# YangChenApril/AMContrast3D

Measured on AMD Instinct MI355X. Metric: train-step points/sec (fwd+bwd) on 24k-pt S3DIS clouds, higher is better.
Workload: dtype f32; 1 GPU; PointNeXt-S + AMContrast3D-AA, S3DIS-shaped 24000-pt voxelised (0.04 m) clouds, batch 8/GPU, fwd + CE/contrast loss + bwd + clip + AdamW; global_batch=8, points=24000, parallelism=dp1, launch=hipGraph replay, batches_per_joint_fps_launch=4, geometry_queue_cus=176, feature_graph_segments=1, collectives=none, update=captured in the feature graph

## Files before the change

### amcontrast3d_amd/_lib.py

```python
import ctypes
import os
import subprocess

_CSRC = os.path.join(os.path.dirname(os.path.abspath(__file__)), "csrc")
_SO = os.environ.get("AMC3D_LIB") or os.path.join(_CSRC, "libamc3d_hip.so")

_vp, _i, _f, _sz, _l = ctypes.c_void_p, ctypes.c_int, ctypes.c_float, ctypes.c_size_t, ctypes.c_long
_ll = ctypes.c_longlong

SIGNATURES = {
    "amc3d_version": (ctypes.c_char_p, []),
    "amc3d_last_error": (ctypes.c_char_p, []),
    "amc3d_stream_create_dedicated": (_i, [ctypes.POINTER(ctypes.c_void_p)]),
    "amc3d_stream_create_masked": (_i, [_vp, _i, _i]),
    "amc3d_reserve_scratch": (_i, [_i, _vp, _vp]),
    "amc3d_stream_destroy": (_i, [_vp]),
    "amc3d_grid_search_workspace_bytes": (_sz, [_i, _i, _i]),
    "amc3d_ball_query": (_i, [_i, _i, _i, _f, _i, _vp, _vp, _vp, _vp, _sz, _vp]),
    "amc3d_group_points": (_i, [_i, _i, _i, _i, _i, _vp, _vp, _vp, _vp]),
    "amc3d_group_points_grad": (_i, [_i, _i, _i, _i, _i, _vp, _vp, _vp, _vp, _sz, _vp]),
    "amc3d_gather_points": (_i, [_i, _i, _i, _i, _vp, _vp, _vp, _vp]),
    "amc3d_gather_points_grad": (_i, [_i, _i, _i, _i, _vp, _vp, _vp, _vp]),
    "amc3d_fps_workspace_bytes": (_sz, [_i, _i]),
    "amc3d_furthest_point_sampling": (_i, [_i, _i, _i, _vp, _vp, _vp, _vp, _sz, _vp]),
    "amc3d_three_nn": (_i, [_i, _i, _i, _vp, _vp, _vp, _vp, _vp, _sz, _vp]),
    "amc3d_three_interpolate": (_i, [_i, _i, _i, _i, _vp, _vp, _vp, _vp, _vp]),
    "amc3d_three_interpolate_add": (_i, [_i, _i, _i, _i, _vp, _vp, _vp, _vp, _vp, _vp]),
    "amc3d_three_interpolate_grad": (_i, [_i, _i, _i, _i, _vp, _vp, _vp, _vp, _vp, _sz, _vp]),
    "amc3d_three_interpolate_grad_route": (_i, [_i, _i, _i, _i, ctypes.POINTER(_i), ctypes.POINTER(_i)]),
    "amc3d_three_interpolate_grad_write": (_i, [_i, _i, _i, _i, _vp, _vp, _vp, _vp, _vp]),
    "amc3d_three_interpolate_grad_lds": (_i, [_i, _i, _i, _i, _i, _i, _i, _vp, _vp, _vp, _vp, _vp]),
    "amc3d_knnquery_workspace_bytes": (_sz, [_i, _i, _i, _i]),
    "amc3d_knnquery_uses_grid": (_i, [_i, _i, _i, _i]),
    "amc3d_knnquery": (_i, [_i, _i, _i, _i, _vp, _vp, _vp, _vp, _vp, _vp, _vp, _sz, _i, _vp]),
    "amc3d_vote_labels": (_i, [_i, _i, _i, _vp, _vp, _vp, _vp]),
    "amc3d_posmask": (_i, [_i, _i, _i, _vp, _vp, _vp, _vp]),
    "amc3d_ambiguity_workspace_bytes": (_sz, [_i]),
    "amc3d_ambiguity": (_i, [_i, _i, _i, _i, _f, _vp, _vp, _vp, _vp, _vp, _sz, _vp]),
    "amc3d_contrast_csr_workspace_bytes": (_sz, [_i]),
    "amc3d_contrast_csr": (_i, [_i, _i, _i, _vp, _vp, _vp, _vp, _sz, _vp]),
    "amc3d_contrast_backward_csr_supported": (_i, [_i]),
    "amc3d_contrast_backward_rows_supported": (_i, [_i]),
    "amc3d_contrast_backward_csr": (_i, [_i, _i, _i, _i, _vp, _vp, _vp, _vp, _vp, _vp, _vp, _f, _f, _f, _vp, _vp, _vp, _vp,
                                         _vp, _vp]),
    "amc3d_contrast_mutual_workspace_bytes": (_sz, [_i]),
    "amc3d_contrast_mutual": (_i, [_i, _i, _i, _vp, _vp, _vp, _vp, _vp, _vp, _sz, _vp]),
    "amc3d_contrast_backward_mutual_workspace_bytes": (_sz, [_i]),
    "amc3d_contrast_backward_mutual": (_i, [_i, _i, _i, _i, _vp, _vp, _vp, _vp, _vp, _vp, _vp, _f, _f, _f, _vp, _vp, _vp, _vp, _vp, _sz,
                                            _vp, _vp]),
    "amc3d_contrast_variant_forward": (_i, [_i, _i, _i, _i, _vp, _vp, _vp, _vp, _vp, _i, _i, _i, _i, _f, _f, _f, _vp, _vp, _vp, _vp,
                                            _vp, _vp]),
    "amc3d_contrast_variant_backward": (_i, [_i, _i, _i, _i, _vp, _vp, _vp, _vp, _vp, _vp, _vp, _i, _i, _i, _i, _f, _f, _f, _vp, _vp,
                                             _vp, _vp, _vp, _vp]),
    "amc3d_adamw_chunk": (_i, []),
    "amc3d_adamw_step": (_i, [_vp, _vp, _i, ctypes.c_double, ctypes.c_double, _f, _f, _vp, _vp, _vp]),
    "amc3d_select_anchors_ints": (_sz, [_i]),
    "amc3d_select_anchors": (_i, [_i, _vp, _vp, _sz, _vp]),
    "amc3d_contrast_forward": (_i, [_i, _i, _i, _i, _vp, _vp, _vp, _vp, _vp, _f, _f, _f, _vp, _vp, _vp, _vp, _vp, _vp, _vp]),
    "amc3d_contrast_forward_cm": (_i, [_i, _i, _i, _i, _i, _vp, _vp, _vp, _vp, _vp, _f, _f, _f, _vp, _vp, _vp, _vp, _vp, _vp, _vp]),
    "amc3d_contrast_backward": (_i, [_i, _i, _i, _i, _vp, _vp, _vp, _vp, _vp, _vp, _f, _f, _f, _vp, _vp, _vp, _vp, _vp]),
    "amc3d_grouped_conv_supported": (_i, [_i, _i]),
    "amc3d_transpose_cn": (_i, [_i, _i, _i, _vp, _vp, _vp]),
    "amc3d_grouped_conv_forward": (_i, [_i, _i, _i, _i, _i, _i, _vp, _vp, _vp, _vp, _vp, _vp]),
    "amc3d_grouped_conv_workspace_bytes": (_sz, [_i, _i, _i, _i, _i]),
    "amc3d_grouped_conv_backward": (_i, [_i, _i, _i, _i, _i, _i, _vp, _vp, _vp, _vp, _vp, _vp, _vp, _vp, _sz, _vp]),
    "amc3d_confusion_update": (_i, [_i, _i, _l, _vp, _vp, _ll, _i, _vp, _vp, _vp]),
    "amc3d_cross_entropy_workspace_bytes": (_sz, [_i, _l]),
    "amc3d_cross_entropy_forward": (_i, [_i, _i, _l, _vp, _vp, _ll, _vp, _vp, _vp, _sz, _vp]),
    "amc3d_cross_entropy_backward": (_i, [_i, _i, _l, _vp, _vp, _ll, _vp, _vp, _vp, _vp, _vp]),
    "amc3d_cross_entropy_general_workspace_bytes": (_sz, [_i, _l]),
    "amc3d_cross_entropy_general_forward": (_i, [_i, _i, _l, _vp, _vp, _ll, _i, _f, _vp, _vp, _vp, _vp, _sz, _vp]),
    "amc3d_cross_entropy_general_backward": (_i, [_i, _i, _l, _vp, _vp, _ll, _i, _f, _vp, _vp, _vp, _vp, _vp, _vp]),
    "amc3d_pointwise_conv_forward": (_i, [_i, _i, _i, _l, _vp, _vp, _vp, _vp, _vp]),
    "amc3d_pointwise_conv_forward_workspace_bytes": (_sz, [_i, _i, _i, _l, _i]),
    "amc3d_pointwise_conv_forward_ws": (_i, [_i, _i, _i, _l, _vp, _vp, _vp, _vp, _vp, _sz, _vp]),
    "amc3d_pointwise_conv_workspace_bytes": (_sz, [_i, _i, _i, _l]),
    "amc3d_pointwise_conv_backward": (_i, [_i, _i, _i, _l, _vp, _vp, _vp, _vp, _vp, _vp, _sz, _vp]),
    "amc3d_pointwise_conv_forward_strided": (_i, [_i, _i, _i, _l, _vp, _vp, _l, _vp, _vp, _vp, _sz, _vp]),
    "amc3d_pointwise_conv_backward_strided": (_i, [_i, _i, _i, _l, _vp, _vp, _l, _vp, _vp, _i, _vp, _l, _vp, _sz, _vp]),
    "amc3d_bn_residual_forward": (_i, [_i, _i, _l, _f, _f] + [_vp] * 11 + [_vp, _sz, _vp]),
    "amc3d_bn_residual_backward": (_i, [_i, _i, _l] + [_vp] * 11 + [_vp, _sz, _vp]),
    "amc3d_split_columns": (_i, [_i, _i, _i, _vp, _vp, _vp, _vp]),
    "amc3d_join_columns": (_i, [_i, _i, _i, _vp, _vp, _vp, _vp]),
    "amc3d_masked_refine_workspace_ints": (_sz, [_i]),
    "amc3d_masked_refine_forward": (_i, [_i, _i, _i, _i, _i, _vp, _vp, _vp, _f, _f, _f, _vp, _vp, _vp, _vp, _vp, _vp]),
    "amc3d_masked_refine_backward": (_i, [_i, _i, _i, _f, _vp, _vp, _vp, _vp, _vp]),
    "amc3d_bn_sigmoid_forward": (_i, [_i, _i, _l, _f, _f] + [_vp] * 10 + [_vp, _sz, _vp]),
    "amc3d_bn_sigmoid_backward": (_i, [_i, _i, _l] + [_vp] * 10 + [_vp, _sz, _vp]),
    "amc3d_bias_grad": (_i, [_i, _i, _l, _vp, _vp, _vp]),
    "amc3d_sa_residual_forward": (_i, [_i, _i, _i, _i, _i] + [_vp] * 8),
    "amc3d_sa_residual_workspace_bytes": (_sz, [_i, _i, _i, _i]),
    "amc3d_sa_residual_backward": (_i, [_i, _i, _i, _i, _i] + [_vp] * 11 + [_sz, _vp]),
    "amc3d_index_duplicates_workspace_bytes": (_sz, [_i, _i]),
    "amc3d_index_duplicates": (_i, [_i, _i, _i, _vp, _vp, _vp, _sz, _vp]),
    "amc3d_augment_workspace_bytes": (_sz, [_i]),
    "amc3d_augment_clouds": (_i, [_i, _i, _i, _f, _f] + [_vp] * 10 + [_sz, _vp]),
    "amc3d_voxelize_workspace_bytes": (_sz, [_i]),
    "amc3d_voxelize": (_i, [_i, _vp, ctypes.c_double] + [_vp] * 7 + [_sz, _vp]),
    "amc3d_voxel_select": (_i, [_i, _vp, _vp, _vp, _vp, _vp, _vp]),
    "amc3d_crop_nearest_workspace_bytes": (_sz, [_i]),
    "amc3d_crop_nearest": (_i, [_i, _vp, _i, _i, _vp, _vp, _vp, _sz, _vp]),
    "amc3d_voxelize_f64": (_i, [_i, _vp, ctypes.c_double] + [_vp] * 7 + [_sz, _vp]),
    "amc3d_crop_nearest_f64_workspace_bytes": (_sz, [_i]),
    "amc3d_crop_nearest_f64": (_i, [_i, _vp, _i, _i, _vp, _vp, _vp, _sz, _vp]),
    "amc3d_scannet_stats_workspace_bytes": (_sz, [_i]),
    "amc3d_scannet_room_stats": (_i, [_i, _vp, _vp, _vp, _vp, _vp, _sz, _vp]),
    "amc3d_scannet_transform_rooms": (_i, [_i, _ll] + [_vp] * 9 + [_vp]),
    "amc3d_scannet_crop_tail": (_i, [_i, _i] + [_vp] * 10 + [_vp]),
    "amc3d_s3dis_voxelize_workspace_bytes": (_sz, [_i, _ll]),
    "amc3d_s3dis_voxelize_rooms": (_i, [_i, _ll, _i, _vp, _vp, _vp, ctypes.c_double] + [_vp] * 8 + [_vp, _sz, _vp]),
    "amc3d_s3dis_crop_workspace_bytes": (_sz, [_i]),
    "amc3d_s3dis_select_crop": (_i, [_i, _i, _i, _i] + [_vp] * 13 + [_vp, _sz, _vp]),
    "amc3d_s3dis_crop_tail": (_i, [_i, _i, _i, _i] + [_vp] * 12 + [_vp]),
    "amc3d_scannet_voxelize_workspace_bytes": (_sz, [_i, _ll]),
    "amc3d_scannet_voxelize_rooms": (_i, [_i, _ll, _vp, _vp, ctypes.c_double] + [_vp] * 8 + [_vp, _sz, _vp]),
    "amc3d_scannet_crop_workspace_bytes": (_sz, [_i]),
    "amc3d_scannet_select_crop": (_i, [_i, _i, _i, _i] + [_vp] * 13 + [_vp, _sz, _vp]),
    "amc3d_scannet_crop_tail_workspace_bytes": (_sz, [_i]),
    "amc3d_scannet_crop_tail_rooms": (_i, [_i, _i, _i, _i] + [_vp] * 12 + [_vp, _sz, _vp]),
    "amc3d_room_parts": (_i, [_i, _i, _i] + [_vp] * 6 + [_vp]),
    "amc3d_part_batch_workspace_bytes": (_sz, [_i]),
    "amc3d_part_batch": (_i, [_i] * 6 + [_vp] * 12 + [_sz, _vp]),
    "amc3d_vote_parts": (_i, [_i, _i, _i, _i] + [_vp] * 8 + [_vp]),
    "amc3d_s3dis_part_batch_workspace_bytes": (_sz, [_i]),
    "amc3d_s3dis_part_batch": (_i, [_i] * 7 + [_vp] * 14 + [_sz, _vp]),
    "amc3d_room_representatives": (_i, [_i, _i] + [_vp] * 7 + [_vp]),
    "amc3d_expand_parts": (_i, [_i, _i, _i] + [_vp] * 6 + [_vp]),
    "amc3d_local_aggregation_supported": (_i, [_i, _i]),
    "amc3d_group_moments_bytes": (_sz, [_i, _i]),
    "amc3d_group_moments": (_i, [_i, _i, _i, _i, _vp, _vp, _vp, _sz, _vp]),
    "amc3d_local_aggregation_workspace_bytes": (_sz, [_i, _i, _i, _i]),
    "amc3d_local_aggregation_forward": (_i, [_i] * 7 + [_f, _f] + [_vp] * 18 + [_i, _vp, _vp, _sz, _vp]),
    "amc3d_local_aggregation_forward_strided": (_i, [_i] * 7 + [_f, _f] + [_vp] * 4 + [_l] + [_vp] * 14 + [_i, _vp, _vp, _sz, _vp]),
    "amc3d_local_aggregation_backward": (_i, [_i] * 6 + [_vp] * 17 + [_i, _vp, _vp, _vp, _sz, _vp]),
    "amc3d_local_aggregation_backward_strided": (_i, [_i] * 6 + [_vp] * 7 + [_l] + [_vp] * 8 + [_l] + [_vp] * 2 + [_i, _vp, _vp, _vp, _sz, _vp]),
    "amc3d_local_aggregation_csr_workspace_bytes": (_sz, [_i, _i, _i, _i]),
    "amc3d_local_aggregation_workspace_q_offset": (_sz, [_i, _i, _i, _i]),
    "amc3d_local_aggregation_backward_csr": (_i, [_i] * 6 + [_vp] * 19 + [_i, _vp, _vp, _vp, _sz, _vp]),
    "amc3d_local_aggregation_backward_csr_strided": (_i, [_i] * 6 + [_vp] * 7 + [_l] + [_vp] * 10 + [_l] + [_vp] * 2 + [_i, _vp, _vp, _vp, _sz, _vp]),
    "amc3d_three_interpolate_grad_csr": (_i, [_i, _i, _i, _i, _vp, _vp, _vp, _vp, _vp, _vp, _vp]),
    "amc3d_masked_refine_backward_csr": (_i, [_i, _i, _i, _f, _vp, _vp, _vp, _vp, _vp, _vp, _vp]),
    "amc3d_pointwise_conv_forward_bf16": (_i, [_i, _i, _i, _l, _vp, _vp, _vp, _vp, _vp]),
    "amc3d_pointwise_conv_workspace_bytes_bf16": (_sz, [_i, _i, _i, _l]),
    "amc3d_pointwise_conv_backward_bf16": (_i, [_i, _i, _i, _l, _vp, _vp, _vp, _vp, _vp, _vp, _sz, _vp]),
    "amc3d_grouped_conv_bn_supported": (_i, [_i, _i]),
    "amc3d_grouped_conv_bn_forward": (_i, [_i] * 7 + [_f, _f] + [_vp] * 16 + [_i, _vp, _vp, _sz, _vp]),
    "amc3d_grouped_conv_bn_forward_strided": (_i, [_i] * 7 + [_f, _f] + [_vp] * 4 + [_l] + [_vp] * 12 + [_i, _vp, _vp, _sz, _vp]),
    "amc3d_grouped_conv_bn_backward": (_i, [_i] * 6 + [_vp] * 15 + [_i, _vp, _vp, _vp, _sz, _vp]),
    "amc3d_grouped_conv_bn_backward_strided": (_i, [_i] * 6 + [_vp] * 5 + [_l] + [_vp] * 8 + [_l] + [_vp] * 2 + [_i, _vp, _vp, _vp, _sz, _vp]),
    "amc3d_group_csr_workspace_bytes": (_sz, [_i, _i, _i]),
    "amc3d_group_csr": (_i, [_i, _i, _i, _i, _vp, _vp, _vp, _vp, _sz, _vp]),
    "amc3d_group_moments_csr": (_i, [_i, _i, _i, _i, _vp, _vp, _vp, _vp, _sz, _vp]),
    "amc3d_grouped_conv_bn_csr_workspace_bytes": (_sz, [_i, _i, _i, _i, _i]),
    "amc3d_grouped_conv_bn_backward_csr": (_i, [_i] * 6 + [_vp, _i] + [_vp] * 16 + [_i, _vp, _vp, _vp, _sz, _vp]),
    "amc3d_grouped_conv_bn_backward_csr_strided": (_i, [_i] * 6 + [_vp, _i] + [_vp] * 6 + [_l] + [_vp] * 8 + [_l] + [_vp] * 2 + [_i, _vp, _vp, _vp, _sz, _vp]),
    "amc3d_group_csr_dp": (_i, [_i, _i, _i, _vp, _vp, _vp, _vp]),
    "amc3d_sa_tail_supported": (_i, [_i, _i, _i]),
    "amc3d_sa_tail_pays": (_i, [_i, _i]),
    "amc3d_sa_tail_workspace_bytes": (_sz, [_i, _i, _i, _i]),
    "amc3d_sa_tail_forward": (_i, [_i, _i, _i, _i, _i] + [_vp] * 8 + [_f, _f, _i] + [_vp] * 10 + [_sz, _vp]),
    "amc3d_sa_tail_backward": (_i, [_i, _i, _i, _i, _i] + [_vp] * 10 + [_i, _vp, _vp, _vp, _vp, _i] + [_vp] * 5 + [_sz, _vp]),
    "amc3d_bn_workspace_bytes": (_sz, [_i]),
    "amc3d_bn_stats": (_i, [_i, _i, _l, _f, _vp, _vp, _vp, _vp, _vp, _sz, _vp]),
    "amc3d_bn_forward": (_i, [_i, _i, _l, _i, _i, _f, _f, _vp, _vp, _vp, _vp, _vp, _vp, _vp, _vp, _vp, _vp, _vp, _vp, _sz, _vp]),
    "amc3d_bn_update_running": (_i, [_i, _f, _vp, _vp, _vp, _vp, _vp, _vp]),
    "amc3d_bn_act": (_i, [_i, _i, _l, _i, _vp, _vp, _vp, _vp, _vp, _vp, _vp]),
    "amc3d_bn_max": (_i, [_i, _i, _i, _i, _i, _vp, _vp, _vp, _vp, _vp, _vp, _vp, _vp]),
    "amc3d_bn_backward": (_i, [_i, _i, _l, _i, _i, _vp, _vp, _vp, _vp, _vp, _vp, _vp, _vp, _vp, _vp, _vp, _sz, _vp]),
    "amc3d_bn_sums": (_i, [_i, _i, _l, _vp, _vp, _vp, _sz, _vp]),
    "amc3d_bn_forward_synced": (_i, [_i, _i, _l, _i, _i, _f, _f, _vp, _vp, _vp, _vp, _vp, _vp, _vp, _vp, _vp, _vp, _vp, _vp, _vp]),
    "amc3d_bn_backward_sums": (_i, [_i, _i, _l, _i, _i, _vp, _vp, _vp, _vp, _vp, _vp, _vp, _vp, _vp, _vp, _vp, _sz, _vp]),
    "amc3d_bn_backward_synced": (_i, [_i, _i, _l, _i, _i, _vp, _vp, _vp, _vp, _vp, _vp, _vp, _vp, _vp, _vp, _vp]),
}


def build(force=False):
    cmd = ["make", "-C", _CSRC, "-j8"] + (["-B"] if force else [])
    proc = subprocess.run(cmd, stdout=subprocess.PIPE, stderr=subprocess.STDOUT, text=True)
    if proc.returncode != 0:
        raise RuntimeError("building libamc3d_hip.so failed:\n" + proc.stdout)
    return _SO


_lib = None


def load():
    global _lib
    if _lib is not None:
        return _lib
    if not os.path.exists(_SO):
        raise ImportError(
            f"{_SO} not found: the HIP extension is not built (run `python -c 'import __graft_entry__ as g; "
            f"g.build()'` or `make -C {_CSRC}`); there is no CPU fallback")
    import torch
    lib = ctypes.CDLL(_SO)
    for name, (res, args) in SIGNATURES.items():
        fn = getattr(lib, name)
        fn.restype = res
        fn.argtypes = args
    _lib = lib
    return lib


def check(status, what):
    if status != 0:
        raise RuntimeError(f"{what} failed (hipError {status}): {load().amc3d_last_error().decode()}")
```

### amcontrast3d_amd/csrc/loss.hip

```cpp
#include "common.h"

#include <type_traits>

namespace amc {

__global__ __launch_bounds__(256) void vote_labels_kernel(int m, int kr, int ncls, const int *__restrict__ labels0,
                                                          const int *__restrict__ nbr, int *__restrict__ out)
{
    const int lane = threadIdx.x & 63;
    const int q = blockIdx.x * 4 + (threadIdx.x >> 6);
    if (q >= m) return;
    int c0 = -1, c1 = -1;
    if (lane < kr) c0 = labels0[nbr[(size_t)q * kr + lane]];
    if (lane + 64 < kr) c1 = labels0[nbr[(size_t)q * kr + lane + 64]];
    int best = -1, bestc = 0;
    for (int c = 0; c < ncls; ++c) {
        const int cnt = (int)__popcll(__ballot(c0 == c)) + (int)__popcll(__ballot(c1 == c));
        if (cnt > best) { best = cnt; bestc = c; }
    }
    if (lane == 0) out[q] = bestc;
}

__global__ void posmask_kernel(int m, int k, int nbr_stride, const int *__restrict__ labels,
                               const int *__restrict__ nbr, unsigned char *__restrict__ posmask)
{
    const size_t t = (size_t)blockIdx.x * blockDim.x + threadIdx.x;
    if (t >= (size_t)m * k) return;
    const int i = (int)(t / k), j = (int)(t - (size_t)i * k);
    posmask[t] = labels[nbr[(size_t)i * nbr_stride + j]] == labels[i] ? 1 : 0;
}

__global__ __launch_bounds__(256) void ambiguity_stats_kernel(int m, int k, int nbr_stride, int mode,
                                                              const float *__restrict__ p,
                                                              const unsigned char *__restrict__ posmask,
                                                              const int *__restrict__ nbr, int *__restrict__ n_pos,
                                                              float *__restrict__ d_pos, float *__restrict__ d_neg,
                                                              int *__restrict__ max_npos)
{
    const int i = blockIdx.x * blockDim.x + threadIdx.x;
    int np = 0;
    if (i < m) {
        const float px = p[(size_t)i * 3], py = p[(size_t)i * 3 + 1], pz = p[(size_t)i * 3 + 2];
        const float ss = __fadd_rn(__fadd_rn(__fmul_rn(px, px), __fmul_rn(py, py)), __fmul_rn(pz, pz));
        float dp = 0.f, dn = 0.f;
        for (int j = 0; j < k; ++j) {
            const int nb = nbr[(size_t)i * nbr_stride + j];
            const float qx = p[(size_t)nb * 3], qy = p[(size_t)nb * 3 + 1], qz = p[(size_t)nb * 3 + 2];
            const float dot = __fadd_rn(__fadd_rn(__fmul_rn(px, qx), __fmul_rn(py, qy)), __fmul_rn(pz, qz));
            const float sd = __fadd_rn(__fadd_rn(__fmul_rn(qx, qx), __fmul_rn(qy, qy)), __fmul_rn(qz, qz));
            float dd = __fadd_rn(__fadd_rn(__fmul_rn(-2.f, dot), ss), sd);
            if (mode == 3) dd = sqrtf(__fadd_rn(fabsf(dd), 1e-12f));
            const bool pos = posmask[(size_t)i * k + j] != 0;
            np += pos ? 1 : 0;
            dp = __fadd_rn(dp, pos ? dd : 0.f);
            dn = __fadd_rn(dn, pos ? 0.f : dd);
        }
        n_pos[i] = np;
        d_pos[i] = mode == 1 ? 5.f : dp;
        d_neg[i] = mode == 1 ? 5.f : dn;
    }
    int w = np;
    for (int s = 32; s >= 1; s >>= 1) w = max(w, __shfl_xor(w, s, 64));
    if ((threadIdx.x & 63) == 0 && w > 0) atomicMax(max_npos, w);
}

__global__ void ambiguity_kernel(int m, int k, float beta, const int *__restrict__ n_pos,
                                 const float *__restrict__ d_pos, const float *__restrict__ d_neg,
                                 const int *__restrict__ max_npos, float *__restrict__ a)
{
    const int i = blockIdx.x * blockDim.x + threadIdx.x;
    if (i >= m) return;
    const int top = *max_npos;
    const int np = n_pos[i];
    float v = __fdiv_rn((float)abs(np - top), (float)top);
    if (0 < np && np < top) {
        const float cc = __fsub_rn(__fdiv_rn((float)np, d_pos[i]), __fdiv_rn((float)(k - np), d_neg[i]));
        v = __fdiv_rn(1.f, __fadd_rn(1.f, powf(2.718281828459045f, __fmul_rn(beta, cc))));
    }
    a[i] = v;
}

__global__ __launch_bounds__(256) void row_norm_kernel(int m, int C, const float *__restrict__ f,
                                                       float *__restrict__ norm)
{
    const int lane = threadIdx.x & 63;
    const int i = blockIdx.x * 4 + (threadIdx.x >> 6);
    if (i >= m) return;
    float s = 0.f;
    for (int c = lane; c < C; c += 64) {
        const float v = f[(size_t)i * C + c];
        s += v * v;
    }
    for (int sft = 32; sft >= 1; sft >>= 1) s += __shfl_xor(s, sft, 64);
    if (lane == 0) norm[i] = fmaxf(sqrtf(s), 1e-8f);
}

template <int LPR>
__global__ __launch_bounds__(256) void row_unit_kernel(int m, const float *__restrict__ f, float *__restrict__ norm,
                                                       float *__restrict__ unit)
{
    const int q = threadIdx.x & (LPR - 1);
    const long i = ((long)blockIdx.x * 256 + threadIdx.x) / LPR;
    if (i >= m) return;
    float4 v = reinterpret_cast<const float4 *>(f)[i * LPR + q];
    float s = v.x * v.x;
    s += v.y * v.y;
    s += v.z * v.z;
    s += v.w * v.w;
#pragma unroll
    for (int d = LPR / 2; d >= 1; d >>= 1) s += __shfl_xor(s, d, 64);
    const float n = fmaxf(sqrtf(s), 1e-8f);
    v.x = __fdiv_rn(v.x, n); v.y = __fdiv_rn(v.y, n); v.z = __fdiv_rn(v.z, n); v.w = __fdiv_rn(v.w, n);
    reinterpret_cast<float4 *>(unit)[i * LPR + q] = v;
    if (q == 0) norm[i] = n;
}

template <int LPR, int TP>
__global__ __launch_bounds__(256) void row_unit_cm_kernel(int n, const float *__restrict__ f_cm, float *__restrict__ norm,
                                                          float *__restrict__ unit)
{
    constexpr int C = 4 * LPR, TS = TP + 1;
    extern __shared__ float s_tile[];
    const int b = blockIdx.y, n0 = blockIdx.x * TP;
    for (int e = threadIdx.x; e < C * TP; e += 256) {
        const int ch = e / TP, pt = e - ch * TP;
        s_tile[ch * TS + pt] = n0 + pt < n ? f_cm[((size_t)b * C + ch) * n + n0 + pt] : 0.f;
    }
    __syncthreads();
    const int q = threadIdx.x & (LPR - 1);
    for (int pl = threadIdx.x / LPR; pl < TP; pl += 256 / LPR) {
        float4 v = make_float4(s_tile[(4 * q) * TS + pl], s_tile[(4 * q + 1) * TS + pl], s_tile[(4 * q + 2) * TS + pl],
                               s_tile[(4 * q + 3) * TS + pl]);
        float s = v.x * v.x;
        s += v.y * v.y;
        s += v.z * v.z;
        s += v.w * v.w;
#pragma unroll
        for (int d = LPR / 2; d >= 1; d >>= 1) s += __shfl_xor(s, d, 64);
        const float nv = fmaxf(sqrtf(s), 1e-8f);
        v.x = __fdiv_rn(v.x, nv); v.y = __fdiv_rn(v.y, nv); v.z = __fdiv_rn(v.z, nv); v.w = __fdiv_rn(v.w, nv);
        if (n0 + pl < n) {
            const size_t i = (size_t)b * n + n0 + pl;
            reinterpret_cast<float4 *>(unit)[i * LPR + q] = v;
            if (q == 0) norm[i] = nv;
        }
    }
}

__device__ __forceinline__ bool contrast_selected(float a) { return 0.f < a && a <= 1.f; }

__device__ __forceinline__ bool contrast_anchor(const int *__restrict__ sel, int m, int w, const float *__restrict__ a, int &i,
                                                float &ai)
{
    if (w >= (sel ? sel[0] : m)) return false;
    i = sel ? sel[1 + w] : w;
    ai = a[i];
    return true;
}

__device__ __forceinline__ float contrast_margin(float mu, float a, float nu) { return __fadd_rn(__fmul_rn(mu, a), nu); }

__device__ __forceinline__ float contrast_exp(float s, bool pos, float margin, float temperature)
{
    return expf(__fdiv_rn(pos ? __fsub_rn(s, margin) : s, temperature));
}

__device__ __forceinline__ float contrast_coef(float scale, float psum, float tsum, float temperature)
{
    const float r = psum / tsum;
    return -scale / ((r + 1e-12f) * tsum * tsum * temperature);
}

__device__ __forceinline__ float contrast_edge_g(float coef, float e, bool pos, float nsum, float psum)
{
    return coef * e * (pos ? nsum : -psum);
}

__device__ __forceinline__ float group32_sum(float v)
{
#pragma unroll
    for (int s = 16; s >= 1; s >>= 1) v += __shfl_xor(v, s, 64);
    return v;
}

struct ContrastSums { float psum, nsum, tsum; };

__device__ __forceinline__ ContrastSums contrast_sums32(int k, int sub, const unsigned char *__restrict__ pm_i,
                                                        const float *__restrict__ sim_i, float margin, float temperature)
{
    ContrastSums r{0.f, 0.f, 0.f};
    for (int j = sub; j < k; j += 32) {
        const bool pos = pm_i[j] != 0;
        const float e = contrast_exp(sim_i[j], pos, margin, temperature);
        r.psum += pos ? e : 0.f;
        r.nsum += pos ? 0.f : e;
        r.tsum += e;
    }
    for (int s = 16; s >= 1; s >>= 1) {
        r.psum += __shfl_xor(r.psum, s, 64);
        r.nsum += __shfl_xor(r.nsum, s, 64);
        r.tsum += __shfl_xor(r.tsum, s, 64);
    }
    return r;
}

__device__ __forceinline__ float row_cosine(const float *__restrict__ fi, const float *__restrict__ fj, float ni, float nj, int C)
{
    float a0 = 0.f, a1 = 0.f, a2 = 0.f, a3 = 0.f;
    if ((C & 3) == 0) {
        for (int c = 0; c < C; c += 4) {
            const float4 u = *reinterpret_cast<const float4 *>(fi + c);
            const float4 v = *reinterpret_cast<const float4 *>(fj + c);
            a0 += __fdiv_rn(u.x, ni) * __fdiv_rn(v.x, nj);
            a1 += __fdiv_rn(u.y, ni) * __fdiv_rn(v.y, nj);
            a2 += __fdiv_rn(u.z, ni) * __fdiv_rn(v.z, nj);
            a3 += __fdiv_rn(u.w, ni) * __fdiv_rn(v.w, nj);
        }
    } else {
        int c = 0;
        for (; c + 3 < C; c += 4) {
            a0 += __fdiv_rn(fi[c], ni) * __fdiv_rn(fj[c], nj);
            a1 += __fdiv_rn(fi[c + 1], ni) * __fdiv_rn(fj[c + 1], nj);
            a2 += __fdiv_rn(fi[c + 2], ni) * __fdiv_rn(fj[c + 2], nj);
            a3 += __fdiv_rn(fi[c + 3], ni) * __fdiv_rn(fj[c + 3], nj);
        }
        for (; c < C; ++c) a0 += __fdiv_rn(fi[c], ni) * __fdiv_rn(fj[c], nj);
    }
    return (a0 + a1) + (a2 + a3);
}

__device__ __forceinline__ float unit_dot4(const float4 &a, const float4 &b)
{
    return __fmaf_rn(a.w, b.w, __fmaf_rn(a.z, b.z, __fmaf_rn(a.y, b.y, __fmul_rn(a.x, b.x))));
}

constexpr int UNIT_U = 4;

template <int LPR>
__device__ __forceinline__ void unit_row_cosines(const float4 *__restrict__ h4, const float4 &u, int q, const int (&x)[UNIT_U],
                                                 float4 (&v)[UNIT_U], float (&s)[UNIT_U])
{
#pragma unroll
    for (int t = 0; t < UNIT_U; ++t) v[t] = x[t] >= 0 ? h4[(unsigned)x[t] * (unsigned)LPR + (unsigned)q] : make_float4(0.f, 0.f, 0.f, 0.f);
#pragma unroll
    for (int t = 0; t < UNIT_U; ++t) {
        float acc = unit_dot4(u, v[t]);
#pragma unroll
        for (int d = LPR / 2; d >= 1; d >>= 1) acc += __shfl_xor(acc, d, 64);
        s[t] = acc;
    }
}

template <int LPR>
__device__ __forceinline__ void unit_gather_indices(const int *__restrict__ nbr, int i, int nbr_stride, int k, int j0, int r,
                                                    int (&nb)[UNIT_U])
{
#pragma unroll
    for (int t = 0; t < UNIT_U; ++t) {
        const int j = j0 + t * (64 / LPR) + r;
        nb[t] = j < k ? nbr[(size_t)i * nbr_stride + j] : -1;
    }
}

template <int LPR>
__device__ __forceinline__ float unit_gather_rows(const float4 *__restrict__ h4, const float4 &u, int q, const int (&nb)[UNIT_U])
{
    float4 v[UNIT_U];
    float c[UNIT_U];
    unit_row_cosines<LPR>(h4, u, q, nb, v, c);
    float s = 0.f;
#pragma unroll
    for (int t = 0; t < UNIT_U; ++t) s = q == t ? c[t] : s;
    return s;
}

__device__ __forceinline__ float contrast_projection(float norm, float s) { return norm > 1e-8f ? s : 0.f; }

template <int LPA, int VPT>
struct EdgeWalk {
    static constexpr int U = VPT >= 8 ? 2 : (VPT >= 4 ? 4 : 8);
    float fhi[VPT], gi[VPT];

    __device__ __forceinline__ void begin(int C, int sub, const float *__restrict__ f, int i, float ni)
    {
#pragma unroll
        for (int v = 0; v < VPT; ++v) {
            const int c = sub + v * LPA;
            fhi[v] = c < C ? __fdiv_rn(f[(size_t)i * C + c], ni) : 0.f;
            gi[v] = 0.f;
        }
    }

    __device__ __forceinline__ void chunk(int C, int sub, const float *__restrict__ f, float ni, int cnt, int nb_l, float sj_l,
                                          float nj_l, float g_l, float *__restrict__ grad_f)
    {
        for (int jj = 0; jj < cnt; jj += U) {
            int nb[U];
            float fj[U][VPT];
#pragma unroll
            for (int u = 0; u < U; ++u) {
                const int src = min(jj + u, LPA - 1);
                const int t = __shfl(nb_l, src, LPA);
                nb[u] = jj + u < cnt ? t : -1;
            }
#pragma unroll
            for (int u = 0; u < U; ++u)
#pragma unroll
                for (int v = 0; v < VPT; ++v) {
                    const int c = sub + v * LPA;
                    fj[u][v] = (nb[u] >= 0 && c < C) ? f[(size_t)nb[u] * C + c] : 0.f;
                }
#pragma unroll
            for (int u = 0; u < U; ++u) {
                const int src = min(jj + u, LPA - 1);
                const float g = __shfl(g_l, src, LPA), sj = __shfl(sj_l, src, LPA), nj = __shfl(nj_l, src, LPA);
                if (nb[u] < 0) continue;
                const float gin = g / ni, gjn = g / nj;
                const float si = contrast_projection(ni, sj), sx = contrast_projection(nj, sj);
#pragma unroll
                for (int v = 0; v < VPT; ++v) {
                    const int c = sub + v * LPA;
                    if (c < C) {
                        const float fhj = __fdiv_rn(fj[u][v], nj);
                        gi[v] += gin * (fhj - si * fhi[v]);
                        atomicAdd(grad_f + (size_t)nb[u] * C + c, gjn * (fhi[v] - sx * fhj));
                    }
                }
            }
        }
    }

    __device__ __forceinline__ void finish(int C, int sub, int i, float *__restrict__ grad_f)
    {
#pragma unroll
        for (int v = 0; v < VPT; ++v) {
            const int c = sub + v * LPA;
            if (c < C) atomicAdd(grad_f + (size_t)i * C + c, gi[v]);
        }
    }
};

__device__ __forceinline__ void rows_edge(int t, int total, int own, int n, int k, const int *__restrict__ nbr_n,
                                          const int *__restrict__ rev_n, const float *__restrict__ gco,
                                          const float *__restrict__ sim, int &x, float &g, float &s)
{
    x = -1; g = 0.f; s = 0.f;
    if (t < total) {
        int pos;
        if (t < own) { pos = n * k + t; x = nbr_n[t]; }
        else { pos = rev_n[t - own]; x = pos / k; }
        g = gco[pos];
        s = sim[pos];
    }
}

__device__ __forceinline__ void rows_accumulate(float4 &acc, float g, float s, float nn, const float4 &fn, const float4 &v, float nx)
{
    const float gn = g / nn;
    const float sn = contrast_projection(nn, s);
    acc.x += gn * (__fdiv_rn(v.x, nx) - sn * fn.x);
    acc.y += gn * (__fdiv_rn(v.y, nx) - sn * fn.y);
    acc.z += gn * (__fdiv_rn(v.z, nx) - sn * fn.z);
    acc.w += gn * (__fdiv_rn(v.w, nx) - sn * fn.w);
}

__global__ __launch_bounds__(256) void select_count_kernel(int m, const float *__restrict__ a, int *__restrict__ sel)
{
    __shared__ int s_cnt[4];
    const int i = blockIdx.x * 256 + threadIdx.x;
    const bool s = i < m && contrast_selected(a[i]);
    const int c = (int)__popcll(__ballot(s));
    if ((threadIdx.x & 63) == 0) s_cnt[threadIdx.x >> 6] = c;
    __syncthreads();
    if (threadIdx.x == 0) sel[(size_t)m + 1 + blockIdx.x] = s_cnt[0] + s_cnt[1] + s_cnt[2] + s_cnt[3];
}

__global__ __launch_bounds__(256) void select_write_kernel(int m, const float *__restrict__ a, int *__restrict__ sel)
{
    __shared__ int s_part[4], s_cnt[4];
    const int *bc = sel + (size_t)m + 1;
    int before = 0;
    for (int b = threadIdx.x; b < (int)blockIdx.x; b += 256) before += bc[b];
    for (int s = 32; s >= 1; s >>= 1) before += __shfl_xor(before, s, 64);
    const int i = blockIdx.x * 256 + threadIdx.x;
    const bool sl = i < m && contrast_selected(a[i]);
    const unsigned long long mask = __ballot(sl);
    const int lane = threadIdx.x & 63, wv = threadIdx.x >> 6;
    if (lane == 0) { s_part[wv] = before; s_cnt[wv] = (int)__popcll(mask); }
    __syncthreads();
    int base = s_part[0] + s_part[1] + s_part[2] + s_part[3];
    for (int w = 0; w < wv; ++w) base += s_cnt[w];
    if (sl) sel[1 + base + (int)__popcll(mask & ((1ull << lane) - 1ull))] = i;
    if (blockIdx.x == gridDim.x - 1 && threadIdx.x == 0)
        sel[0] = s_part[0] + s_part[1] + s_part[2] + s_part[3] + s_cnt[0] + s_cnt[1] + s_cnt[2] + s_cnt[3];
}

template <int LPR>
__global__ __launch_bounds__(256) void contrast_forward_unit_kernel(
    int m, int k, int nbr_stride, const float *__restrict__ unit, const int *__restrict__ nbr,
    const unsigned char *__restrict__ posmask, const float *__restrict__ a, const int *__restrict__ sel, float mu, float nu,
    float temperature, float *__restrict__ sim, float *__restrict__ stats, float *__restrict__ loss_pt)
{
    constexpr int R = 64 / LPR;
    const int lane = threadIdx.x & 63, q = lane & (LPR - 1), r = lane / LPR;
    int i;
    float ai;
    if (!contrast_anchor(sel, m, blockIdx.x * 4 + (threadIdx.x >> 6), a, i, ai)) return;
    if (!contrast_selected(ai)) {
        if (lane == 0) loss_pt[i] = 0.f;
        return;
    }
    const float margin = contrast_margin(mu, ai, nu);
    const float4 *h4 = reinterpret_cast<const float4 *>(unit);
    const float4 u = h4[(size_t)i * LPR + q];
    float psum = 0.f, tsum = 0.f, nsum = 0.f;
    for (int j0 = 0; j0 < k; j0 += UNIT_U * R) {
        int nb[UNIT_U];
        unit_gather_indices<LPR>(nbr, i, nbr_stride, k, j0, r, nb);
        const int jq = j0 + q * R + r;
        const bool mine = q < UNIT_U && jq < k;
        const bool pos = mine ? posmask[(size_t)i * k + jq] != 0 : false;
        const float s = unit_gather_rows<LPR>(h4, u, q, nb);
        if (mine) {
            if (sim) sim[(size_t)i * k + jq] = s;
            const float e = contrast_exp(s, pos, margin, temperature);
            psum += pos ? e : 0.f;
            nsum += pos ? 0.f : e;
            tsum += e;
        }
    }
#pragma unroll
    for (int d = 1; d < 64; d <<= 1) {
        psum += __shfl_xor(psum, d, 64);
        tsum += __shfl_xor(tsum, d, 64);
    }
    if (stats) {
#pragma unroll
        for (int d = 1; d < 64; d <<= 1) nsum += __shfl_xor(nsum, d, 64);
    }
    if (lane == 0) {
        loss_pt[i] = -logf(__fadd_rn(__fdiv_rn(psum, tsum), 1e-12f));
        if (stats) { stats[(size_t)i * 2] = psum; stats[(size_t)i * 2 + 1] = nsum; }
    }
}

__global__ __launch_bounds__(256) void contrast_forward_kernel(
    int m, int C, int k, int nbr_stride, const float *__restrict__ f, const float *__restrict__ norm,
    const int *__restrict__ nbr, const unsigned char *__restrict__ posmask, const float *__restrict__ a,
    const int *__restrict__ sel, float mu, float nu, float temperature, float *__restrict__ sim,
    float *__restrict__ loss_pt)
{
    const int sub = threadIdx.x & 31;
    int i;
    float ai;
    if (!contrast_anchor(sel, m, (blockIdx.x * blockDim.x + threadIdx.x) >> 5, a, i, ai)) return;
    if (!contrast_selected(ai)) {
        if (sub == 0) loss_pt[i] = 0.f;
        return;
    }
    const float ni = norm[i];
    const float margin = contrast_margin(mu, ai, nu);
    const float *fi = f + (size_t)i * C;
    float psum = 0.f, tsum = 0.f;
    for (int j0 = 0; j0 < k; j0 += 32) {
        const int j = j0 + sub;
        float e = 0.f;
        bool pos = false;
        if (j < k) {
            const int nb = nbr[(size_t)i * nbr_stride + j];
            const float nj = norm[nb];
            const float acc = row_cosine(fi, f + (size_t)nb * C, ni, nj, C);
            sim[(size_t)i * k + j] = acc;
            pos = posmask[(size_t)i * k + j] != 0;
            e = contrast_exp(acc, pos, margin, temperature);
        }
        psum += pos ? e : 0.f;
        tsum += e;
    }
    for (int s = 16; s >= 1; s >>= 1) {
        psum += __shfl_xor(psum, s, 64);
        tsum += __shfl_xor(tsum, s, 64);
    }
    if (sub == 0) loss_pt[i] = -logf(__fadd_rn(__fdiv_rn(psum, tsum), 1e-12f));
}

__global__ __launch_bounds__(1024) void masked_mean_kernel(int m, const float *__restrict__ loss_pt,
                                                           const float *__restrict__ a, float *__restrict__ out)
{
    __shared__ double s_sum[16];
    __shared__ int s_cnt[16];
    double sum = 0.0;
    int cnt = 0;
    const int m4 = ((((uintptr_t)loss_pt | (uintptr_t)a) & 15) == 0) ? (m & ~3) : 0;
    for (int i0 = threadIdx.x * 4; i0 < m4; i0 += 4096 * 4) {
        float4 lv[4], av[4];
#pragma unroll
        for (int u = 0; u < 4; ++u) {
            const int i = i0 + u * 4096;
            const bool ok = i < m4;
            lv[u] = ok ? *reinterpret_cast<const float4 *>(loss_pt + i) : make_float4(0.f, 0.f, 0.f, 0.f);
            av[u] = ok ? *reinterpret_cast<const float4 *>(a + i) : make_float4(-1.f, -1.f, -1.f, -1.f);
        }
#pragma unroll
        for (int u = 0; u < 4; ++u) {
            const float l4[4] = {lv[u].x, lv[u].y, lv[u].z, lv[u].w}, a4[4] = {av[u].x, av[u].y, av[u].z, av[u].w};
#pragma unroll
            for (int e = 0; e < 4; ++e)
                if (contrast_selected(a4[e])) { sum += (double)l4[e]; cnt += 1; }
        }
    }
    for (int i = m4 + threadIdx.x; i < m; i += 1024) {
        const float ai = a[i];
        if (contrast_selected(ai)) { sum += (double)loss_pt[i]; cnt += 1; }
    }
    for (int s = 32; s >= 1; s >>= 1) {
        sum += __shfl_xor(sum, s, 64);
        cnt += __shfl_xor(cnt, s, 64);
    }
    if ((threadIdx.x & 63) == 0) { s_sum[threadIdx.x >> 6] = sum; s_cnt[threadIdx.x >> 6] = cnt; }
    __syncthreads();
    if (threadIdx.x == 0) {
        double t = 0.0;
        int c = 0;
        for (int w = 0; w < 16; ++w) { t += s_sum[w]; c += s_cnt[w]; }
        out[0] = (float)(t / (double)c);
        out[1] = (float)c;
    }
}

template <int LPA, int VPT>
__global__ __launch_bounds__(256) void contrast_backward_kernel(
    int m, int C, int k, int nbr_stride, const float *__restrict__ f, const float *__restrict__ norm,
    const int *__restrict__ nbr, const unsigned char *__restrict__ posmask, const float *__restrict__ a,
    const int *__restrict__ sel, float mu, float nu, float temperature, const float *__restrict__ sim,
    const float *__restrict__ mean_cnt, const float *__restrict__ grad_out, float *__restrict__ grad_f)
{
    const int sub = threadIdx.x & (LPA - 1);
    int i;
    float ai;
    if (!contrast_anchor(sel, m, (blockIdx.x * blockDim.x + threadIdx.x) / LPA, a, i, ai)) return;
    if (!contrast_selected(ai)) return;
    const float scale = grad_out[0] / mean_cnt[1];
    const float ni = norm[i];
    const float margin = contrast_margin(mu, ai, nu);

    EdgeWalk<LPA, VPT> walk;
    walk.begin(C, sub, f, i, ni);
    int nb_l = -1;
    bool pos_l = false;
    float sj_l = 0.f, nj_l = 1.f, e_l = 0.f;
    auto load_chunk = [&](int j0) {
        const int j = j0 + sub;
        nb_l = -1; pos_l = false; sj_l = 0.f; nj_l = 1.f; e_l = 0.f;
        if (j < k) {
            nb_l = nbr[(size_t)i * nbr_stride + j];
            pos_l = posmask[(size_t)i * k + j] != 0;
            sj_l = sim[(size_t)i * k + j];
            nj_l = norm[nb_l];
            e_l = contrast_exp(sj_l, pos_l, margin, temperature);
        }
    };
    float psum = 0.f, tsum = 0.f, nsum = 0.f;
    for (int j0 = (k - 1) / LPA * LPA; j0 >= 0; j0 -= LPA) {
        load_chunk(j0);
        psum += pos_l ? e_l : 0.f;
        nsum += pos_l ? 0.f : e_l;
        tsum += e_l;
    }
#pragma unroll
    for (int s = LPA / 2; s >= 1; s >>= 1) {
        psum += __shfl_xor(psum, s, 64);
        nsum += __shfl_xor(nsum, s, 64);
        tsum += __shfl_xor(tsum, s, 64);
    }
    const float coef = contrast_coef(scale, psum, tsum, temperature);
    if (psum == 0.f) return;

    for (int j0 = 0; j0 < k; j0 += LPA) {
        if (j0 > 0) load_chunk(j0);
        const float g_l = contrast_edge_g(coef, e_l, pos_l, nsum, psum);
        walk.chunk(C, sub, f, ni, min(LPA, k - j0), nb_l, sj_l, nj_l, g_l, grad_f);
    }
    walk.finish(C, sub, i, grad_f);
}

__global__ __launch_bounds__(256) void contrast_coef_kernel(
    int m, int k, const unsigned char *__restrict__ posmask, const float *__restrict__ a, const int *__restrict__ sel,
    float mu, float nu, float temperature, const float *__restrict__ sim, const float *__restrict__ mean_cnt,
    const float *__restrict__ grad_out, float *__restrict__ gco)
{
    const int sub = threadIdx.x & 31;
    int i;
    float ai;
    if (!contrast_anchor(sel, m, (blockIdx.x * blockDim.x + threadIdx.x) >> 5, a, i, ai)) return;
    const float scale = grad_out[0] / mean_cnt[1];
    const float margin = contrast_margin(mu, ai, nu);
    const unsigned char *pm_i = posmask + (size_t)i * k;
    const float *sim_i = sim + (size_t)i * k;
    const ContrastSums t = contrast_sums32(k, sub, pm_i, sim_i, margin, temperature);
    const float coef = t.psum == 0.f ? 0.f : contrast_coef(scale, t.psum, t.tsum, temperature);
    for (int j = sub; j < k; j += 32) {
        const bool pos = pm_i[j] != 0;
        const float e = contrast_exp(sim_i[j], pos, margin, temperature);
        gco[(size_t)i * k + j] = t.psum == 0.f ? 0.f : contrast_edge_g(coef, e, pos, t.nsum, t.psum);
    }
}

template <int LPR>
__global__ __launch_bounds__(256) void contrast_backward_rows_kernel(
    int m, int k, int nbr_stride, const float *__restrict__ f, const float *__restrict__ norm,
    const int *__restrict__ nbr, const float *__restrict__ a, const int *__restrict__ rev,
    const float *__restrict__ sim, const float *__restrict__ gco, float *__restrict__ grad_f)
{
    constexpr int R = 64 / LPR;
    constexpr int U = 4;
    const int lane = threadIdx.x & 63, q = lane & (LPR - 1), r = lane / LPR;
    const int n = blockIdx.x * 4 + (threadIdx.x >> 6);
    if (n >= m) return;
    const float an = a[n];
    const int own = contrast_selected(an) ? k : 0;
    const int e0 = rev[n], deg = rev[n + 1] - e0;
    const int *rev_edge = rev + m + 1;
    const int total = own + deg;
    const float4 *f4 = reinterpret_cast<const float4 *>(f);
    float4 acc = make_float4(0.f, 0.f, 0.f, 0.f);
    if (total > 0) {
        const float nn = norm[n];
        float4 fn = f4[(size_t)n * LPR + q];
        fn.x = __fdiv_rn(fn.x, nn); fn.y = __fdiv_rn(fn.y, nn); fn.z = __fdiv_rn(fn.z, nn); fn.w = __fdiv_rn(fn.w, nn);
        for (int t0 = 0; t0 < total; t0 += U * R) {
            int x[U];
            float g[U], sv[U], nx[U];
            float4 v[U];
#pragma unroll
            for (int u = 0; u < U; ++u)
                rows_edge(t0 + u * R + r, total, own, n, k, nbr + (size_t)n * nbr_stride, rev_edge + e0, gco, sim, x[u], g[u], sv[u]);
#pragma unroll
            for (int u = 0; u < U; ++u) {
                nx[u] = x[u] >= 0 ? norm[x[u]] : 1.f;
                v[u] = x[u] >= 0 ? f4[(size_t)x[u] * LPR + q] : make_float4(0.f, 0.f, 0.f, 0.f);
            }
#pragma unroll
            for (int u = 0; u < U; ++u) {
                if (x[u] < 0) continue;
                rows_accumulate(acc, g[u], sv[u], nn, fn, v[u], nx[u]);
            }
        }
#pragma unroll
        for (int s = LPR; s < 64; s <<= 1) {
            acc.x += __shfl_xor(acc.x, s, 64);
            acc.y += __shfl_xor(acc.y, s, 64);
            acc.z += __shfl_xor(acc.z, s, 64);
            acc.w += __shfl_xor(acc.w, s, 64);
        }
    }
    if (r == 0) reinterpret_cast<float4 *>(grad_f)[(size_t)n * LPR + q] = acc;
}

template <int P>
__global__ __launch_bounds__(256) void contrast_backward_rows_wide_kernel(
    int m, int C4, int k, int nbr_stride, const float *__restrict__ f, const float *__restrict__ norm,
    const int *__restrict__ nbr, const float *__restrict__ a, const int *__restrict__ rev,
    const float *__restrict__ sim, const float *__restrict__ gco, float *__restrict__ grad_f)
{
    constexpr int U = 4;
    const int q = threadIdx.x & 63;
    const int n = blockIdx.x * 4 + (threadIdx.x >> 6);
    if (n >= m) return;
    const float an = a[n];
    const int own = contrast_selected(an) ? k : 0;
    const int e0 = rev[n], deg = rev[n + 1] - e0;
    const int *rev_edge = rev + m + 1;
    const int total = own + deg;
    const float4 *f4 = reinterpret_cast<const float4 *>(f);
    const float4 zero = make_float4(0.f, 0.f, 0.f, 0.f);
    float4 acc[P];
#pragma unroll
    for (int p = 0; p < P; ++p) acc[p] = zero;
    if (total > 0) {
        const float nn = norm[n];
        float4 fn[P];
#pragma unroll
        for (int p = 0; p < P; ++p) {
            const int piece = q + 64 * p;
            fn[p] = piece < C4 ? f4[(size_t)n * C4 + piece] : zero;
            fn[p].x = __fdiv_rn(fn[p].x, nn); fn[p].y = __fdiv_rn(fn[p].y, nn);
            fn[p].z = __fdiv_rn(fn[p].z, nn); fn[p].w = __fdiv_rn(fn[p].w, nn);
        }
        for (int t0 = 0; t0 < total; t0 += U) {
            int x[U];
            float g[U], sv[U], nx[U];
            float4 v[U][P];
#pragma unroll
            for (int u = 0; u < U; ++u)
                rows_edge(t0 + u, total, own, n, k, nbr + (size_t)n * nbr_stride, rev_edge + e0, gco, sim, x[u], g[u], sv[u]);
#pragma unroll
            for (int u = 0; u < U; ++u) {
                nx[u] = x[u] >= 0 ? norm[x[u]] : 1.f;
#pragma unroll
                for (int p = 0; p < P; ++p) {
                    const int piece = q + 64 * p;
                    v[u][p] = (x[u] >= 0 && piece < C4) ? f4[(size_t)x[u] * C4 + piece] : zero;
                }
            }
#pragma unroll
            for (int u = 0; u < U; ++u) {
                if (x[u] < 0) continue;
#pragma unroll
                for (int p = 0; p < P; ++p) rows_accumulate(acc[p], g[u], sv[u], nn, fn[p], v[u][p], nx[u]);
            }
        }
    }
#pragma unroll
    for (int p = 0; p < P; ++p) {
        const int piece = q + 64 * p;
        if (piece < C4) reinterpret_cast<float4 *>(grad_f)[(size_t)n * C4 + piece] = acc[p];
    }
}

struct __attribute__((aligned(16))) ContrastRecord { float norm, coef, tsum, psum, margin, nsum, pad1, pad2; };

__global__ __launch_bounds__(256) void contrast_record_kernel(
    int m, int k, const float *__restrict__ norm, const unsigned char *__restrict__ posmask, const float *__restrict__ a,
    float mu, float nu, float temperature, const float *__restrict__ sim, const float *__restrict__ mean_cnt,
    const float *__restrict__ grad_out, ContrastRecord *__restrict__ rec)
{
    const int sub = threadIdx.x & 31;
    const int i = (blockIdx.x * blockDim.x + threadIdx.x) >> 5;
    if (i >= m) return;
    const float ai = a[i];
    const bool selected = contrast_selected(ai);
    const float margin = contrast_margin(mu, ai, nu);
    const ContrastSums t = contrast_sums32(selected ? k : 0, sub, posmask + (size_t)i * k, sim + (size_t)i * k, margin, temperature);
    if (sub == 0) {
        const float scale = grad_out[0] / mean_cnt[1];
        ContrastRecord o;
        o.norm = norm[i];
        o.coef = (selected && t.psum != 0.f) ? contrast_coef(scale, t.psum, t.tsum, temperature) : 0.f;
        o.tsum = t.tsum; o.psum = t.psum; o.margin = margin; o.nsum = t.nsum; o.pad1 = o.pad2 = 0.f;
        rec[i] = o;
    }
}

__global__ __launch_bounds__(256) void contrast_record_stats_kernel(int m, const float *__restrict__ norm, const float *__restrict__ a,
                                                                    float mu, float nu, float temperature,
                                                                    const float *__restrict__ stats, const float *__restrict__ mean_cnt,
                                                                    const float *__restrict__ grad_out, ContrastRecord *__restrict__ rec)
{
    const int i = blockIdx.x * 256 + threadIdx.x;
    if (i >= m) return;
    const float ai = a[i];
    const bool selected = contrast_selected(ai);
    const float psum = selected ? stats[(size_t)i * 2] : 0.f, nsum = selected ? stats[(size_t)i * 2 + 1] : 1.f;
    const float tsum = __fadd_rn(psum, nsum);
    const float scale = grad_out[0] / mean_cnt[1];
    ContrastRecord o;
    o.norm = norm[i];
    o.coef = (selected && psum != 0.f) ? contrast_coef(scale, psum, tsum, temperature) : 0.f;
    o.tsum = tsum; o.psum = psum; o.margin = contrast_margin(mu, ai, nu); o.nsum = nsum; o.pad1 = o.pad2 = 0.f;
    rec[i] = o;
}

template <int LPR>
__global__ __launch_bounds__(256) void contrast_backward_mutual_kernel(
    int m, int k, int nbr_stride, const float *__restrict__ unit, const int *__restrict__ nbr,
    const unsigned char *__restrict__ posmask, const unsigned char *__restrict__ mutual, const int *__restrict__ rev,
    const ContrastRecord *__restrict__ rec, float temperature, float *__restrict__ grad_f)
{
    constexpr int R = 64 / LPR;
    constexpr int U = UNIT_U;
    const int lane = threadIdx.x & 63, q = lane & (LPR - 1), r = lane / LPR, row0 = lane & ~(LPR - 1);
    const int n = blockIdx.x * 4 + (threadIdx.x >> 6);
    if (n >= m) return;
    const float4 *h4 = reinterpret_cast<const float4 *>(unit);
    const float4 *rec4 = reinterpret_cast<const float4 *>(rec);
    const float4 rn0 = rec4[(size_t)n * 2];
    const float4 rn1 = rec4[(size_t)n * 2 + 1];
    const float margin_n = rn1.x, nsum_n = rn1.y;
    const float nn = rn0.x, coef_n = rn0.y, psum_n = rn0.w;
    const float4 fn = h4[(size_t)n * LPR + q];
    const int e0 = rev[n], deg = rev[n + 1] - e0;
    const int *rev_edge = rev + m + 1;
    const int total = k + deg;
    float4 acc = make_float4(0.f, 0.f, 0.f, 0.f);
    for (int t0 = 0; t0 < total; t0 += U * R) {
        const int tq = t0 + q * R + r;
        int myx = -1;
        bool pos = false, own = false;
        float inc = 0.f;
        if (q < U) {
            if (tq < k) {
                myx = nbr[(size_t)n * nbr_stride + tq];
                pos = posmask[(size_t)n * k + tq] != 0;
                inc = (float)(mutual[(size_t)n * k + tq] & 0x7f);
                own = coef_n != 0.f;
                if (!own && inc == 0.f) myx = -1;
            } else if (tq < total) {
                const int p = rev_edge[e0 + tq - k];
                myx = p / k;
                pos = posmask[p] != 0;
                inc = 1.f;
            }
        }
        int x[U];
        float4 v[U];
#pragma unroll
        for (int u = 0; u < U; ++u) x[u] = __shfl(myx, row0 | u, 64);
        const float4 rx = myx >= 0 ? rec4[(size_t)myx * 2] : make_float4(1.f, 0.f, 1.f, 0.f);
        const float4 rx1 = myx >= 0 ? rec4[(size_t)myx * 2 + 1] : make_float4(0.f, 0.f, 0.f, 0.f);
        const float mx = rx1.x;
        float s[U], smine = 0.f;
        unit_row_cosines<LPR>(h4, fn, q, x, v, s);
#pragma unroll
        for (int u = 0; u < U; ++u) smine = q == u ? s[u] : smine;
        float gn = 0.f;
        if (myx >= 0) {
            float g = 0.f;
            if (own) {
                g += contrast_edge_g(coef_n, contrast_exp(smine, pos, margin_n, temperature), pos, nsum_n, psum_n);
            }
            if (inc != 0.f && rx.y != 0.f) {
                g += inc * contrast_edge_g(rx.y, contrast_exp(smine, pos, mx, temperature), pos, rx1.y, rx.w);
            }
            gn = g / nn;
        }
#pragma unroll
        for (int u = 0; u < U; ++u) {
            const float gu = __shfl(gn, row0 | u, 64);
            const float sn = contrast_projection(nn, s[u]);
            acc.x = __fmaf_rn(gu, __fmaf_rn(-sn, fn.x, v[u].x), acc.x);
            acc.y = __fmaf_rn(gu, __fmaf_rn(-sn, fn.y, v[u].y), acc.y);
            acc.z = __fmaf_rn(gu, __fmaf_rn(-sn, fn.z, v[u].z), acc.z);
            acc.w = __fmaf_rn(gu, __fmaf_rn(-sn, fn.w, v[u].w), acc.w);
        }
    }
#pragma unroll
    for (int d = LPR; d < 64; d <<= 1) {
        acc.x += __shfl_xor(acc.x, d, 64);
        acc.y += __shfl_xor(acc.y, d, 64);
        acc.z += __shfl_xor(acc.z, d, 64);
        acc.w += __shfl_xor(acc.w, d, 64);
    }
    if (r == 0) reinterpret_cast<float4 *>(grad_f)[(size_t)n * LPR + q] = acc;
}

template <int LPR>
__global__ __launch_bounds__(256) void contrast_sim_unit_kernel(
    int m, int k, int nbr_stride, const float *__restrict__ unit, const int *__restrict__ nbr, const float *__restrict__ a,
    const int *__restrict__ sel, float *__restrict__ sim)
{
    constexpr int R = 64 / LPR;
    const int lane = threadIdx.x & 63, q = lane & (LPR - 1), r = lane / LPR;
    int i;
    float ai;
    if (!contrast_anchor(sel, m, blockIdx.x * 4 + (threadIdx.x >> 6), a, i, ai)) return;
    if (!contrast_selected(ai)) return;
    const float4 *h4 = reinterpret_cast<const float4 *>(unit);
    const float4 u = h4[(size_t)i * LPR + q];
    for (int j0 = 0; j0 < k; j0 += UNIT_U * R) {
        int nb[UNIT_U];
        unit_gather_indices<LPR>(nbr, i, nbr_stride, k, j0, r, nb);
        const int jq = j0 + q * R + r;
        const float s = unit_gather_rows<LPR>(h4, u, q, nb);
        if (q < UNIT_U && jq < k) sim[(size_t)i * k + jq] = s;
    }
}

__global__ __launch_bounds__(256) void contrast_sim_kernel(
    int m, int C, int k, int nbr_stride, const float *__restrict__ f, const float *__restrict__ norm,
    const int *__restrict__ nbr, const float *__restrict__ a, const int *__restrict__ sel, float *__restrict__ sim)
{
    const int sub = threadIdx.x & 31;
    int i;
    float ai;
    if (!contrast_anchor(sel, m, (blockIdx.x * blockDim.x + threadIdx.x) >> 5, a, i, ai)) return;
    if (!contrast_selected(ai)) return;
    const float ni = norm[i];
    const float *fi = f + (size_t)i * C;
    for (int j = sub; j < k; j += 32) {
        const int nb = nbr[(size_t)i * nbr_stride + j];
        const float nj = norm[nb];
        sim[(size_t)i * k + j] = row_cosine(fi, f + (size_t)nb * C, ni, nj, C);
    }
}

struct ContrastForm { int margin_mode, db, method, has_temperature; float mu, nu, temperature; };

__device__ __forceinline__ float variant_arg(const ContrastForm &F, float s, bool pos, float margin)
{
    float z = s;
    if (F.db == 1) z = pos ? __fsub_rn(s, margin) : s;
    else if (F.db == 2) z = pos ? s : __fadd_rn(s, margin);
    return F.has_temperature ? __fdiv_rn(z, F.temperature) : z;
}

struct ContrastAnchorSums { float margin, psum, nsum, npos, ysum, wsum; };

__device__ __forceinline__ ContrastAnchorSums variant_anchor_sums(const ContrastForm &F, int k, int sub, float ai,
                                                                 const float *__restrict__ sim_i,
                                                                 const unsigned char *__restrict__ pm_i)
{
    ContrastAnchorSums r;
    r.margin = F.nu;
    if (F.margin_mode == 1) r.margin = contrast_margin(F.mu, ai, F.nu);
    if (F.margin_mode == 2) {
        float su = 0.f, sv = 0.f;
        for (int j = sub; j < k; j += 32) {
            const bool pos = pm_i[j] != 0;
            const float s = sim_i[j];
            su += pos ? 0.f : s;
            sv += pos ? s : 0.f;
        }
        const float u = __fdiv_rn(group32_sum(su), (float)k), v = __fdiv_rn(group32_sum(sv), (float)k);
        r.margin = __fadd_rn(__fmul_rn(__fsub_rn(u, 1.f), ai), v);
    }
    float psum = 0.f, nsum = 0.f, npos = 0.f;
    for (int j = sub; j < k; j += 32) {
        const bool pos = pm_i[j] != 0;
        const float e = expf(variant_arg(F, sim_i[j], pos, r.margin));
        psum += pos ? e : 0.f;
        nsum += pos ? 0.f : e;
        npos += pos ? 1.f : 0.f;
    }
    r.psum = group32_sum(psum);
    r.nsum = group32_sum(nsum);
    r.npos = group32_sum(npos);
    r.ysum = r.wsum = 0.f;
    if (F.method == 2) {
        float y = 0.f, wv = 0.f;
        for (int j = sub; j < k; j += 32) {
            const bool pos = pm_i[j] != 0;
            const float ep = pos ? expf(variant_arg(F, sim_i[j], pos, r.margin)) : 0.f;
            const float den = ep + r.nsum;
            y += __fadd_rn(__fdiv_rn(ep, den), 1e-12f);
            wv += pos ? __fdiv_rn(__fdiv_rn(ep, den), den) : 0.f;
        }
        r.ysum = group32_sum(y);
        r.wsum = group32_sum(wv);
    }
    return r;
}

__global__ __launch_bounds__(256) void contrast_variant_loss_kernel(
    int m, int k, const unsigned char *__restrict__ posmask, const float *__restrict__ a, const int *__restrict__ sel,
    ContrastForm F, const float *__restrict__ sim, float *__restrict__ loss_pt)
{
    const int sub = threadIdx.x & 31;
    int i;
    float ai;
    if (!contrast_anchor(sel, m, (blockIdx.x * blockDim.x + threadIdx.x) >> 5, a, i, ai)) return;
    if (!contrast_selected(ai)) {
        if (sub == 0) loss_pt[i] = 0.f;
        return;
    }
    const ContrastAnchorSums r = variant_anchor_sums(F, k, sub, ai, sim + (size_t)i * k, posmask + (size_t)i * k);
    if (sub == 0) {
        const float ratio = F.method == 2 ? __fdiv_rn(r.ysum, __fadd_rn(r.npos, 1e-12f))
                                          : __fadd_rn(__fdiv_rn(r.psum, __fadd_rn(r.psum, r.nsum)), 1e-12f);
        loss_pt[i] = -logf(ratio);
    }
}

__global__ __launch_bounds__(256) void contrast_variant_coef_kernel(
    int m, int k, const unsigned char *__restrict__ posmask, const float *__restrict__ a, const int *__restrict__ sel,
    ContrastForm F, const float *__restrict__ sim, const float *__restrict__ mean_cnt,
    const float *__restrict__ grad_out, float *__restrict__ gco)
{
    const int sub = threadIdx.x & 31;
    int i;
    float ai;
    if (!contrast_anchor(sel, m, (blockIdx.x * blockDim.x + threadIdx.x) >> 5, a, i, ai)) return;
    if (!contrast_selected(ai)) return;
    const float *sim_i = sim + (size_t)i * k;
    const unsigned char *pm_i = posmask + (size_t)i * k;
    const ContrastAnchorSums r = variant_anchor_sums(F, k, sub, ai, sim_i, pm_i);
    const float scale = grad_out[0] / mean_cnt[1];
    const float inv_t = F.has_temperature ? 1.f / F.temperature : 1.f;
    float cp, cn, qpos;
    bool dead = false;
    if (F.method == 2) {
        cp = -1.f / r.ysum;
        cn = r.wsum / r.ysum;
        qpos = -r.nsum * cn;
    } else {
        const float S = r.psum + r.nsum, rp = r.psum / S, rn = r.nsum / S;
        const float den = (rp + 1e-12f) * S;
        cp = -rn / den;
        cn = rp / den;
        qpos = -rn * rp / (rp + 1e-12f);
        dead = r.psum == 0.f;
    }
    const float dm = F.db != 0 ? -inv_t * qpos : 0.f;
    const float dm_pos = F.margin_mode == 2 ? dm / (float)k : 0.f, dm_neg = dm_pos * ai;
    for (int j = sub; j < k; j += 32) {
        const bool pos = pm_i[j] != 0;
        const float e = expf(variant_arg(F, sim_i[j], pos, r.margin));
// ... 111 lines not shown
    const long long t = target[(size_t)b * N + n];
    const bool counted = t != ignore && t >= 0 && t < C;
    const float scale = counted ? grad_out[0] / mean_cnt[1] : 0.f;
    const float l = lse[(size_t)b * N + n];
    for (int c = 0; c < C; ++c) {
        const float p = __expf(x[(size_t)c * N] - l);
        d[(size_t)c * N] = scale * (p - (c == (int)t ? 1.f : 0.f));
    }
}

__global__ __launch_bounds__(CE_THREADS) void ce_general_forward_kernel(int C, long N, const float *__restrict__ logits,
                                                                        const long long *__restrict__ target, long long ignore,
                                                                        int has_ignore, float eps, const float *__restrict__ weight,
                                                                        float *__restrict__ lse, double *__restrict__ partial)
{
    __shared__ double s_num[CE_THREADS / 64], s_den[CE_THREADS / 64];
    const int b = blockIdx.y;
    const long n = (long)blockIdx.x * CE_THREADS + threadIdx.x;
    double num = 0.0, den = 0.0;
    if (n < N) {
        const float *x = logits + (size_t)b * C * N + n;
        float mx = -__builtin_inff();
        for (int c = 0; c < C; ++c) mx = fmaxf(mx, x[(size_t)c * N]);
        float se = 0.f;
        for (int c = 0; c < C; ++c) se += expf(x[(size_t)c * N] - mx);
        const float l = mx + logf(se);
        lse[(size_t)b * N + n] = l;
        const long long t = target[(size_t)b * N + n];
        if (!(has_ignore && t == ignore) && t >= 0 && t < C) {
            const float wy = weight ? weight[t] : 1.f;
            den = (double)wy;
            num = (1.0 - (double)eps) * (double)wy * (double)(l - x[(size_t)t * N]);
            if (eps > 0.f) {
                float sm = 0.f;
                for (int c = 0; c < C; ++c) {
                    const float nlp = l - x[(size_t)c * N];
                    sm += weight ? weight[c] * nlp : nlp;
                }
                num += (double)eps / (double)C * (double)sm;
            }
        }
    }
    for (int s = 32; s >= 1; s >>= 1) {
        num += __shfl_xor(num, s, 64);
        den += __shfl_xor(den, s, 64);
    }
    if ((threadIdx.x & 63) == 0) { s_num[threadIdx.x >> 6] = num; s_den[threadIdx.x >> 6] = den; }
    __syncthreads();
    if (threadIdx.x == 0) {
        double t = 0.0, d = 0.0;
        for (int w = 0; w < CE_THREADS / 64; ++w) { t += s_num[w]; d += s_den[w]; }
        const size_t slot = (size_t)blockIdx.y * gridDim.x + blockIdx.x;
        partial[slot * 2] = t;
        partial[slot * 2 + 1] = d;
    }
}

__global__ __launch_bounds__(CE_THREADS) void ce_general_backward_kernel(int C, long N, const float *__restrict__ logits,
                                                                         const long long *__restrict__ target, long long ignore,
                                                                         int has_ignore, float eps, const float *__restrict__ weight,
                                                                         const float *__restrict__ lse,
                                                                         const float *__restrict__ loss_den,
                                                                         const float *__restrict__ grad_out,
                                                                         float *__restrict__ dlogits)
{
    const int b = blockIdx.y;
    const long n = (long)blockIdx.x * CE_THREADS + threadIdx.x;
    if (n >= N) return;
    const float *x = logits + (size_t)b * C * N + n;
    float *d = dlogits + (size_t)b * C * N + n;
    const long long t = target[(size_t)b * N + n];
    if ((has_ignore && t == ignore) || t < 0 || t >= C) {
        for (int c = 0; c < C; ++c) d[(size_t)c * N] = 0.f;
        return;
    }
    float wsum = (float)C;
    if (weight) {
        wsum = 0.f;
        for (int c = 0; c < C; ++c) wsum += weight[c];
    }
    const float scale = grad_out[0] / loss_den[1];
    const float hard = (1.f - eps) * (weight ? weight[t] : 1.f);
    const float soft = eps / (float)C;
    const float l = lse[(size_t)b * N + n];
    for (int c = 0; c < C; ++c) {
        const float p = expf(x[(size_t)c * N] - l);
        const float wc = weight ? weight[c] : 1.f;
        d[(size_t)c * N] = scale * (hard * (p - (c == (int)t ? 1.f : 0.f)) + soft * (p * wsum - wc));
    }
}

}

using namespace amc;

AMC_API int amc3d_vote_labels(int m, int kr, int num_classes, const int *labels0, const int *nbr_idx, int *labels,
                              void *stream)
{
    if (m <= 0) return 0;
    if (kr <= 0 || kr > 128 || num_classes <= 0 || !labels0 || !nbr_idx || !labels)
        return bad_arg("amc3d_vote_labels: bad argument (kr must be in 1..128)");
    hipLaunchKernelGGL(vote_labels_kernel, dim3(div_up(m, 4)), dim3(256), 0, (hipStream_t)stream, m, kr, num_classes,
                       labels0, nbr_idx, labels);
    return launch_status("amc3d_vote_labels");
}

AMC_API int amc3d_posmask(int m, int k, int nbr_stride, const int *labels, const int *nbr, unsigned char *posmask,
                          void *stream)
{
    if (m <= 0) return 0;
    if (k <= 0 || nbr_stride < k || !labels || !nbr || !posmask) return bad_arg("amc3d_posmask: bad argument");
    hipLaunchKernelGGL(posmask_kernel, dim3(div_up((long)m * k, 256)), dim3(256), 0, (hipStream_t)stream, m, k,
                       nbr_stride, labels, nbr, posmask);
    return launch_status("amc3d_posmask");
}

AMC_API size_t amc3d_ambiguity_workspace_bytes(int m) { return (size_t)m * 12 + 64; }

AMC_API int amc3d_ambiguity(int m, int k, int nbr_stride, int mode, float beta, const float *p,
                            const unsigned char *posmask, const int *nbr, float *a, void *workspace,
                            size_t workspace_bytes, void *stream_)
{
    if (m <= 0) return 0;
    if (k <= 0 || nbr_stride < k || mode < 1 || mode > 3 || !p || !posmask || !nbr || !a || !workspace ||
        workspace_bytes < amc3d_ambiguity_workspace_bytes(m))
        return bad_arg("amc3d_ambiguity: bad argument");
    hipStream_t stream = (hipStream_t)stream_;
    int *max_npos = (int *)workspace;
    int *n_pos = (int *)((char *)workspace + 64);
    float *d_pos = (float *)(n_pos + m);
    float *d_neg = d_pos + m;
    if (int st = fill_i32(max_npos, 0, 1, stream)) return st;
    hipLaunchKernelGGL(ambiguity_stats_kernel, dim3(div_up(m, 256)), dim3(256), 0, stream, m, k, nbr_stride, mode, p,
                       posmask, nbr, n_pos, d_pos, d_neg, max_npos);
    hipLaunchKernelGGL(ambiguity_kernel, dim3(div_up(m, 256)), dim3(256), 0, stream, m, k, beta, n_pos, d_pos, d_neg,
                       max_npos, a);
    return launch_status("amc3d_ambiguity");
}

AMC_API size_t amc3d_select_anchors_ints(int m) { return (size_t)(m > 0 ? m : 0) + 1 + (size_t)div_up(m > 0 ? m : 1, 256); }

AMC_API int amc3d_select_anchors(int m, const float *a, int *sel, size_t sel_ints, void *stream_)
{
    if (m < 0 || !sel || sel_ints < amc3d_select_anchors_ints(m) || (m > 0 && !a))
        return bad_arg("amc3d_select_anchors: bad argument");
    hipStream_t stream = (hipStream_t)stream_;
    if (m == 0) return fill_i32(sel, 0, 1, stream);
    const int nb = div_up(m, 256);
    hipLaunchKernelGGL(select_count_kernel, dim3(nb), dim3(256), 0, stream, m, a, sel);
    hipLaunchKernelGGL(select_write_kernel, dim3(nb), dim3(256), 0, stream, m, a, sel);
    return launch_status("amc3d_select_anchors");
}

template <int N> using int_c = std::integral_constant<int, N>;

template <class F>
static bool with_lpr(int C, F &&fn)
{
    switch (C) {
    case 16: fn(int_c<4>{}); return true;
    case 32: fn(int_c<8>{}); return true;
    case 64: fn(int_c<16>{}); return true;
    case 128: fn(int_c<32>{}); return true;
    case 256: fn(int_c<64>{}); return true;
    default: return false;
    }
}

template <class F>
static void with_wide_p(int C, F &&fn)
{
    if (C < 256) fn(int_c<1>{});
    else fn(int_c<2>{});
}

template <class F>
static void with_lpa_vpt(int C, F &&fn)
{
    if (C <= 32) fn(int_c<32>{}, int_c<1>{});
    else if (C <= 64) fn(int_c<64>{}, int_c<1>{});
    else if (C <= 128) fn(int_c<64>{}, int_c<2>{});
    else if (C <= 256) fn(int_c<64>{}, int_c<4>{});
    else fn(int_c<64>{}, int_c<8>{});
}

static bool contrast_rows_ok(const float *f, const float *unit, int m, int C)
{
    return unit && ((((uintptr_t)f) | ((uintptr_t)unit)) & 15) == 0 && amc3d_contrast_backward_csr_supported(C) &&
           (long)m * C < (1L << 34);
}

static int contrast_forward_launch(int cm_b, int m, int C, int k, int nbr_stride, const float *f, const int *nbr,
                                   const unsigned char *posmask, const float *a, const int *sel, float mu, float nu,
                                   float temperature, float *norm, float *unit, float *sim, float *stats, float *loss_pt,
                                   float *mean_cnt, hipStream_t stream)
{
    const bool rows = contrast_rows_ok(f, unit, m, C);
    if (cm_b > 0 && !rows) return bad_arg("amc3d_contrast_forward_cm: C must be 16, 32, 64, 128 or 256; unit required, 16-byte aligned");
    if (!sim && !(rows && stats)) return bad_arg("amc3d_contrast_forward: sim may be NULL only with the unit-row kernels and stats");
    if (rows) {
        const bool launched = with_lpr(C, [&](auto lpr) {
            constexpr int LPR = decltype(lpr)::value;
            if (cm_b > 0) {
                constexpr int TP = LPR >= 32 ? 16 : 64;
                const size_t lds = (size_t)4 * LPR * (TP + 1) * sizeof(float);
                hipLaunchKernelGGL((row_unit_cm_kernel<LPR, TP>), dim3(div_up(m / cm_b, TP), cm_b), dim3(256), lds, stream,
                                   m / cm_b, f, norm, unit);
            } else
                hipLaunchKernelGGL((row_unit_kernel<LPR>), dim3(div_up((long)m * LPR, 256)), dim3(256), 0, stream, m, f, norm, unit);
            hipLaunchKernelGGL((contrast_forward_unit_kernel<LPR>), dim3(div_up(m, 4)), dim3(256), 0, stream, m, k, nbr_stride,
                               (const float *)unit, nbr, posmask, a, sel, mu, nu, temperature, sim, stats, loss_pt);
        });
        if (!launched) return bad_arg("amc3d_contrast_forward: no unit-row kernel for this width");
    } else {
        hipLaunchKernelGGL(row_norm_kernel, dim3(div_up(m, 4)), dim3(256), 0, stream, m, C, f, norm);
        hipLaunchKernelGGL(contrast_forward_kernel, dim3(div_up((long)m * 32, 256)), dim3(256), 0, stream, m, C, k,
                           nbr_stride, f, norm, nbr, posmask, a, sel, mu, nu, temperature, sim, loss_pt);
    }
    hipLaunchKernelGGL(masked_mean_kernel, dim3(1), dim3(1024), 0, stream, m, loss_pt, a, mean_cnt);
    return launch_status("amc3d_contrast_forward");
}

AMC_API int amc3d_contrast_forward(int m, int C, int k, int nbr_stride, const float *f, const int *nbr,
                                   const unsigned char *posmask, const float *a, const int *sel, float mu, float nu,
                                   float temperature, float *norm, float *unit, float *sim, float *stats, float *loss_pt,
                                   float *mean_cnt, void *stream_)
{
    if (m <= 0) return 0;
    if (C <= 0 || k <= 0 || nbr_stride < k || !f || !nbr || !posmask || !a || !norm || !loss_pt || !mean_cnt)
        return bad_arg("amc3d_contrast_forward: bad argument");
    return contrast_forward_launch(0, m, C, k, nbr_stride, f, nbr, posmask, a, sel, mu, nu, temperature, norm, unit, sim, stats,
                                   loss_pt, mean_cnt, (hipStream_t)stream_);
}

AMC_API int amc3d_contrast_forward_cm(int b, int C, int n, int k, int nbr_stride, const float *f_cm, const int *nbr,
                                      const unsigned char *posmask, const float *a, const int *sel, float mu, float nu,
                                      float temperature, float *norm, float *unit, float *sim, float *stats, float *loss_pt,
                                      float *mean_cnt, void *stream_)
{
    if (b <= 0 || n <= 0) return 0;
    if ((long)b * n > 0x7fffffffL || C <= 0 || k <= 0 || nbr_stride < k || !f_cm || !nbr || !posmask || !a || !norm || !unit ||
        !loss_pt || !mean_cnt)
        return bad_arg("amc3d_contrast_forward_cm: bad argument");
    return contrast_forward_launch(b, b * n, C, k, nbr_stride, f_cm, nbr, posmask, a, sel, mu, nu, temperature, norm, unit, sim,
                                   stats, loss_pt, mean_cnt, (hipStream_t)stream_);
}

AMC_API int amc3d_contrast_backward(int m, int C, int k, int nbr_stride, const float *f, const float *norm,
                                    const int *nbr, const unsigned char *posmask, const float *a, const int *sel,
                                    float mu, float nu, float temperature, const float *sim, const float *mean_cnt,
                                    const float *grad_out, float *grad_f, void *stream_)
{
    if (m <= 0) return 0;
    if (C <= 0 || C > 512 || k <= 0 || !f || !norm || !nbr || !posmask || !a || !sim || !mean_cnt || !grad_out || !grad_f)
        return bad_arg("amc3d_contrast_backward: bad argument (C must be in 1..512)");
    hipStream_t stream = (hipStream_t)stream_;
    with_lpa_vpt(C, [&](auto lpa, auto vpt) {
        constexpr int LPA = decltype(lpa)::value, VPT = decltype(vpt)::value;
        hipLaunchKernelGGL((contrast_backward_kernel<LPA, VPT>), dim3(div_up((long)m * LPA, 256)), dim3(256), 0, stream, m, C, k,
                           nbr_stride, f, norm, nbr, posmask, a, sel, mu, nu, temperature, sim, mean_cnt, grad_out, grad_f);
    });
    return launch_status("amc3d_contrast_backward");
}

AMC_API int amc3d_contrast_backward_csr_supported(int C)
{
    return C == 16 || C == 32 || C == 64 || C == 128 || C == 256;
}

AMC_API int amc3d_contrast_backward_rows_supported(int C) { return C % 4 == 0 && C >= 4 && C <= 512; }

static void contrast_rows_launch(int m, int C, int k, int nbr_stride, const float *f, const float *norm, const int *nbr,
                                 const float *a, const int *rev, const float *sim, const float *gco, float *grad_f,
                                 hipStream_t stream)
{
    const bool narrow = with_lpr(C, [&](auto lpr) {
        hipLaunchKernelGGL((contrast_backward_rows_kernel<decltype(lpr)::value>), dim3(div_up(m, 4)), dim3(256), 0, stream, m, k,
                           nbr_stride, f, norm, nbr, a, rev, sim, gco, grad_f);
    });
    if (!narrow)
        with_wide_p(C, [&](auto p) {
            hipLaunchKernelGGL((contrast_backward_rows_wide_kernel<decltype(p)::value>), dim3(div_up(m, 4)), dim3(256), 0, stream,
                               m, C / 4, k, nbr_stride, f, norm, nbr, a, rev, sim, gco, grad_f);
        });
}

AMC_API int amc3d_contrast_backward_csr(int m, int C, int k, int nbr_stride, const float *f, const float *norm,
                                        const int *nbr, const unsigned char *posmask, const float *a, const int *sel,
                                        const int *rev, float mu, float nu, float temperature, const float *sim,
                                        const float *mean_cnt, const float *grad_out, float *gco, float *grad_f,
                                        void *stream_)
{
    if (m <= 0) return 0;
    if (!amc3d_contrast_backward_rows_supported(C) || k <= 0 || nbr_stride < k || !f || !norm || !nbr || !posmask || !a ||
        !sel || !rev || !sim || !mean_cnt || !grad_out || !gco || !grad_f || (((uintptr_t)f | (uintptr_t)grad_f) & 15))
        return bad_arg("amc3d_contrast_backward_csr: bad argument (C must be a multiple of 4 in 4..512; 16-byte aligned rows)");
    hipStream_t stream = (hipStream_t)stream_;
    hipLaunchKernelGGL(contrast_coef_kernel, dim3(div_up((long)m * 32, 256)), dim3(256), 0, stream, m, k, posmask, a, sel, mu,
                       nu, temperature, sim, mean_cnt, grad_out, gco);
    contrast_rows_launch(m, C, k, nbr_stride, f, norm, nbr, a, rev, sim, gco, grad_f, stream);
    return launch_status("amc3d_contrast_backward_csr");
}

static bool contrast_form_ok(int margin_mode, int db, int method, int has_temperature, float temperature)
{
    return margin_mode >= 0 && margin_mode <= 2 && db >= 0 && db <= 2 && (method == 1 || method == 2) &&
           (has_temperature == 0 || (has_temperature == 1 && temperature != 0.f));
}

AMC_API int amc3d_contrast_variant_forward(int m, int C, int k, int nbr_stride, const float *f, const int *nbr,
                                           const unsigned char *posmask, const float *a, const int *sel, int margin_mode,
                                           int db, int method, int has_temperature, float mu, float nu, float temperature,
                                           float *norm, float *unit, float *sim, float *loss_pt, float *mean_cnt,
                                           void *stream_)
{
    if (m <= 0) return 0;
    if (C <= 0 || k <= 0 || nbr_stride < k || !f || !nbr || !posmask || !a || !norm || !sim || !loss_pt || !mean_cnt ||
        !contrast_form_ok(margin_mode, db, method, has_temperature, temperature))
        return bad_arg("amc3d_contrast_variant_forward: bad argument (margin_mode 0..2, db 0..2, method 1..2, has_temperature 0..1)");
    hipStream_t stream = (hipStream_t)stream_;
    const ContrastForm F{margin_mode, db, method, has_temperature, mu, nu, temperature};
    if (contrast_rows_ok(f, unit, m, C)) {
        const bool launched = with_lpr(C, [&](auto lpr) {
            constexpr int LPR = decltype(lpr)::value;
            hipLaunchKernelGGL((row_unit_kernel<LPR>), dim3(div_up((long)m * LPR, 256)), dim3(256), 0, stream, m, f, norm, unit);
            hipLaunchKernelGGL((contrast_sim_unit_kernel<LPR>), dim3(div_up(m, 4)), dim3(256), 0, stream, m, k, nbr_stride,
                               (const float *)unit, nbr, a, sel, sim);
        });
        if (!launched) return bad_arg("amc3d_contrast_variant_forward: no unit-row kernel for this width");
    } else {
        hipLaunchKernelGGL(row_norm_kernel, dim3(div_up(m, 4)), dim3(256), 0, stream, m, C, f, norm);
        hipLaunchKernelGGL(contrast_sim_kernel, dim3(div_up((long)m * 32, 256)), dim3(256), 0, stream, m, C, k, nbr_stride, f,
                           (const float *)norm, nbr, a, sel, sim);
    }
    hipLaunchKernelGGL(contrast_variant_loss_kernel, dim3(div_up((long)m * 32, 256)), dim3(256), 0, stream, m, k, posmask, a, sel,
                       F, (const float *)sim, loss_pt);
    hipLaunchKernelGGL(masked_mean_kernel, dim3(1), dim3(1024), 0, stream, m, loss_pt, a, mean_cnt);
    return launch_status("amc3d_contrast_variant_forward");
}

AMC_API int amc3d_contrast_variant_backward(int m, int C, int k, int nbr_stride, const float *f, const float *norm,
                                            const int *nbr, const unsigned char *posmask, const float *a, const int *sel,
                                            const int *rev, int margin_mode, int db, int method, int has_temperature,
                                            float mu, float nu, float temperature, const float *sim, const float *mean_cnt,
                                            const float *grad_out, float *gco, float *grad_f, void *stream_)
{
    if (m <= 0) return 0;
    if (C <= 0 || C > 512 || k <= 0 || nbr_stride < k || !f || !norm || !nbr || !posmask || !a || !sim || !mean_cnt ||
        !grad_out || !gco || !grad_f || !contrast_form_ok(margin_mode, db, method, has_temperature, temperature))
        return bad_arg("amc3d_contrast_variant_backward: bad argument (C in 1..512, margin_mode 0..2, db 0..2, method 1..2)");
    if (rev && (!sel || !amc3d_contrast_backward_rows_supported(C) || (((uintptr_t)f | (uintptr_t)grad_f) & 15) ||
                (long)m * k > 0x7fffffffL))
        return bad_arg("amc3d_contrast_variant_backward: rev needs sel, C a multiple of 4 in 4..512 and 16-byte aligned rows");
    hipStream_t stream = (hipStream_t)stream_;
    const ContrastForm F{margin_mode, db, method, has_temperature, mu, nu, temperature};
    hipLaunchKernelGGL(contrast_variant_coef_kernel, dim3(div_up((long)m * 32, 256)), dim3(256), 0, stream, m, k, posmask, a, sel,
                       F, sim, mean_cnt, grad_out, gco);
    if (rev) {
        contrast_rows_launch(m, C, k, nbr_stride, f, norm, nbr, a, rev, sim, gco, grad_f, stream);
    } else {
        with_lpa_vpt(C, [&](auto lpa, auto vpt) {
            constexpr int LPA = decltype(lpa)::value, VPT = decltype(vpt)::value;
            hipLaunchKernelGGL((contrast_backward_edges_kernel<LPA, VPT>), dim3(div_up((long)m * LPA, 256)), dim3(256), 0, stream,
                               m, C, k, nbr_stride, f, norm, nbr, a, sel, sim, (const float *)gco, grad_f);
        });
    }
    return launch_status("amc3d_contrast_variant_backward");
}

AMC_API size_t amc3d_contrast_backward_mutual_workspace_bytes(int m) { return (size_t)(m > 0 ? m : 0) * sizeof(ContrastRecord) + 64; }

AMC_API int amc3d_contrast_backward_mutual(int m, int C, int k, int nbr_stride, const float *unit, const float *norm,
                                           const int *nbr, const unsigned char *posmask, const float *a,
                                           const unsigned char *mutual, const int *rev, float mu, float nu, float temperature,
                                           const float *sim, const float *stats, const float *mean_cnt, const float *grad_out,
                                           void *workspace, size_t workspace_bytes, float *grad_f, void *stream_)
{
    if (m <= 0) return 0;
    if (!amc3d_contrast_backward_csr_supported(C) || k <= 0 || nbr_stride < k || !unit || !norm || !nbr || !posmask || !a || !mutual ||
        !rev || (!sim && !stats) || !mean_cnt || !grad_out || !grad_f || !workspace ||
        workspace_bytes < amc3d_contrast_backward_mutual_workspace_bytes(m) || (long)m * C >= (1L << 34) ||
        (((uintptr_t)unit | (uintptr_t)grad_f | (uintptr_t)workspace) & 15))
        return bad_arg("amc3d_contrast_backward_mutual: bad argument (C must be 16, 32, 64, 128 or 256; 16-byte aligned rows)");
    hipStream_t stream = (hipStream_t)stream_;
    ContrastRecord *rec = (ContrastRecord *)workspace;
    if (stats)
        hipLaunchKernelGGL(contrast_record_stats_kernel, dim3(div_up(m, 256)), dim3(256), 0, stream, m, norm, a, mu, nu, temperature, stats,
                           mean_cnt, grad_out, rec);
    else
        hipLaunchKernelGGL(contrast_record_kernel, dim3(div_up((long)m * 32, 256)), dim3(256), 0, stream, m, k, norm, posmask, a, mu, nu,
                           temperature, sim, mean_cnt, grad_out, rec);
    const bool launched = with_lpr(C, [&](auto lpr) {
        hipLaunchKernelGGL((contrast_backward_mutual_kernel<decltype(lpr)::value>), dim3(div_up(m, 4)), dim3(256), 0, stream, m, k,
                           nbr_stride, unit, nbr, posmask, mutual, rev, (const ContrastRecord *)rec, temperature, grad_f);
    });
    if (!launched) return bad_arg("amc3d_contrast_backward_mutual: no row kernel for this width");
    return launch_status("amc3d_contrast_backward_mutual");
}

__global__ __launch_bounds__(256) void confusion_kernel(int C, long N, int v, long long ignore, int has_ignore,
                                                        const float *__restrict__ logits, const long long *__restrict__ target,
                                                        long long *__restrict__ cm, long long *__restrict__ invalid)
{
    extern __shared__ int s_bins[];
    for (int i = threadIdx.x; i <= v * v; i += 256) s_bins[i] = 0;
    __syncthreads();
    const int b = blockIdx.y;
    for (long n = (long)blockIdx.x * 256 + threadIdx.x; n < N; n += (long)gridDim.x * 256) {
        const float *lp = logits + (size_t)b * C * N + n;
        float best = lp[0];
        int arg = 0;
        for (int c = 1; c < C; ++c) {
            const float x = lp[(size_t)c * N];
            if (x > best || (x != x && best == best)) { best = x; arg = c; }
        }
        long long t = target[(size_t)b * N + n];
        int p = arg;
        if (has_ignore && t == ignore) { t = v - 1; p = v - 1; }
        if (t >= 0 && t < v) atomicAdd(&s_bins[(int)t * v + p], 1);
        else atomicAdd(&s_bins[v * v], 1);
    }
    __syncthreads();
    for (int i = threadIdx.x; i < v * v; i += 256)
        if (s_bins[i]) atomicAdd((unsigned long long *)(cm + i), (unsigned long long)s_bins[i]);
    if (threadIdx.x == 0 && s_bins[v * v]) atomicAdd((unsigned long long *)invalid, (unsigned long long)s_bins[v * v]);
}

AMC_API int amc3d_confusion_update(int B, int C, long N, const float *logits, const long long *target, long long ignore,
                                   int has_ignore, long long *cm, long long *invalid, void *stream_)
{
    if (B <= 0 || N <= 0) return 0;
    const int v = C + (has_ignore ? 1 : 0);
    if (C <= 0 || v > 64 || !logits || !target || !cm || !invalid) return bad_arg("amc3d_confusion_update: bad argument (at most 64 classes)");
    const int bx = (int)(div_up(N, 256) < 64 ? div_up(N, 256) : 64);
    hipLaunchKernelGGL(confusion_kernel, dim3(bx, B), dim3(256), (size_t)(v * v + 1) * sizeof(int), (hipStream_t)stream_, C, N, v, ignore,
                       has_ignore, logits, target, cm, invalid);
    return launch_status("amc3d_confusion_update");
}

AMC_API size_t amc3d_cross_entropy_workspace_bytes(int B, long N)
{
    return (size_t)(B > 0 ? B : 0) * (size_t)div_up(N > 0 ? N : 1, CE_THREADS) * 2 * sizeof(double);
}

AMC_API int amc3d_cross_entropy_forward(int B, int C, long N, const float *logits, const long long *target,
                                        long long ignore_index, float *lse, float *mean_cnt, void *workspace,
                                        size_t workspace_bytes, void *stream_)
{
    if (B <= 0 || N <= 0) return 0;
    if (C <= 0 || !logits || !target || !lse || !mean_cnt || !workspace ||
        workspace_bytes < amc3d_cross_entropy_workspace_bytes(B, N))
        return bad_arg("amc3d_cross_entropy_forward: bad argument");
    hipStream_t stream = (hipStream_t)stream_;
    const int gx = div_up(N, CE_THREADS);
    hipLaunchKernelGGL(ce_forward_kernel, dim3(gx, B), dim3(CE_THREADS), 0, stream, C, N, logits, target, ignore_index, lse,
                       (double *)workspace);
    hipLaunchKernelGGL(ce_finalize_kernel, dim3(1), dim3(1024), 0, stream, gx * B, (const double *)workspace, mean_cnt);
    return launch_status("amc3d_cross_entropy_forward");
}

AMC_API int amc3d_cross_entropy_backward(int B, int C, long N, const float *logits, const long long *target,
                                         long long ignore_index, const float *lse, const float *mean_cnt,
                                         const float *grad_out, float *dlogits, void *stream)
{
    if (B <= 0 || N <= 0) return 0;
    if (C <= 0 || !logits || !target || !lse || !mean_cnt || !grad_out || !dlogits)
        return bad_arg("amc3d_cross_entropy_backward: bad argument");
    hipLaunchKernelGGL(ce_backward_kernel, dim3(div_up(N, CE_THREADS), B), dim3(CE_THREADS), 0, (hipStream_t)stream, C, N,
                       logits, target, ignore_index, lse, mean_cnt, grad_out, dlogits);
    return launch_status("amc3d_cross_entropy_backward");
}

AMC_API size_t amc3d_cross_entropy_general_workspace_bytes(int B, long N) { return amc3d_cross_entropy_workspace_bytes(B, N); }

AMC_API int amc3d_cross_entropy_general_forward(int B, int C, long N, const float *logits, const long long *target,
                                                long long ignore_index, int has_ignore, float label_smoothing,
                                                const float *weight, float *lse, float *loss_den, void *workspace,
                                                size_t workspace_bytes, void *stream_)
{
    if (B <= 0 || N <= 0) return 0;
    if (C <= 0 || !logits || !target || !lse || !loss_den || !workspace || !(label_smoothing >= 0.f && label_smoothing < 1.f) ||
        workspace_bytes < amc3d_cross_entropy_general_workspace_bytes(B, N))
        return bad_arg("amc3d_cross_entropy_general_forward: bad argument (label_smoothing must be in [0, 1))");
    hipStream_t stream = (hipStream_t)stream_;
    const int gx = div_up(N, CE_THREADS);
    hipLaunchKernelGGL(ce_general_forward_kernel, dim3(gx, B), dim3(CE_THREADS), 0, stream, C, N, logits, target, ignore_index,
                       has_ignore, label_smoothing, weight, lse, (double *)workspace);
    hipLaunchKernelGGL(ce_finalize_kernel, dim3(1), dim3(1024), 0, stream, gx * B, (const double *)workspace, loss_den);
    return launch_status("amc3d_cross_entropy_general_forward");
}

AMC_API int amc3d_cross_entropy_general_backward(int B, int C, long N, const float *logits, const long long *target,
                                                 long long ignore_index, int has_ignore, float label_smoothing,
                                                 const float *weight, const float *lse, const float *loss_den,
                                                 const float *grad_out, float *dlogits, void *stream)
{
    if (B <= 0 || N <= 0) return 0;
    if (C <= 0 || !logits || !target || !lse || !loss_den || !grad_out || !dlogits ||
        !(label_smoothing >= 0.f && label_smoothing < 1.f))
        return bad_arg("amc3d_cross_entropy_general_backward: bad argument (label_smoothing must be in [0, 1))");
    hipLaunchKernelGGL(ce_general_backward_kernel, dim3(div_up(N, CE_THREADS), B), dim3(CE_THREADS), 0, (hipStream_t)stream, C, N,
                       logits, target, ignore_index, has_ignore, label_smoothing, weight, lse, loss_den, grad_out, dlogits);
    return launch_status("amc3d_cross_entropy_general_backward");
}
```

### amcontrast3d_amd/openpoints/AMContrast3D/MarginContrast.py

```python
import os

import torch
import torch.nn as nn
import torch.nn.functional as F

from openpoints.cpp.pointops.functions import pointops
from .AEF.ambiguity import ambiguity_function
from .AEF.function import _eps
from .AEF.utils import fetch_pxo, get_ftype, get_subscene_class, get_subscene_label_CBL


def _posmask_cnt(labels, neighbor_label):
    return torch.argmax(torch.unsqueeze(labels, -2), -1) == torch.argmax(neighbor_label, -1)


def plan_stage(n, i, stageACE_list, target, nstride, num_classes, ignore_index, ambiguity_args, ftype='f_out'):
    from amcontrast3d_amd import ops
    p, o = stageACE_list[n][i]['p_out'], stageACE_list[n][i]['offset']
    labels, _ = get_subscene_class(n, i, stageACE_list, target, nstride, num_classes, ignore_index)
    knn = ops.knnquery_squared if p.is_cuda else pointops.knnquery
    neighbor_idx, neighbor_d2 = knn(ambiguity_args.nsample, p, p, o, o)
    neighbor_idx = neighbor_idx[..., 1:]
    posmask = ops.posmask_from_labels(labels, neighbor_idx)
    a, shares = ambiguity_function(p, posmask, neighbor_idx.shape[1], neighbor_idx, ambiguity_args.cctype,
                                   ambiguity_args.ccbeta, ambiguity_args.vis, ambiguity_args.nu)
    anchors = ops.select_anchors(a) if a.is_cuda and a.dtype == torch.float32 else None
    rev = mutual = None
    default_form = ops.contrast_form_is_default(getattr(ambiguity_args, 'margin', 'adaptive'), getattr(ambiguity_args, 'db', '-m'),
                                                getattr(ambiguity_args, 'supervisedCL', 'Method1'),
                                                getattr(ambiguity_args, 'temperature', 1.0))
    if anchors is not None and neighbor_idx.shape[1] <= 64 and not default_form:
        rev = ops.contrast_csr(neighbor_idx, anchors)
    elif anchors is not None and neighbor_idx.shape[1] <= 64:
        d2 = neighbor_d2[..., 1:] if (torch.is_tensor(neighbor_d2) and neighbor_d2.dtype == torch.float32 and o.numel() == 1
                                      and neighbor_d2.shape[0] == neighbor_idx.shape[0] > neighbor_idx.shape[1] + 2) else None
        mutual, rev = ops.contrast_mutual(neighbor_idx, a, d2)
    return {'neighbor_idx': neighbor_idx, 'posmask': posmask, 'ambiguity': a, 'shares': shares, 'anchors': anchors,
            'rev': rev, 'mutual': mutual}


def _stage_plan(n, i, stageACE_list, target, nstride, num_classes, ignore_index, ambiguity_args, ftype):
    geometry = stageACE_list.get('geometry') if hasattr(stageACE_list, 'get') else None
    if geometry is not None and 'loss' in geometry:
        return geometry['loss'][i]
    return plan_stage(n, i, stageACE_list, target, nstride, num_classes, ignore_index, ambiguity_args, ftype)


class AmbiguityHead(nn.Module):
    def __init__(self):
        super().__init__()
        self.nstride = torch.tensor([4, 4, 4, 4])
        self.ftype = get_ftype('latent')[0]
        self.posmask_func = _posmask_cnt
        self.main = self.point_ambiguity

    def posmask_cnt(self, labels, neighbor_label):
        return _posmask_cnt(labels, neighbor_label)

    def point_ambiguity(self, n, i, stageACE_list, target, num_classes, ignore_index, ambiguity_args):
        return _stage_plan(n, i, stageACE_list, target, self.nstride, num_classes, ignore_index, ambiguity_args,
                           self.ftype)['ambiguity']

    def forward(self, target, stageACE_list, num_classes, ignore_index, ambiguity_args):
        return [self.main(ambiguity_args.stages, i, stageACE_list, target, num_classes, ignore_index, ambiguity_args)
                for i in range(ambiguity_args.stages_num)]


class ContrastHead(nn.Module):
    def __init__(self):
        super().__init__()
        self.nstride = torch.tensor([4, 4, 4, 4])
        self.stages = [('up', 0), ('up', 1), ('up', 2), ('up', 3)]
        self.ftype = get_ftype('latent')[0]
        self.project = None
        self.dist_func = self.dist_cos
        self.contrast_func = self.contrast_softnn_margin
        self.posmask_func = self.posmask_cnt
        self.main_contrast = self.point_contrast_margin

    def dist_cos(self, features, neighbor_feature):
        return F.cosine_similarity(torch.unsqueeze(features, -2), neighbor_feature, dim=2)

    def posmask_cnt(self, labels, neighbor_label):
        return _posmask_cnt(labels, neighbor_label)

    def contrast_softnn_margin(self, dist, posmask, ambiguity, ambiguity_args, invalid_mask=None):
        if ambiguity_args.margin == 'constant':
            margin = ambiguity_args.nu
        elif ambiguity_args.margin == 'adaptive':
            margin = ambiguity_args.mu * torch.unsqueeze(ambiguity, -1) + ambiguity_args.nu
        elif ambiguity_args.margin == 'learned':
            u = torch.mean(dist * ~posmask, 1)
            v = torch.mean(dist * posmask, 1)
            margin = (torch.unsqueeze(u, -1) - 1) * torch.unsqueeze(ambiguity, -1) + torch.unsqueeze(v, -1)

        if ambiguity_args.db == '-m':
            dist = (dist - margin) * posmask + dist * ~posmask
        elif ambiguity_args.db == '+m':
            dist = dist * posmask + (dist + margin) * ~posmask
        else:
            dist = dist * posmask + dist * ~posmask

        if ambiguity_args.temperature is not None:
            dist = dist / ambiguity_args.temperature
        exp = torch.exp(dist)
        if invalid_mask is not None:
            exp = exp * (1 - invalid_mask)

        pos = torch.sum(exp * posmask, axis=-1)
        neg = torch.sum(exp * (1 - posmask.int()), axis=-1)
        pos_neg = torch.sum(exp, axis=-1)
        if ambiguity_args.supervisedCL == 'Method1':
            loss = pos / pos_neg + _eps
        elif ambiguity_args.supervisedCL == 'Method2':
            loss = (exp * posmask) / (exp * posmask + neg.unsqueeze(-1)) + _eps
            loss = torch.sum(loss, axis=-1) / (torch.sum(posmask.int(), axis=-1) + _eps)
        return -torch.log(loss)

    def plan(self, target, stageACE_list, num_classes, ignore_index, ambiguity_args):
        from amcontrast3d_amd import ops
        with torch.no_grad(), ops.knn_grid_reuse():
            return [plan_stage(ambiguity_args.stages, i, stageACE_list, target.flatten(), self.nstride, num_classes,
                               ignore_index, ambiguity_args, self.ftype) for i in range(ambiguity_args.stages_num)]

    def point_contrast_margin(self, n, i, stageACE_list, target, num_classes, ignore_index, ambiguity_args):
        from amcontrast3d_amd import ops
        g = _stage_plan(n, i, stageACE_list, target, self.nstride, num_classes, ignore_index, ambiguity_args,
                        self.ftype)
        neighbor_idx, posmask, ambiguity_soft = g['neighbor_idx'], g['posmask'], g['ambiguity']
        target_ai = ambiguity_soft
        output_ai = stageACE_list['ambiguity'][i].flatten() if 'ambiguity' in stageACE_list.keys() else None
        fused = (ambiguity_args.margin == 'adaptive' and ambiguity_args.db == '-m'
                 and ambiguity_args.supervisedCL == 'Method1' and ambiguity_args.temperature is not None)
        stage = stageACE_list[n][i]
        f_cm = stage.channel_major() if fused and hasattr(stage, 'channel_major') else None
        if (f_cm is not None
                and ops.contrast_stage_supported_cm(f_cm, g.get('anchors'), g.get('rev'), g.get('mutual'))):
            loss = ops.contrast_stage_cm(f_cm, neighbor_idx, posmask, ambiguity_soft, ambiguity_args.mu, ambiguity_args.nu,
                                         ambiguity_args.temperature, g['anchors'], g['rev'], g['mutual'])
            return loss, output_ai, target_ai
        features = fetch_pxo(n, i, stageACE_list, self.ftype)[1]
        if features.dtype != torch.float32:
            features = features.float()
        k = neighbor_idx.shape[1]
        if fused:
            loss = ops.contrast_stage(features, neighbor_idx, posmask, ambiguity_soft, ambiguity_args.mu,
                                      ambiguity_args.nu, ambiguity_args.temperature, g.get('anchors'), g.get('rev'),
                                      g.get('mutual'))
            return loss, output_ai, target_ai
        if features.is_cuda:
            rev = g.get('rev') if g.get('mutual') is None else None
            loss = ops.contrast_stage_variant(features, neighbor_idx, posmask, ambiguity_soft, ambiguity_args.margin,
                                              ambiguity_args.db, ambiguity_args.supervisedCL, ambiguity_args.mu,
                                              ambiguity_args.nu, ambiguity_args.temperature, g.get('anchors'), rev)
            return loss, output_ai, target_ai
        keep = torch.logical_and(0 < ambiguity_soft, ambiguity_soft <= 1)
        m = neighbor_idx.shape[0]
        neighbor_feature = features[neighbor_idx.reshape(-1).long(), :].view(m, k, features.shape[1])
        dist = self.dist_func(features[keep], neighbor_feature[keep])
        loss = self.contrast_func(dist, posmask[keep], ambiguity_soft[keep], ambiguity_args)
        return torch.mean(loss), output_ai, target_ai

    def forward(self, output, target, stageACE_list, num_classes, ignore_index, ambiguity_args):
        loss_sum = 0
        target_ai_list = []
        for i in range(ambiguity_args.stages_num):
            loss, _, target_ai = self.main_contrast(ambiguity_args.stages, i, stageACE_list, target, num_classes,
                                                    ignore_index, ambiguity_args)
            loss_sum += loss
            target_ai_list.append(target_ai)
        return loss_sum, torch.cat(target_ai_list), target_ai_list
```

### amcontrast3d_amd/openpoints/loss/build.py

```python
import torch
from torch.nn import BCEWithLogitsLoss, CrossEntropyLoss

from openpoints.AMContrast3D.MarginContrast import ContrastHead
from openpoints.utils import registry

LOSS = registry.Registry('loss')


class CrossEntropy(CrossEntropyLoss):

    def forward(self, input, target):
        if ((self.label_smoothing > 0.0 or self.weight is not None) and self.reduction == 'mean' and input.is_cuda
                and input.dtype == torch.float32 and input.dim() == 3 and input.is_contiguous()
                and target.dtype == torch.int64 and target.shape == (input.shape[0], input.shape[2])
                and (self.weight is None or (self.weight.is_cuda and self.weight.dtype == torch.float32))):
            from amcontrast3d_amd.ops import cross_entropy_general
            return cross_entropy_general(input, target, self.ignore_index, self.label_smoothing, self.weight)
        return super().forward(input, target)


LOSS.register_module(name='CrossEntropy', module=CrossEntropy)
LOSS.register_module(name='CrossEntropyLoss', module=CrossEntropy)
LOSS.register_module(name='BCEWithLogitsLoss', module=BCEWithLogitsLoss)


def _cross_entropy(crit, logit, target):
    if (type(crit) is CrossEntropyLoss and crit.weight is None and crit.label_smoothing == 0.0
            and crit.reduction == 'mean' and logit.is_cuda and logit.dtype == torch.float32 and logit.dim() == 3):
        from amcontrast3d_amd.ops import cross_entropy_mean
        return cross_entropy_mean(logit, target, crit.ignore_index), target.flatten()
    target = target.flatten()
    return crit(logit.transpose(1, 2).reshape(-1, logit.shape[1]), target), target


def _l1_mean(crit, pred, target, rows=1024):
    if not (type(crit) is torch.nn.L1Loss and crit.reduction == 'mean' and pred.is_cuda and pred.dim() == 1
            and pred.shape == target.shape and pred.numel() > rows):
        return crit(pred, target)
    d = (pred - target).abs()
    n = d.numel()
    pad = (-n) % rows
    if pad:
        d = torch.nn.functional.pad(d, (0, pad))
    return d.view(-1, rows).sum(1).sum() / n


@LOSS.register_module()
class CrossEntropyAce(torch.nn.Module):

    def __init__(self, **kwargs):
        super().__init__()
        self.creterion = CrossEntropyLoss()
        self.contrast_head = ContrastHead()

    def forward(self, logit, target, stageACE_list, num_classes, ignore_index, ambiguity_args):
        ce, target = _cross_entropy(self.creterion, logit, target)
        contrast, _, _ = self.contrast_head(logit, target, stageACE_list, num_classes, ignore_index, ambiguity_args)
        return ambiguity_args.w1 * ce + ambiguity_args.w2 * contrast


@LOSS.register_module()
class CrossEntropyAcePre(torch.nn.Module):

    def __init__(self, **kwargs):
        super().__init__()
        self.creterion = CrossEntropyLoss()
        self.contrast_head = ContrastHead()
        self.MAE = torch.nn.L1Loss()
        self.MSE = torch.nn.MSELoss()
        self.HUBER = torch.nn.HuberLoss(reduction='mean', delta=0.1)

    def forward(self, logit, target, stageACE_list, num_classes, ignore_index, ambiguity_args):
        ce, target = _cross_entropy(self.creterion, logit, target)
        contrast, target_ai, _ = self.contrast_head(logit, target, stageACE_list, num_classes, ignore_index,
                                                    ambiguity_args)
        logits_ai = torch.cat(stageACE_list['ambiguity']).flatten()
        regression = _l1_mean(self.MAE, logits_ai, target_ai)
        ce = ambiguity_args.w1 * ce
        contrast = ambiguity_args.w2 * contrast
        regression = ambiguity_args.w3 * regression
        return ce + contrast, ce, contrast, regression


def build_criterion_from_cfg(cfg, **kwargs):
    return LOSS.build(cfg, **kwargs)
```

### amcontrast3d_amd/ops.py

```python
import ctypes

import torch
from torch.autograd import Function

from . import _lib, timing


def _ptr(t):
    return ctypes.c_void_p(t.data_ptr())


_dedicated = []


def _destroy_dedicated():
    if not _dedicated:
        return
    try:
        torch.cuda.synchronize()
        for handle, _ in _dedicated:
            _lib.load().amc3d_stream_destroy(handle)
    finally:
        _dedicated.clear()

# ... 625 lines not shown
        g = _contrast_grad_out(grad_out)
        nptr = _ptr(nbr)
        lib = _lib.load()
        route, anchors, rev = _contrast_route_and_lists("contrast_backward", ctx, f, nbr, a, anchors, rev, mutual, unit)
        if route == "mutual":
            grad_f = torch.empty_like(f)
            wb = int(lib.amc3d_contrast_backward_mutual_workspace_bytes(m))
            work = torch.empty(wb, dtype=torch.uint8, device=f.device)
            with torch.cuda.device(f.device), timing.span("contrast_backward", m * C * 8 + m * k * 10 + m * 8,
                                                          moved=m * C * 4 * (2 + k) + m * k * 42 + m * 40):
                _lib.check(lib.amc3d_contrast_backward_mutual(m, C, k, stride, _ptr(unit), _ptr(norm), nptr, _ptr(posmask), _ptr(a),
                                                              _ptr(mutual), _ptr(rev), mu, nu, temperature, _ptr(sim), None,
                                                              _ptr(mean_cnt), _ptr(g), _ptr(work), wb, _ptr(grad_f), _stream(f)),
                           "contrast_backward_mutual")
        elif route == "rows":
            grad_f = torch.empty_like(f)
            gco = torch.empty(m * k, dtype=torch.float32, device=f.device)
            with torch.cuda.device(f.device), timing.span("contrast_backward_csr", m * C * 8 + m * k * 17, moved=m * C * 4 * (2 + 2 * k) + m * k * 17):
                _lib.check(lib.amc3d_contrast_backward_csr(m, C, k, stride, _ptr(f), _ptr(norm), nptr, _ptr(posmask),
                                                           _ptr(a), _ptr(anchors), _ptr(rev), mu, nu, temperature,
                                                           _ptr(sim), _ptr(mean_cnt), _ptr(g), _ptr(gco), _ptr(grad_f),
                                                           _stream(f)), "contrast_backward_csr")
        else:
            grad_f = torch.zeros_like(f)
            with torch.cuda.device(f.device), timing.span("contrast_backward", m * C * 8 + m * k * 9 + m * 8, moved=m * C * 4 * (1 + 2 * k) + m * k * 9):
                _lib.check(lib.amc3d_contrast_backward(m, C, k, stride, _ptr(f), _ptr(norm), nptr, _ptr(posmask), _ptr(a),
                                                       _opt(anchors), mu, nu, temperature, _ptr(sim), _ptr(mean_cnt),
                                                       _ptr(g), _ptr(grad_f), _stream(f)), "contrast_backward")
        return (grad_f,) + (None,) * 9


contrast_stage = ContrastStage.apply


_MARGIN_MODE = {"constant": 0, "adaptive": 1, "learned": 2}
_SUPERVISED_CL = {"Method1": 1, "Method2": 2}


def contrast_form(margin, db, supervisedCL, temperature):
    if margin not in _MARGIN_MODE:
        raise ValueError(f"ambiguity_args.margin must be one of {sorted(_MARGIN_MODE)} (got {margin!r})")
    if supervisedCL not in _SUPERVISED_CL:
        raise ValueError(f"ambiguity_args.supervisedCL must be one of {sorted(_SUPERVISED_CL)} (got {supervisedCL!r})")
    return (_MARGIN_MODE[margin], {"-m": 1, "+m": 2}.get(db, 0), _SUPERVISED_CL[supervisedCL],
            0 if temperature is None else 1, 1.0 if temperature is None else float(temperature))


def contrast_form_is_default(margin, db, supervisedCL, temperature):
    return margin == "adaptive" and db == "-m" and supervisedCL == "Method1" and temperature is not None


def contrast_variant_forward(features, neighbor_idx, posmask, a, form, mu, nu, anchors=None):
    f = features.contiguous()
    m, C = f.shape
    nptr, k, stride, keep = _contrast_inputs(f, m, neighbor_idx, posmask, a, anchors)
    lib = _lib.load()
    norm, unit, sim, loss_pt, mean_cnt = _contrast_buffers(m, C, k, f.device, lib.amc3d_contrast_backward_csr_supported(C), True)
    mode, dbv, method, has_t, T = form
    with torch.cuda.device(f.device), timing.span("contrast_variant_forward", m * C * 4 + m * k * 13 + m * 12,
                                             moved=m * C * 4 * (3 + k) + m * k * 13 + m * 12):
        _lib.check(lib.amc3d_contrast_variant_forward(m, C, k, stride, _ptr(f), nptr, _ptr(posmask), _ptr(a), _opt(anchors),
                                                      mode, dbv, method, has_t, float(mu), float(nu), T, _ptr(norm),
                                                      _opt(unit), _ptr(sim), _ptr(loss_pt), _ptr(mean_cnt), _stream(f)),
                   "contrast_variant_forward")
    return {"f": f, "norm": norm, "unit": unit, "sim": sim, "loss_pt": loss_pt, "mean_cnt": mean_cnt, "nbr": keep, "k": k,
            "stride": stride}


class ContrastStageVariant(Function):

    @staticmethod
    def forward(ctx, features, neighbor_idx, posmask, a, margin, db, supervisedCL, mu, nu, temperature, anchors=None, rev=None):
        form = contrast_form(margin, db, supervisedCL, temperature)
        f = features.contiguous()
        _contrast_inputs(f, f.shape[0], neighbor_idx, posmask, a, anchors, rev)
        b = contrast_variant_forward(f, neighbor_idx, posmask, a, form, mu, nu, anchors)
        ctx.save_for_backward(b["f"], b["norm"], b["nbr"], posmask, a, b["sim"], b["mean_cnt"], anchors, rev)
        ctx.args = (form, float(mu), float(nu), b["k"], b["stride"])
        ctx.det = deterministic()
        return b["mean_cnt"][0].clone()

    @staticmethod
    def backward(ctx, grad_out):
        f, norm, nbr, posmask, a, sim, mean_cnt, anchors, rev = ctx.saved_tensors
        (mode, dbv, method, has_t, T), mu, nu, k, stride = ctx.args
        m, C = f.shape
        g = _contrast_grad_out(grad_out)
        lib = _lib.load()
        route, anchors, rev = _contrast_route_and_lists("contrast_variant_backward", ctx, f, nbr, a, anchors, rev)
        gather = route == "rows"
        grad_f = torch.empty_like(f) if gather else torch.zeros_like(f)
        gco = torch.empty(m * k, dtype=torch.float32, device=f.device)
        name = "contrast_variant_backward_csr" if gather else "contrast_variant_backward"
        with torch.cuda.device(f.device), timing.span(name, m * C * 8 + m * k * 17, moved=m * C * 4 * (2 + 2 * k) + m * k * 17):
            _lib.check(lib.amc3d_contrast_variant_backward(m, C, k, stride, _ptr(f), _ptr(norm), _ptr(nbr), _ptr(posmask), _ptr(a),
                                                           _opt(anchors), _ptr(rev) if gather else None, mode, dbv, method, has_t,
                                                           mu, nu, T, _ptr(sim), _ptr(mean_cnt), _ptr(g), _ptr(gco), _ptr(grad_f),
                                                           _stream(f)), name)
        return (grad_f,) + (None,) * 11


def contrast_stage_variant(features, neighbor_idx, posmask, a, margin, db, supervisedCL, mu, nu, temperature, anchors=None,
                           rev=None):
    return ContrastStageVariant.apply(features, neighbor_idx, posmask, a, margin, db, supervisedCL, mu, nu, temperature,
                                      anchors, rev)


class ContrastStageChannelMajor(Function):

    @staticmethod
    def forward(ctx, f_cm, neighbor_idx, posmask, a, mu, nu, temperature, anchors, rev, mutual):
        assert anchors is not None and rev is not None and mutual is not None
        f_cm = f_cm.contiguous()
        B, C, n = f_cm.shape
        m = B * n
        nptr, k, stride, keep = _contrast_inputs(f_cm, m, neighbor_idx, posmask, a, anchors, rev, mutual, "f_cm")
        norm, unit, stats, loss_pt, mean_cnt = _contrast_buffers(m, C, k, f_cm.device, True, False)
        with torch.cuda.device(f_cm.device), timing.span("contrast_forward", m * C * 4 + m * k * 5 + m * 20, moved=m * C * 4 * (2 + k) + m * k * 5 + m * 20):
            _lib.check(_lib.load().amc3d_contrast_forward_cm(B, C, n, k, stride, _ptr(f_cm), nptr, _ptr(posmask), _ptr(a), _ptr(anchors),
                                                             float(mu), float(nu), float(temperature), _ptr(norm), _ptr(unit),
                                                             None, _ptr(stats), _ptr(loss_pt), _ptr(mean_cnt), _stream(f_cm)),
                       "contrast_forward_cm")
        ctx.save_for_backward(norm, keep, posmask, a, stats, mean_cnt, rev, mutual, unit)
        ctx.args = (float(mu), float(nu), float(temperature), k, stride, B, C, n)
        return mean_cnt[0].clone()

    @staticmethod
    def backward(ctx, grad_out):
        norm, nbr, posmask, a, stats, mean_cnt, rev, mutual, unit = ctx.saved_tensors
        mu, nu, temperature, k, stride, B, C, n = ctx.args
        m = B * n
        g = _contrast_grad_out(grad_out)
        lib = _lib.load()
        grad_rows = torch.empty_like(unit)
        grad_cm = torch.empty(B, C, n, dtype=torch.float32, device=unit.device)
        wb = int(lib.amc3d_contrast_backward_mutual_workspace_bytes(m))
        work = torch.empty(wb, dtype=torch.uint8, device=unit.device)
        with torch.cuda.device(unit.device), timing.span("contrast_backward", m * C * 8 + m * k * 10 + m * 8,
                                                         moved=m * C * 4 * (4 + k) + m * k * 42 + m * 40):
            _lib.check(lib.amc3d_contrast_backward_mutual(m, C, k, stride, _ptr(unit), _ptr(norm), _ptr(nbr), _ptr(posmask), _ptr(a),
                                                          _ptr(mutual), _ptr(rev), mu, nu, temperature, None, _ptr(stats),
                                                          _ptr(mean_cnt), _ptr(g), _ptr(work), wb, _ptr(grad_rows), _stream(unit)),
                       "contrast_backward_mutual")
            _lib.check(lib.amc3d_transpose_cn(B, n, C, _ptr(grad_rows), _ptr(grad_cm), _stream(unit)), "transpose_cn")
        return (grad_cm,) + (None,) * 9


def contrast_stage_supported_cm(f_cm, anchors, rev, mutual):
    return (torch.is_tensor(f_cm) and f_cm.is_cuda and f_cm.dtype == torch.float32 and f_cm.dim() == 3 and anchors is not None
            and rev is not None and mutual is not None and bool(_lib.load().amc3d_contrast_backward_csr_supported(int(f_cm.shape[1]))))


contrast_stage_cm = ContrastStageChannelMajor.apply


def _bn_ws(C, dev, extra=0):
    n = int(_lib.load().amc3d_bn_workspace_bytes(C)) + extra
    return torch.empty(n, dtype=torch.uint8, device=dev), n


def _bn_running_args(bn):
    if bn is None or not bn.track_running_stats or bn.running_mean is None:
        return 0.0, None, None, None
    assert bn.running_mean.dtype == torch.float32 and bn.num_batches_tracked.dtype == torch.int64
    mom = -1.0 if bn.momentum is None else float(bn.momentum)
    return mom, _ptr(bn.running_mean), _ptr(bn.running_var), _ptr(bn.num_batches_tracked)


def _bn_stat_bufs(C, dev):
    mean = torch.empty(C, dtype=torch.float32, device=dev)
    return mean, torch.empty_like(mean), torch.empty_like(mean)


def _bn_begin(x, bn):
    x = x.contiguous()
    B, C = x.shape[0], x.shape[1]
    return x, (B, C, x.numel() // (B * C)), _bn_stat_bufs(C, x.device), _bn_ws(C, x.device), _bn_running_args(bn)


def _bn_finish(ctx, y, mean, var_u, *saved):
    ctx.save_for_backward(*saved)
    ctx.mark_non_differentiable(mean, var_u)
    ctx.set_materialize_grads(False)
    return y, mean, var_u


def _bn_backward_begin(x, dy, gamma, beta):
    B, C = x.shape[0], x.shape[1]
    return ((B, C, x.numel() // (B * C)), dy.contiguous(), torch.empty_like(x), torch.empty_like(gamma), torch.empty_like(beta),
            _bn_ws(C, x.device, extra=C * 8))


class BatchNormAct(Function):

    @staticmethod
    def forward(ctx, x, gamma, beta, eps, relu, bn=None):
        _need_gpu(x, gamma, beta)
        x, (B, C, L), (mean, invstd, var_u), (work, wb), (mom, rm, rv, nbt) = _bn_begin(x, bn)
        y = torch.empty_like(x)
        with torch.cuda.device(x.device), timing.span("bn_act_forward", x.numel() * 8, moved=x.numel() * 12):
            _lib.check(_lib.load().amc3d_bn_forward(B, C, L, 0, int(bool(relu)), float(eps), mom, _ptr(x), _ptr(gamma),
                                                    _ptr(beta), _ptr(y), None, _ptr(mean), _ptr(invstd), _ptr(var_u), rm, rv,
                                                    nbt, _ptr(work), wb, _stream(x)), "bn_forward")
        ctx.relu = bool(relu)
        return _bn_finish(ctx, y, mean, var_u, x, gamma, beta, mean, invstd)

    @staticmethod
    def backward(ctx, dy, _dm, _dv):
        x, gamma, beta, mean, invstd = ctx.saved_tensors
        (B, C, L), dy, dx, dgamma, dbeta, (work, wb) = _bn_backward_begin(x, dy, gamma, beta)
        with torch.cuda.device(x.device), timing.span("bn_act_backward", x.numel() * 12, moved=x.numel() * 20):
            _lib.check(_lib.load().amc3d_bn_backward(B, C, L, 1, int(ctx.relu), _ptr(x), _ptr(dy), None, _ptr(mean),
                                                     _ptr(invstd), _ptr(gamma), _ptr(beta), _ptr(dx), _ptr(dgamma),
                                                     _ptr(dbeta), _ptr(work), wb, _stream(x)), "bn_backward")
        return dx, dgamma, dbeta, None, None, None


class BatchNormResidualAct(Function):

    @staticmethod
    def forward(ctx, x, res, gamma, beta, eps, bn=None):
        _need_gpu(x, res, gamma, beta)
        _need_dtype(torch.float32, x=x, res=res, gamma=gamma, beta=beta)
        x, (B, C, L), (mean, invstd, var_u), (work, wb), (mom, rm, rv, nbt) = _bn_begin(x, bn)
        res = res.contiguous()
        assert x.shape == res.shape
        y = torch.empty_like(x)
        with torch.cuda.device(x.device), timing.span("bn_residual_forward", x.numel() * 12, moved=x.numel() * 16):
            _lib.check(_lib.load().amc3d_bn_residual_forward(B, C, L, float(eps), mom, _ptr(x), _ptr(res), _ptr(gamma), _ptr(beta),
                                                             _ptr(y), _ptr(mean), _ptr(invstd), _ptr(var_u), rm, rv, nbt,
                                                             _ptr(work), wb, _stream(x)), "bn_residual_forward")
        return _bn_finish(ctx, y, mean, var_u, x, y, gamma, beta, mean, invstd)

    @staticmethod
    def backward(ctx, dy, _dm, _dv):
        x, y, gamma, beta, mean, invstd = ctx.saved_tensors
        (B, C, L), dy, dx, dgamma, dbeta, (work, wb) = _bn_backward_begin(x, dy, gamma, beta)
        dres = torch.empty_like(x)
        with torch.cuda.device(x.device), timing.span("bn_residual_backward", x.numel() * 20, moved=x.numel() * 28):
            _lib.check(_lib.load().amc3d_bn_residual_backward(B, C, L, _ptr(x), _ptr(y), _ptr(dy), _ptr(mean), _ptr(invstd),
                                                              _ptr(gamma), _ptr(beta), _ptr(dx), _ptr(dres), _ptr(dgamma),
                                                              _ptr(dbeta), _ptr(work), wb, _stream(x)), "bn_residual_backward")
        return dx, dres, dgamma, dbeta, None, None


class BatchNormSigmoid(Function):

    @staticmethod
    def forward(ctx, x, gamma, beta, eps, bn=None):
        _need_gpu(x, gamma, beta)
        _need_dtype(torch.float32, x=x, gamma=gamma, beta=beta)
        x, (B, C, L), (mean, invstd, var_u), (work, wb), (mom, rm, rv, nbt) = _bn_begin(x, bn)
        y = torch.empty_like(x)
        with torch.cuda.device(x.device), timing.span("bn_sigmoid_forward", x.numel() * 8, moved=x.numel() * 12):
            _lib.check(_lib.load().amc3d_bn_sigmoid_forward(B, C, L, float(eps), mom, _ptr(x), _ptr(gamma), _ptr(beta), _ptr(y),
                                                            _ptr(mean), _ptr(invstd), _ptr(var_u), rm, rv, nbt, _ptr(work), wb,
                                                            _stream(x)), "bn_sigmoid_forward")
        return _bn_finish(ctx, y, mean, var_u, x, y, gamma, beta, mean, invstd)

    @staticmethod
    def backward(ctx, dy, _dm, _dv):
        x, y, gamma, beta, mean, invstd = ctx.saved_tensors
        (B, C, L), dy, dx, dgamma, dbeta, (work, wb) = _bn_backward_begin(x, dy, gamma, beta)
        with torch.cuda.device(x.device), timing.span("bn_sigmoid_backward", x.numel() * 16, moved=x.numel() * 24):
            _lib.check(_lib.load().amc3d_bn_sigmoid_backward(B, C, L, _ptr(x), _ptr(y), _ptr(dy), _ptr(mean), _ptr(invstd),
                                                             _ptr(gamma), _ptr(beta), _ptr(dx), _ptr(dgamma), _ptr(dbeta),
                                                             _ptr(work), wb, _stream(x)), "bn_sigmoid_backward")
        return dx, dgamma, dbeta, None, None


@torch.no_grad()
def bn_update_running(bn, mean, var_unbiased):
    _need_gpu(mean, var_unbiased, bn.running_mean, bn.running_var, bn.num_batches_tracked)
    mom = -1.0 if bn.momentum is None else float(bn.momentum)
    _lib.check(_lib.load().amc3d_bn_update_running(mean.numel(), mom, _ptr(mean), _ptr(var_unbiased),
                                                   _ptr(bn.running_mean), _ptr(bn.running_var),
                                                   _ptr(bn.num_batches_tracked), _stream(mean)), "bn_update_running")


class BatchNormMax(Function):

    @staticmethod
    def forward(ctx, x, gamma, beta, eps, relu, bn=None):
        _need_gpu(x, gamma, beta)
        x, (B, C, L), (mean, invstd, var_u), (work, wb), (mom, rm, rv, nbt) = _bn_begin(x, bn)
        _, _, M, K = x.shape
        y = torch.empty(B, C, M, dtype=torch.float32, device=x.device)
        arg = torch.empty(B, C, M, dtype=torch.uint8, device=x.device)
        with torch.cuda.device(x.device), timing.span("bn_max_forward", x.numel() * 4 + y.numel() * 5, moved=x.numel() * 8 + y.numel() * 5):
            _lib.check(_lib.load().amc3d_bn_forward(B, C, L, K, int(bool(relu)), float(eps), mom, _ptr(x), _ptr(gamma),
                                                    _ptr(beta), _ptr(y), _ptr(arg), _ptr(mean), _ptr(invstd), _ptr(var_u), rm, rv,
                                                    nbt, _ptr(work), wb, _stream(x)), "bn_forward")
        ctx.relu = bool(relu)
        if _pool_log is not None:
            _pool_log[_next_pool_seq()] = arg
        return _bn_finish(ctx, y, mean, var_u, x, gamma, beta, mean, invstd, arg)

    @staticmethod
    def backward(ctx, dy, _dm, _dv):
        x, gamma, beta, mean, invstd, arg = ctx.saved_tensors
        (B, C, L), dy, dx, dgamma, dbeta, (work, wb) = _bn_backward_begin(x, dy, gamma, beta)
        with torch.cuda.device(x.device), timing.span("bn_max_backward", x.numel() * 4 + dy.numel() * 9, moved=x.numel() * 8 + dy.numel() * 5):
            _lib.check(_lib.load().amc3d_bn_backward(B, C, L, x.shape[-1], int(ctx.relu), _ptr(x), _ptr(dy), _ptr(arg),
                                                     _ptr(mean), _ptr(invstd), _ptr(gamma), _ptr(beta), _ptr(dx),
                                                     _ptr(dgamma), _ptr(dbeta), _ptr(work), wb, _stream(x)),
                       "bn_backward")
# ... 1156 lines not shown
```

### amcontrast3d_amd/roofline.py

```python
import csv
import json
import os

HBM_PEAK_GBS = 8000.0
F32_MFMA_PEAK_TFLOPS = 157.3
ALGORITHMIC_PER_POINT = {"S": (1.197e9 / 192000, 137.7e9 / 192000), "L": (1.992e9 / 192000, 578.8e9 / 192000),
                         "XL": (4.26e9 / 192000, 3241e9 / 192000)}
GEOMETRY_OPS = ("furthest_point_sampling", "ball_query", "three_nn", "knnquery", "posmask", "ambiguity", "vote_labels",
                "select_anchors", "group_csr", "group_moments", "group_points", "contrast_csr")
OPERATOR_KERNELS = {
    "contrast_backward": ("contrast_backward_kernel", "contrast_backward_mutual_kernel", "contrast_record_kernel",
                          "contrast_record_stats_kernel"),
    "contrast_backward_csr": ("contrast_backward_rows_kernel", "contrast_backward_rows_wide_kernel", "contrast_coef_kernel"),
    "contrast_forward": ("contrast_forward_unit_kernel", "contrast_forward_kernel", "row_norm_kernel", "row_unit_kernel",
                         "row_unit_cm_kernel", "masked_mean_kernel"),
    "pointwise_conv_forward": ("pw_gemm_kernel", "gm_gemm_kernel", "gb_gemm_kernel", "gm_split_reduce"),
    "pointwise_conv_backward": ("pw_gemm_kernel", "pw_wgrad_kernel", "gw_wgrad_kernel", "gm_gemm_kernel", "gcc_reduce", "gb_gemm_kernel"),
    "sa_tail_forward": ("sat_kernel", "sat_finalize"),
    "sa_tail_backward": ("sat_kernel", "sat_bwd", "sat_pool_grad", "sat_alg_reduce", "sat_alg_dw"),
    "grouped_conv_bn_forward": ("lagg_stats", "lagg_expand", "lagg_finalize"),
    "grouped_conv_bn_backward": ("csr_collapse", "lagg_collapse", "lagg_bwd"),
    "local_aggregation_forward": ("lagg_stats", "lagg_pool", "lagg_finalize"),
    "local_aggregation_backward": ("lagg_bwd_scatter", "lagg_bwd_apply"),
    "bn_act_forward": ("bn_stats", "bn_act_kernel", "bn_fwd_channel"), "bn_act_backward": ("bn_bwd",),
    "bn_max_forward": ("bn_stats", "bn_max"), "bn_max_backward": ("bn_max_bwd", "bn_bwd"),
    "three_interpolate": ("three_interpolate",), "three_interpolate_grad": ("three_interpolate_grad", "scatter_pm"),
    "local_aggregation_backward_csr": ("lagg_bwd_scatter", "lagg_bwd_gather", "lagg_bwd_apply"),
    "three_interpolate_grad_csr": ("three_interpolate_grad_csr",), "masked_refine_backward_csr": ("refine_backward_csr",),
    "sa_residual_forward": ("sa_res_fwd",), "sa_residual_backward": ("sa_res_mask", "sa_res_bwd"),
    "cross_entropy_forward": ("ce_forward",), "cross_entropy_backward": ("ce_backward",),
    "furthest_point_sampling": ("fps_kernel",), "knnquery": ("kg_", "knn_"),
}


def _profiles_dir():
    return os.path.join(os.path.dirname(os.path.dirname(os.path.abspath(__file__))), "profiles")


def load_profiles(variant="S"):
    d = _profiles_dir()
    traffic, rows, name = {}, [], None
    try:
        with open(os.path.join(d, "hbm_traffic.json")) as fh:
            traffic = json.load(fh)
    except OSError:
        pass
    name = "round3_kernel_stats.csv" if variant == "S" else f"round3_{variant}_kernel_stats.csv"
    try:
        with open(os.path.join(d, name)) as fh:
            rows = list(csv.DictReader(fh))
    except OSError:
        name = None
    return traffic, rows, name


def family_traffic(op, kernels, steps):
    pats = OPERATOR_KERNELS.get(op)
    try:
        with open(os.path.join(_profiles_dir(), "round3_hbm_pmc.csv")) as fh:
            pmc = list(csv.DictReader(fh))
    except OSError:
        return None
    if not pats or not pmc:
        return None
    family = sorted(o for o, ps in OPERATOR_KERNELS.items() if set(ps) & set(pats) and o in kernels)
    allp = sorted({p for o in family for p in OPERATOR_KERNELS[o]})
    mb = sum(float(r["HBM_MB_per_step_corrected"]) for r in pmc if any(p in r["kernel"] for p in allp))
    alg = sum(kernels[o]["bytes"] for o in family) / steps
    if not mb or not alg:
        return None
    return {"operators": family, "traffic_GB_per_step": round(mb / 1e3, 3), "algorithmic_GB_per_step": round(alg / 1e9, 3),
            "ratio": round(mb * 1e6 / alg, 2), "file": "profiles/round3_hbm_pmc.csv"}


def rocprof_of(op, rows, csv_name):
    pats = OPERATOR_KERNELS.get(op)
    if not pats or not rows:
        return None
    hit = [r for r in rows if any(p in r["Name"] for p in pats)]
    if not hit:
        return None
    return {"file": f"profiles/{csv_name}", "us_per_step": round(sum(float(r["UsPerStep"]) for r in hit), 1),
            "kernels": [{"name": r["Name"].split("(")[0][-60:], "calls_per_step": float(r["CallsPerStep"]),
                         "avg_us": float(r["AverageUs"])} for r in hit[:6]]}


def operator_roofline(name, v, steps, traffic, rows, csv_name):
    nbytes, fl, tms, n = v["bytes"], v["flops"], v["total_ms"], max(v["launches"], 1)
    tr = traffic.get(name, {}).get("bytes_per_launch")
    if tr is None and traffic.get(name, {}).get("bytes_per_step"):
        tr = traffic[name]["bytes_per_step"] / max(n / steps, 1e-9)
    out = {"kernel": name, "avg_launch_ms": round(tms / n, 4), "launches_per_step": round(n / steps, 2),
           "ms_per_step": round(tms / steps, 4), "algorithmic_bytes_per_launch": int(nbytes / n),
           "moved_bytes_per_launch": int(v.get("moved", nbytes) / n),
           "moved_note": "what the implementation requests incl. gathered neighbour rows / atomic rows / re-read passes; mostly L2 + Infinity Cache",
           "traffic": tr, "traffic_over_algorithmic": round(tr / (nbytes / n), 2) if tr and nbytes else None,
           "rocprof": rocprof_of(name, rows, csv_name)}
    if fl > 0 and fl / max(nbytes, 1) > F32_MFMA_PEAK_TFLOPS * 1e12 / (HBM_PEAK_GBS * 1e9):
        ach = fl / (tms * 1e-3) / 1e12
        out.update(bound="mfma", achieved=round(ach, 2), peak=F32_MFMA_PEAK_TFLOPS, unit="TFLOP/s",
                   frac=round(ach / F32_MFMA_PEAK_TFLOPS, 4), algorithmic_flops_per_launch=fl / n)
    else:
        ach = nbytes / (tms * 1e-3) / 1e9
        out.update(bound="hbm", achieved=round(ach, 1), peak=HBM_PEAK_GBS, unit="GB/s", frac=round(ach / HBM_PEAK_GBS, 4))
    return out


def report(kernels, steps, ms_per_step, points_per_step, variant, mm, overlapped, fps=None):
    traffic, rows, csv_name = load_profiles(variant)
    crit = {k: v for k, v in kernels.items() if not (overlapped and k in GEOMETRY_OPS)}
    out = {"roofline": None, "roofline_hbm": None, "roofline_mfma": None, "roofline_step": None, "latency_chain": None}
    if crit:
        name, v = max(crit.items(), key=lambda kv: kv[1]["total_ms"])
        out["roofline"] = operator_roofline(name, v, steps, traffic, rows, csv_name)
        if out["roofline"]["traffic"] is None:
            out["roofline"]["traffic_family"] = family_traffic(name, kernels, steps)
        out["roofline"]["note"] = ("largest live HIP-event time among the operators of the feature half (the stream that bounds the "
                                   "overlapped step); achieved = SURVEY 8(d) algorithmic bytes or FLOPs / that time")
    hbm = {k: v for k, v in crit.items() if v["flops"] == 0 or v["flops"] / max(v["bytes"], 1) < 19.7}
    if hbm:
        name, v = max(hbm.items(), key=lambda kv: kv[1]["total_ms"])
        out["roofline_hbm"] = operator_roofline(name, v, steps, traffic, rows, csv_name)
    mf = [k for k in kernels if k.startswith(("grouped_conv", "pointwise_conv", "sa_tail", "local_aggregation"))]
    if mf:
        fl, tm = sum(kernels[k]["flops"] for k in mf), sum(kernels[k]["total_ms"] for k in mf)
        ach = fl / (tm * 1e-3) / 1e12
        out["roofline_mfma"] = {"bound": "mfma", "kernel": "+".join(sorted(mf)), "achieved": round(ach, 2), "peak": F32_MFMA_PEAK_TFLOPS,
                                "unit": "TFLOP/s", "frac": round(ach / F32_MFMA_PEAK_TFLOPS, 4), "traffic": None,
                                "ms_per_step": round(tm / steps, 3),
                                "note": "launched FLOPs (recomputation included) of every MFMA operator / their summed time"}
    if variant in ALGORITHMIC_PER_POINT and not mm:
        bpp, fpp = ALGORITHMIC_PER_POINT[variant]
        ab, af = bpp * points_per_step, fpp * points_per_step
        st = traffic.get("_step", {})
        meas = st.get("bytes_per_step") if st.get("workload") == f"{variant}:{points_per_step}" else None
        out["roofline_step"] = {
            "algorithmic_GB": round(ab / 1e9, 3), "algorithmic_GFLOP": round(af / 1e9, 1), "ms": round(ms_per_step, 3),
            "hbm_GBps": round(ab / (ms_per_step * 1e-3) / 1e9, 1), "hbm_frac": round(ab / (ms_per_step * 1e-3) / 1e9 / HBM_PEAK_GBS, 4),
            "mfma_TFLOPs": round(af / (ms_per_step * 1e-3) / 1e12, 2),
            "mfma_frac": round(af / (ms_per_step * 1e-3) / 1e12 / F32_MFMA_PEAK_TFLOPS, 4),
            "measured_hbm_GB": round(meas / 1e9, 2) if meas else None,
            "traffic_over_algorithmic": round(meas / ab, 2) if meas else None,
            "algorithmic_over_measured": round(ab / meas, 3) if meas else None,
            "operators_algorithmic_GB": round(sum(v["bytes"] for v in kernels.values()) / steps / 1e9, 3),
            "note": "algorithmic = SURVEY 8(d) (ideal fusion, forward x 3); measured = sum over every kernel of one step of FETCH_SIZE x 2 "
                    "+ WRITE_SIZE (profiles/hbm_traffic.json, rocprofv3 --pmc passes); operators_algorithmic = sum of the per-operator "
                    "figures (each operator's own inputs + outputs: what fusion of neighbouring operators could still remove)"}
    if fps and "furthest_point_sampling" in kernels:
        its = sum(fps["points"] // 4 ** k for k in range(1, fps["levels"]))
        out["latency_chain"] = {
            "kernel": "furthest_point_sampling", "iterations_per_cloud_all_levels": its, "joint_launch_ms": fps["joint_ms"],
            "us_per_iteration": round(fps["joint_ms"] * 1e3 / its, 3) if fps["joint_ms"] else None,
            "clouds_per_launch": fps["clouds"], "launch_every_steps": fps["lanes"],
            "hbm_bytes_per_launch": traffic.get("furthest_point_sampling", {}).get("bytes_per_launch"),
            "note": (f"serial arg-max chain, off the critical path: all sampling levels of {fps['lanes']} future batches run as one "
                     f"launch every {fps['lanes']} steps on the sampling queue, one workgroup per cloud")}
    return out
```

### amcontrast3d_amd/timing.py

```python
import collections

import torch

_enabled = False
_records = []
calls = None


class count_calls:

    def __enter__(self):
        global calls
        self.prev = calls
        calls = collections.Counter()
        return calls

    def __exit__(self, *exc):
        global calls
        calls = self.prev
        return False


def enable(flag=True):
    global _enabled
    _enabled = bool(flag)
    if not flag:
        _records.clear()


def enabled():
    return _enabled


def note(name):
    if calls is not None:
        calls[name] += 1


class span:
    __slots__ = ("name", "nbytes", "flops", "moved", "start")

    def __init__(self, name, nbytes=0, flops=0.0, moved=None):
        self.name, self.nbytes, self.flops, self.start = name, nbytes, flops, None
        self.moved = nbytes if moved is None else moved
        if calls is not None:
            calls[name] += 1

    def __enter__(self):
        if _enabled:
            self.start = torch.cuda.Event(enable_timing=True)
            self.start.record()
        return self

    def __exit__(self, *exc):
        if self.start is not None:
            end = torch.cuda.Event(enable_timing=True)
            end.record()
            _records.append((self.name, self.start, end, self.nbytes, self.flops, self.moved))
        return False


def collect():
    out = collections.OrderedDict()
    for name, s, e, nbytes, flops, moved in _records:
        d = out.setdefault(name, {"launches": 0, "total_ms": 0.0, "bytes": 0, "flops": 0.0, "moved": 0})
        d["launches"] += 1
        d["total_ms"] += s.elapsed_time(e)
        d["bytes"] += nbytes
        d["flops"] += flops
        d["moved"] += moved
    for d in out.values():
        d["avg_ms"] = d["total_ms"] / d["launches"]
        d["bytes_per_launch"] = d["bytes"] / d["launches"]
    _records.clear()
    return out
```

### include/amc3d.h

```cpp
#ifndef AMC3D_H
#define AMC3D_H

#include <stddef.h>
#include <stdint.h>

#ifdef __cplusplus
extern "C" {
#endif

const char *amc3d_version(void);
const char *amc3d_last_error(void);

int amc3d_stream_create_dedicated(void **stream);
int amc3d_stream_create_masked(void **stream, int first_cu, int n_cus);
int amc3d_reserve_scratch(int bytes_per_lane, int *scratch_out, void *stream);
int amc3d_stream_destroy(void *stream);


size_t amc3d_grid_search_workspace_bytes(int b, int n_support, int m_queries);
int amc3d_ball_query(int b, int n, int m, float radius, int nsample,
                     const float *new_xyz, const float *xyz, int *idx,
                     void *workspace, size_t workspace_bytes, void *stream);

int amc3d_group_points(int b, int c, int n, int npoints, int nsample,
                       const float *points, const int *idx, float *out, void *stream);

int amc3d_group_points_grad(int b, int c, int n, int npoints, int nsample,
                            const float *grad_out, const int *idx, float *grad_points,
                            void *workspace, size_t workspace_bytes, void *stream);

int amc3d_gather_points(int b, int c, int n, int npoints,
                        const float *points, const int *idx, float *out, void *stream);
int amc3d_gather_points_grad(int b, int c, int n, int npoints,
                             const float *grad_out, const int *idx, float *grad_points, void *stream);

size_t amc3d_fps_workspace_bytes(int b, int n);
int amc3d_furthest_point_sampling(int b, int n, int m, const float *dataset,
                                  float *temp, int *idxs, void *workspace, size_t workspace_bytes,
                                  void *stream);

int amc3d_three_nn(int b, int n, int m, const float *unknown, const float *known,
                   float *dist2, int *idx, void *workspace, size_t workspace_bytes, void *stream);

int amc3d_three_interpolate(int b, int c, int m, int n, const float *points,
                            const int *idx, const float *weight, float *out, void *stream);

int amc3d_three_interpolate_add(int b, int c, int m, int n, const float *points, const int *idx, const float *weight,
                                const float *base, float *out, void *stream);
int amc3d_three_interpolate_grad(int b, int c, int n, int m, const float *grad_out,
                                 const int *idx, const float *weight, float *grad_points,
                                 void *workspace, size_t workspace_bytes, void *stream);
int amc3d_three_interpolate_grad_route(int b, int c, int n, int m, int *cg, int *threads);
int amc3d_three_interpolate_grad_write(int b, int c, int n, int m, const float *grad_out, const int *idx,
                                       const float *weight, float *grad_points, void *stream);
int amc3d_three_interpolate_grad_lds(int b, int c, int n, int m, int cg, int threads, int accumulate, const float *grad_out,
                                     const int *idx, const float *weight, float *grad_points, void *stream);
int amc3d_three_interpolate_grad_csr(int b, int c, int n, int m, const float *grad_out, const int *idx, const float *weight,
                                     const int *rev_start, const int *rev_edge, float *grad_points, void *stream);


size_t amc3d_knnquery_workspace_bytes(int n, int m, int nsample, int nbatch);
int amc3d_knnquery_uses_grid(int m, int nsample, int n, int nbatch);
int amc3d_knnquery(int m, int nsample, int n, int nbatch, const float *xyz, const float *new_xyz,
                   const int *offset, const int *new_offset, int *idx, float *dist2,
                   void *workspace, size_t workspace_bytes, int reuse_grid, void *stream);


int amc3d_vote_labels(int m, int kr, int num_classes, const int *labels0, const int *nbr_idx, int *labels,
                      void *stream);

int amc3d_posmask(int m, int k, int nbr_stride, const int *labels, const int *nbr, unsigned char *posmask,
                  void *stream);

size_t amc3d_ambiguity_workspace_bytes(int m);
int amc3d_ambiguity(int m, int k, int nbr_stride, int mode, float beta, const float *p,
                    const unsigned char *posmask, const int *nbr, float *a, void *workspace,
                    size_t workspace_bytes, void *stream);

size_t amc3d_select_anchors_ints(int m);
int amc3d_select_anchors(int m, const float *a, int *sel, size_t sel_ints, void *stream);

int amc3d_contrast_forward(int m, int C, int k, int nbr_stride, const float *f, const int *nbr,
                           const unsigned char *posmask, const float *a, const int *sel, float mu, float nu,
                           float temperature, float *norm, float *unit, float *sim, float *stats, float *loss_pt,
                           float *mean_cnt, void *stream);

int amc3d_contrast_forward_cm(int b, int C, int n, int k, int nbr_stride, const float *f_cm, const int *nbr,
                              const unsigned char *posmask, const float *a, const int *sel, float mu, float nu,
                              float temperature, float *norm, float *unit, float *sim, float *stats, float *loss_pt,
                              float *mean_cnt, void *stream);

int amc3d_contrast_backward(int m, int C, int k, int nbr_stride, const float *f, const float *norm,
                            const int *nbr, const unsigned char *posmask, const float *a, const int *sel, float mu,
                            float nu, float temperature, const float *sim, const float *mean_cnt,
                            const float *grad_out, float *grad_f, void *stream);

size_t amc3d_contrast_csr_workspace_bytes(int m);
int amc3d_contrast_csr(int m, int k, int nbr_stride, const int *nbr, const int *sel, int *rev, void *workspace,
                       size_t workspace_bytes, void *stream);
int amc3d_contrast_backward_csr_supported(int C);
int amc3d_contrast_backward_rows_supported(int C);
int amc3d_contrast_backward_csr(int m, int C, int k, int nbr_stride, const float *f, const float *norm, const int *nbr,
                                const unsigned char *posmask, const float *a, const int *sel, const int *rev, float mu,
                                float nu, float temperature, const float *sim, const float *mean_cnt,
                                const float *grad_out, float *gco, float *grad_f, void *stream);

size_t amc3d_contrast_mutual_workspace_bytes(int m);
int amc3d_contrast_mutual(int m, int k, int nbr_stride, const int *nbr, const float *dist2, const float *a,
                          unsigned char *mutual, int *rev, void *workspace, size_t workspace_bytes, void *stream);
size_t amc3d_contrast_backward_mutual_workspace_bytes(int m);
int amc3d_contrast_backward_mutual(int m, int C, int k, int nbr_stride, const float *unit, const float *norm, const int *nbr,
                                   const unsigned char *posmask, const float *a, const unsigned char *mutual, const int *rev,
                                   float mu, float nu, float temperature, const float *sim, const float *stats ,
                                   const float *mean_cnt, const float *grad_out, void *workspace, size_t workspace_bytes,
                                   float *grad_f, void *stream);

int amc3d_contrast_variant_forward(int m, int C, int k, int nbr_stride, const float *f, const int *nbr,
                                   const unsigned char *posmask, const float *a, const int *sel, int margin_mode, int db,
                                   int method, int has_temperature, float mu, float nu, float temperature, float *norm,
                                   float *unit , float *sim, float *loss_pt, float *mean_cnt, void *stream);
int amc3d_contrast_variant_backward(int m, int C, int k, int nbr_stride, const float *f, const float *norm, const int *nbr,
                                    const unsigned char *posmask, const float *a, const int *sel, const int *rev ,
                                    int margin_mode, int db, int method, int has_temperature, float mu, float nu,
                                    float temperature, const float *sim, const float *mean_cnt, const float *grad_out,
                                    float *gco, float *grad_f, void *stream);

int amc3d_grouped_conv_supported(int cin, int cout);
int amc3d_transpose_cn(int b, int c, int n, const float *src, float *dst, void *stream);
int amc3d_grouped_conv_forward(int b, int cin, int cout, int n, int npoints, int nsample, const float *f_pm,
                               const float *dp, const int *idx, const float *weight, float *y, void *stream);
size_t amc3d_grouped_conv_workspace_bytes(int b, int cin, int cout, int npoints, int nsample);
int amc3d_grouped_conv_backward(int b, int cin, int cout, int n, int npoints, int nsample, const float *f_pm,
                                const float *dp, const int *idx, const float *weight, const float *dy,
                                float *df_pm, float *dweight, void *workspace, size_t workspace_bytes, void *stream);

int amc3d_confusion_update(int B, int C, long N, const float *logits, const long long *target, long long ignore,
                           int has_ignore, long long *cm, long long *invalid, void *stream);

size_t amc3d_cross_entropy_workspace_bytes(int B, long N);
int amc3d_cross_entropy_forward(int B, int C, long N, const float *logits, const long long *target,
                                long long ignore_index, float *lse, float *mean_cnt, void *workspace,
                                size_t workspace_bytes, void *stream);
int amc3d_cross_entropy_backward(int B, int C, long N, const float *logits, const long long *target,
                                 long long ignore_index, const float *lse, const float *mean_cnt,
                                 const float *grad_out, float *dlogits, void *stream);
size_t amc3d_cross_entropy_general_workspace_bytes(int B, long N);
int amc3d_cross_entropy_general_forward(int B, int C, long N, const float *logits, const long long *target,
                                        long long ignore_index, int has_ignore, float label_smoothing,
                                        const float *weight, float *lse, float *loss_den, void *workspace,
                                        size_t workspace_bytes, void *stream);
int amc3d_cross_entropy_general_backward(int B, int C, long N, const float *logits, const long long *target,
                                         long long ignore_index, int has_ignore, float label_smoothing,
                                         const float *weight, const float *lse, const float *loss_den,
                                         const float *grad_out, float *dlogits, void *stream);

int amc3d_pointwise_conv_forward(int b, int cin, int cout, long P, const float *x, const float *weight,
                                 const float *bias, float *y, void *stream);
size_t amc3d_pointwise_conv_forward_workspace_bytes(int b, int cin, int cout, long P, int has_bias);
int amc3d_pointwise_conv_forward_ws(int b, int cin, int cout, long P, const float *x, const float *weight,
                                    const float *bias, float *y, void *workspace, size_t workspace_bytes, void *stream);
size_t amc3d_pointwise_conv_workspace_bytes(int b, int cin, int cout, long P);
int amc3d_pointwise_conv_backward(int b, int cin, int cout, long P, const float *x, const float *weight,
                                  const float *dy, float *dx, float *dweight, void *workspace,
                                  size_t workspace_bytes, void *stream);
int amc3d_pointwise_conv_forward_strided(int b, int cin, int cout, long P, const float *x, const float *weight, long ldw,
                                         const float *bias, float *y, void *workspace, size_t workspace_bytes, void *stream);
int amc3d_pointwise_conv_backward_strided(int b, int cin, int cout, long P, const float *x, const float *weight, long ldw,
                                          const float *dy, float *dx, int dx_position_major, float *dweight, long lddw,
                                          void *workspace, size_t workspace_bytes, void *stream);

int amc3d_split_columns(int rows, int c1, int c2, const float *w, float *a, float *b, void *stream);
int amc3d_join_columns(int rows, int c1, int c2, const float *a, const float *b, float *w, void *stream);
int amc3d_bias_grad(int b, int c, long P, const float *dy, float *dbias, void *stream);

int amc3d_sa_residual_forward(int b, int cin, int cout, int n, int m, const float *f, const int *fps_idx,
                              const float *weight, const float *bias, const float *y, float *out, float *fi, void *stream);
size_t amc3d_sa_residual_workspace_bytes(int b, int cin, int cout, int m);
int amc3d_sa_residual_backward(int b, int cin, int cout, int n, int m, const float *dout, const float *out,
                               const float *fi, const int *fps_idx, const int *dup_flag, const float *weight, float *g, float *df,
                               float *dweight, float *dbias, void *workspace, size_t workspace_bytes, void *stream);
size_t amc3d_index_duplicates_workspace_bytes(int b, int n);
int amc3d_index_duplicates(int b, int n, int m, const int *idx, int *flag, void *workspace, size_t workspace_bytes, void *stream);

size_t amc3d_voxelize_workspace_bytes(int n);
int amc3d_voxelize(int n, const float *coord, double voxel_size, unsigned long long *key, int *idx_sort, int *voxel_idx,
                   int *start, int *count, int *nvox, void *workspace, size_t workspace_bytes, void *stream);
int amc3d_voxel_select(int nvox, const int *start, const int *count, const int *idx_sort, const int *rnd, int *idx_unique,
                       void *stream);
size_t amc3d_crop_nearest_workspace_bytes(int n);
int amc3d_crop_nearest(int n, const float *coord, int init_idx, int keep, float *d2, int *crop_idx, void *workspace,
                       size_t workspace_bytes, void *stream);
int amc3d_voxelize_f64(int n, const double *coord, double voxel_size, unsigned long long *key, int *idx_sort, int *voxel_idx,
                       int *start, int *count, int *nvox, void *workspace, size_t workspace_bytes, void *stream);
size_t amc3d_crop_nearest_f64_workspace_bytes(int n);
int amc3d_crop_nearest_f64(int n, const double *coord, int init_idx, int keep, double *d2, int *crop_idx, void *workspace,
                           size_t workspace_bytes, void *stream);

int amc3d_local_aggregation_supported(int cout, int nsample);
size_t amc3d_group_moments_bytes(int b, int n);
int amc3d_group_moments(int b, int n, int npoints, int nsample, const int *idx, const float *dp, void *moments,
                        size_t moments_bytes, void *stream);
size_t amc3d_local_aggregation_workspace_bytes(int b, int cout, int n, int npoints);
int amc3d_local_aggregation_forward(int b, int cout, int n, int npoints, int nsample, int training, int relu, float eps,
                                    float momentum, const float *g_cm, const int *idx, const float *dp, const float *w_dp,
                                    const void *moments, const float *gamma, const float *beta, float *g_pm, float *pooled,
                                    unsigned char *arg, float *ystar, float *mean, float *invstd, float *var_unbiased,
                                    double *gd, float *running_mean, float *running_var, long long *num_batches_tracked,
                                    int phase, double *sums, void *workspace, size_t workspace_bytes, void *stream);
int amc3d_local_aggregation_backward(int b, int cout, int n, int npoints, int nsample, int relu, const float *dpooled,
                                     const float *ystar, const unsigned char *arg, const float *g_pm, const int *idx,
                                     const float *dp, const float *w_dp, const void *moments, const double *gd,
                                     const float *mean, const float *invstd, const float *gamma, const float *beta,
                                     float *dg_cm, float *dw_dp, float *dgamma, float *dbeta, int phase, double *dsums,
                                     const double *count, void *workspace, size_t workspace_bytes, void *stream);

int amc3d_pointwise_conv_forward_bf16(int b, int cin, int cout, long P, const float *x, const float *weight,
                                      const float *bias, float *y, void *stream);
size_t amc3d_pointwise_conv_workspace_bytes_bf16(int b, int cin, int cout, long P);
int amc3d_pointwise_conv_backward_bf16(int b, int cin, int cout, long P, const float *x, const float *weight,
                                       const float *dy, float *dx, float *dweight, void *workspace,
                                       size_t workspace_bytes, void *stream);

int amc3d_grouped_conv_bn_supported(int cout, int nsample);
int amc3d_grouped_conv_bn_forward(int b, int cout, int n, int npoints, int nsample, int training, int relu, float eps,
                                  float momentum, const float *g_cm, const int *idx, const float *dp, const float *w_dp,
                                  const void *moments, const float *gamma, const float *beta, float *g_pm, float *x1,
                                  float *mean, float *invstd, float *var_unbiased, double *gd, float *running_mean,
                                  float *running_var, long long *num_batches_tracked, int phase, double *sums,
                                  void *workspace, size_t workspace_bytes, void *stream);
int amc3d_grouped_conv_bn_backward(int b, int cout, int n, int npoints, int nsample, int relu, const float *dx1,
                                   const float *g_pm, const int *idx, const float *dp, const float *w_dp,
                                   const void *moments, const double *gd, const float *mean, const float *invstd,
                                   const float *gamma, const float *beta, float *dg_cm, float *dw_dp, float *dgamma,
                                   float *dbeta, int phase, double *dsums, const double *count, void *workspace,
                                   size_t workspace_bytes, void *stream);

size_t amc3d_group_csr_workspace_bytes(int b, int npoints, int nsample);
int amc3d_group_csr(int b, int n, int npoints, int nsample, const int *idx, int *rev_start, int *rev_edge, void *workspace,
                    size_t workspace_bytes, void *stream);
int amc3d_group_csr_dp(int b, int npoints, int nsample, const int *rev_edge, const float *dp, float *rev_dp, void *stream);
int amc3d_group_moments_csr(int b, int n, int npoints, int nsample, const int *rev_start, const int *rev_edge,
                            const float *dp, void *moments, size_t moments_bytes, void *stream);
size_t amc3d_grouped_conv_bn_csr_workspace_bytes(int b, int cout, int n, int npoints, int nsample);
int amc3d_grouped_conv_bn_backward_csr(int b, int cout, int n, int npoints, int nsample, int relu, const float *dx1,
                                       int dx1_position_major, const float *g_pm, const int *rev_start, const int *rev_edge,
                                       const float *rev_dp , const float *dp, const float *w_dp, const void *moments, const double *gd, const float *mean,
                                       const float *invstd, const float *gamma, const float *beta, float *dg_cm, float *dw_dp,
                                       float *dgamma, float *dbeta, int phase, double *dsums, const double *count,
                                       void *workspace, size_t workspace_bytes, void *stream);
int amc3d_local_aggregation_forward_strided(int b, int cout, int n, int npoints, int nsample, int training,
                                            int relu, float eps, float momentum, const float *g_cm,
                                            const int *idx, const float *dp, const float *w_dp, long ldw,
                                            const void *moments, const float *gamma, const float *beta,
                                            float *g_pm, float *pooled, unsigned char *arg, float *ystar,
                                            float *mean, float *invstd, float *var_unbiased, double *gd,
                                            float *running_mean, float *running_var,
                                            long long *num_batches_tracked, int phase, double *sums,
                                            void *workspace, size_t workspace_bytes, void *stream);
int amc3d_local_aggregation_backward_strided(int b, int cout, int n, int npoints, int nsample, int relu,
                                             const float *dpooled, const float *ystar, const unsigned char *arg,
                                             const float *g_pm, const int *idx, const float *dp,
                                             const float *w_dp, long ldw, const void *moments, const double *gd,
                                             const float *mean, const float *invstd, const float *gamma,
                                             const float *beta, float *dg_cm, float *dw_dp, long lddw,
                                             float *dgamma, float *dbeta, int phase, double *dsums,
                                             const double *count_dev, void *workspace, size_t workspace_bytes,
                                             void *stream);
int amc3d_grouped_conv_bn_forward_strided(int b, int cout, int n, int npoints, int nsample, int training,
// ... 206 lines not shown
```

Before: 33.44 million points/s.

## Batch per-stage contrastive loss into multi-stage kernels for forward and backward

```diff
diff --git a/amcontrast3d_amd/_lib.py b/amcontrast3d_amd/_lib.py
--- a/amcontrast3d_amd/_lib.py
+++ b/amcontrast3d_amd/_lib.py
@@ -48,6 +48,9 @@
     "amc3d_contrast_backward_mutual_workspace_bytes": (_sz, [_i]),
     "amc3d_contrast_backward_mutual": (_i, [_i, _i, _i, _i, _vp, _vp, _vp, _vp, _vp, _vp, _vp, _f, _f, _f, _vp, _vp, _vp, _vp, _vp, _sz,
                                             _vp, _vp]),
+    "amc3d_contrast_stages_forward_cm": (_i, [_i, _vp, _f, _f, _f, _f, _vp, _vp]),
+    "amc3d_contrast_stages_backward_cm_workspace_bytes": (_sz, [_i, _vp]),
+    "amc3d_contrast_stages_backward_cm": (_i, [_i, _vp, _f, _f, _f, _f, _vp, _vp, _sz, _vp]),
     "amc3d_contrast_variant_forward": (_i, [_i, _i, _i, _i, _vp, _vp, _vp, _vp, _vp, _i, _i, _i, _i, _f, _f, _f, _vp, _vp, _vp, _vp,
                                             _vp, _vp]),
     "amc3d_contrast_variant_backward": (_i, [_i, _i, _i, _i, _vp, _vp, _vp, _vp, _vp, _vp, _vp, _i, _i, _i, _i, _f, _f, _f, _vp, _vp,
@@ -174,6 +177,15 @@
 }
 
 
+CONTRAST_MAX_STAGES = 8
+
+
+class ContrastStageDesc(ctypes.Structure):
+    _fields_ = ([(n, _i) for n in ("b", "C", "n", "k", "nbr_stride")]
+                + [(n, _vp) for n in ("f_cm", "nbr", "posmask", "a", "sel", "mutual", "rev", "norm", "unit", "stats", "loss_pt",
+                                      "mean_cnt", "rec", "grad_cm")])
+
+
 def build(force=False):
     cmd = ["make", "-C", _CSRC, "-j8"] + (["-B"] if force else [])
     proc = subprocess.run(cmd, stdout=subprocess.PIPE, stderr=subprocess.STDOUT, text=True)
diff --git a/amcontrast3d_amd/csrc/loss.hip b/amcontrast3d_amd/csrc/loss.hip
--- a/amcontrast3d_amd/csrc/loss.hip
+++ b/amcontrast3d_amd/csrc/loss.hip
@@ -1,6 +1,7 @@
 #include "common.h"
 
 #include <type_traits>
+#include <utility>
 
 namespace amc {
 
@@ -115,13 +116,13 @@
     if (q == 0) norm[i] = n;
 }
 
+template <int LPR> constexpr int unit_tile_points() { return LPR >= 32 ? 16 : 64; }
+
 template <int LPR, int TP>
-__global__ __launch_bounds__(256) void row_unit_cm_kernel(int n, const float *__restrict__ f_cm, float *__restrict__ norm,
-                                                          float *__restrict__ unit)
+__device__ __forceinline__ void row_unit_cm_tile(float *s_tile, int n, int b, int n0, const float *__restrict__ f_cm,
+                                                 float *__restrict__ norm, float *__restrict__ unit)
 {
     constexpr int C = 4 * LPR, TS = TP + 1;
-    extern __shared__ float s_tile[];
-    const int b = blockIdx.y, n0 = blockIdx.x * TP;
     for (int e = threadIdx.x; e < C * TP; e += 256) {
         const int ch = e / TP, pt = e - ch * TP;
         s_tile[ch * TS + pt] = n0 + pt < n ? f_cm[((size_t)b * C + ch) * n + n0 + pt] : 0.f;
@@ -145,6 +146,14 @@
             if (q == 0) norm[i] = nv;
         }
     }
+}
+
+template <int LPR, int TP>
+__global__ __launch_bounds__(256) void row_unit_cm_kernel(int n, const float *__restrict__ f_cm, float *__restrict__ norm,
+                                                          float *__restrict__ unit)
+{
+    extern __shared__ float s_tile[];
+    row_unit_cm_tile<LPR, TP>(s_tile, n, blockIdx.y, blockIdx.x * TP, f_cm, norm, unit);
 }
 
 __device__ __forceinline__ bool contrast_selected(float a) { return 0.f < a && a <= 1.f; }
@@ -396,8 +405,8 @@
 }
 
 template <int LPR>
-__global__ __launch_bounds__(256) void contrast_forward_unit_kernel(
-    int m, int k, int nbr_stride, const float *__restrict__ unit, const int *__restrict__ nbr,
+__device__ __forceinline__ void contrast_forward_unit_wave(
+    int w, int m, int k, int nbr_stride, const float *__restrict__ unit, const int *__restrict__ nbr,
     const unsigned char *__restrict__ posmask, const float *__restrict__ a, const int *__restrict__ sel, float mu, float nu,
     float temperature, float *__restrict__ sim, float *__restrict__ stats, float *__restrict__ loss_pt)
 {
@@ -405,7 +414,7 @@
     const int lane = threadIdx.x & 63, q = lane & (LPR - 1), r = lane / LPR;
     int i;
     float ai;
-    if (!contrast_anchor(sel, m, blockIdx.x * 4 + (threadIdx.x >> 6), a, i, ai)) return;
+    if (!contrast_anchor(sel, m, w, a, i, ai)) return;
     if (!contrast_selected(ai)) {
         if (lane == 0) loss_pt[i] = 0.f;
         return;
@@ -444,6 +453,16 @@
     }
 }
 
+template <int LPR>
+__global__ __launch_bounds__(256) void contrast_forward_unit_kernel(
+    int m, int k, int nbr_stride, const float *__restrict__ unit, const int *__restrict__ nbr,
+    const unsigned char *__restrict__ posmask, const float *__restrict__ a, const int *__restrict__ sel, float mu, float nu,
+    float temperature, float *__restrict__ sim, float *__restrict__ stats, float *__restrict__ loss_pt)
+{
+    contrast_forward_unit_wave<LPR>(blockIdx.x * 4 + (threadIdx.x >> 6), m, k, nbr_stride, unit, nbr, posmask, a, sel, mu, nu,
+                                    temperature, sim, stats, loss_pt);
+}
+
 __global__ __launch_bounds__(256) void contrast_forward_kernel(
     int m, int C, int k, int nbr_stride, const float *__restrict__ f, const float *__restrict__ norm,
     const int *__restrict__ nbr, const unsigned char *__restrict__ posmask, const float *__restrict__ a,
@@ -484,11 +503,9 @@
     if (sub == 0) loss_pt[i] = -logf(__fadd_rn(__fdiv_rn(psum, tsum), 1e-12f));
 }
 
-__global__ __launch_bounds__(1024) void masked_mean_kernel(int m, const float *__restrict__ loss_pt,
-                                                           const float *__restrict__ a, float *__restrict__ out)
-{
-    __shared__ double s_sum[16];
-    __shared__ int s_cnt[16];
+__device__ __forceinline__ float masked_mean_block(double (&s_sum)[16], int (&s_cnt)[16], int m, const float *__restrict__ loss_pt,
+                                                   const float *__restrict__ a, float *__restrict__ out)
+{
     double sum = 0.0;
     int cnt = 0;
     const int m4 = ((((uintptr_t)loss_pt | (uintptr_t)a) & 15) == 0) ? (m & ~3) : 0;
@@ -519,13 +536,24 @@
     }
     if ((threadIdx.x & 63) == 0) { s_sum[threadIdx.x >> 6] = sum; s_cnt[threadIdx.x >> 6] = cnt; }
     __syncthreads();
+    float mean = 0.f;
     if (threadIdx.x == 0) {
         double t = 0.0;
         int c = 0;
         for (int w = 0; w < 16; ++w) { t += s_sum[w]; c += s_cnt[w]; }
-        out[0] = (float)(t / (double)c);
+        mean = (float)(t / (double)c);
+        out[0] = mean;
         out[1] = (float)c;
     }
+    return mean;
+}
+
+__global__ __launch_bounds__(1024) void masked_mean_kernel(int m, const float *__restrict__ loss_pt,
+                                                           const float *__restrict__ a, float *__restrict__ out)
+{
+    __shared__ double s_sum[16];
+    __shared__ int s_cnt[16];
+    masked_mean_block(s_sum, s_cnt, m, loss_pt, a, out);
 }
 
 template <int LPA, int VPT>
@@ -742,18 +770,17 @@
     }
 }
 
-__global__ __launch_bounds__(256) void contrast_record_stats_kernel(int m, const float *__restrict__ norm, const float *__restrict__ a,
-                                                                    float mu, float nu, float temperature,
-                                                                    const float *__restrict__ stats, const float *__restrict__ mean_cnt,
-                                                                    const float *__restrict__ grad_out, ContrastRecord *__restrict__ rec)
-{
-    const int i = blockIdx.x * 256 + threadIdx.x;
+__device__ __forceinline__ void contrast_record_stats_anchor(int i, int m, const float *__restrict__ norm, const float *__restrict__ a,
+                                                             float mu, float nu, float temperature, const float *__restrict__ stats,
+                                                             const float *__restrict__ mean_cnt, float g,
+                                                             ContrastRecord *__restrict__ rec)
+{
     if (i >= m) return;
     const float ai = a[i];
     const bool selected = contrast_selected(ai);
     const float psum = selected ? stats[(size_t)i * 2] : 0.f, nsum = selected ? stats[(size_t)i * 2 + 1] : 1.f;
     const float tsum = __fadd_rn(psum, nsum);
-    const float scale = grad_out[0] / mean_cnt[1];
+    const float scale = g / mean_cnt[1];
     ContrastRecord o;
     o.norm = norm[i];
     o.coef = (selected && psum != 0.f) ? contrast_coef(scale, psum, tsum, temperature) : 0.f;
@@ -761,17 +788,23 @@
     rec[i] = o;
 }
 
+__global__ __launch_bounds__(256) void contrast_record_stats_kernel(int m, const float *__restrict__ norm, const float *__restrict__ a,
+                                                                    float mu, float nu, float temperature,
+                                                                    const float *__restrict__ stats, const float *__restrict__ mean_cnt,
+                                                                    const float *__restrict__ grad_out, ContrastRecord *__restrict__ rec)
+{
+    contrast_record_stats_anchor(blockIdx.x * 256 + threadIdx.x, m, norm, a, mu, nu, temperature, stats, mean_cnt, grad_out[0], rec);
+}
+
 template <int LPR>
-__global__ __launch_bounds__(256) void contrast_backward_mutual_kernel(
-    int m, int k, int nbr_stride, const float *__restrict__ unit, const int *__restrict__ nbr,
+__device__ __forceinline__ float4 contrast_mutual_row(
+    int lane, int n, int m, int k, int nbr_stride, const float *__restrict__ unit, const int *__restrict__ nbr,
     const unsigned char *__restrict__ posmask, const unsigned char *__restrict__ mutual, const int *__restrict__ rev,
-    const ContrastRecord *__restrict__ rec, float temperature, float *__restrict__ grad_f)
+    const ContrastRecord *__restrict__ rec, float temperature)
 {
     constexpr int R = 64 / LPR;
     constexpr int U = UNIT_U;
-    const int lane = threadIdx.x & 63, q = lane & (LPR - 1), r = lane / LPR, row0 = lane & ~(LPR - 1);
-    const int n = blockIdx.x * 4 + (threadIdx.x >> 6);
-    if (n >= m) return;
+    const int q = lane & (LPR - 1), r = lane / LPR, row0 = lane & ~(LPR - 1);
     const float4 *h4 = reinterpret_cast<const float4 *>(unit);
     const float4 *rec4 = reinterpret_cast<const float4 *>(rec);
     const float4 rn0 = rec4[(size_t)n * 2];
@@ -841,7 +874,138 @@
         acc.z += __shfl_xor(acc.z, d, 64);
         acc.w += __shfl_xor(acc.w, d, 64);
     }
-    if (r == 0) reinterpret_cast<float4 *>(grad_f)[(size_t)n * LPR + q] = acc;
+    return acc;
+}
+
+template <int LPR>
+__global__ __launch_bounds__(256) void contrast_backward_mutual_kernel(
+    int m, int k, int nbr_stride, const float *__restrict__ unit, const int *__restrict__ nbr,
+    const unsigned char *__restrict__ posmask, const unsigned char *__restrict__ mutual, const int *__restrict__ rev,
+    const ContrastRecord *__restrict__ rec, float temperature, float *__restrict__ grad_f)
+{
+    const int lane = threadIdx.x & 63;
+    const int n = blockIdx.x * 4 + (threadIdx.x >> 6);
+    if (n >= m) return;
+    const float4 acc = contrast_mutual_row<LPR>(lane, n, m, k, nbr_stride, unit, nbr, posmask, mutual, rev, rec, temperature);
+    if (lane < LPR) reinterpret_cast<float4 *>(grad_f)[(size_t)n * LPR + lane] = acc;
+}
+
+struct ContrastStages {
+    int nstages;
+    int first[AMC_CONTRAST_MAX_STAGES + 1];
+    AmcContrastStage st[AMC_CONTRAST_MAX_STAGES];
+};
+
+__device__ __forceinline__ int contrast_stage_of_block(const ContrastStages &S, int &blk)
+{
+    int s = 0;
+    while (s + 1 < S.nstages && blk >= S.first[s + 1]) ++s;
+    blk -= S.first[s];
+    return s;
+}
+
+template <int N> using int_c = std::integral_constant<int, N>;
+
+template <class F>
+__device__ __forceinline__ void device_with_lpr(int C, F &&fn)
+{
+    switch (C) {
+    case 16: fn(int_c<4>{}); break;
+    case 32: fn(int_c<8>{}); break;
+    case 64: fn(int_c<16>{}); break;
+    case 128: fn(int_c<32>{}); break;
+    case 256: fn(int_c<64>{}); break;
+    default: break;
+    }
+}
+
+template <int LPR> constexpr int grad_tile_points() { return LPR >= 64 ? 4 : LPR >= 32 ? 8 : 16; }
+
+__global__ __launch_bounds__(256) void contrast_stages_unit_kernel(const ContrastStages S)
+{
+    extern __shared__ float s_tile[];
+    int blk = blockIdx.x;
+    const AmcContrastStage &st = S.st[contrast_stage_of_block(S, blk)];
+    device_with_lpr(st.C, [&](auto lpr) {
+        constexpr int LPR = decltype(lpr)::value, TP = unit_tile_points<LPR>();
+        const int tiles = (st.n + TP - 1) / TP;
+        row_unit_cm_tile<LPR, TP>(s_tile, st.n, blk / tiles, (blk % tiles) * TP, st.f_cm, st.norm, st.unit);
+    });
+}
+
+__global__ __launch_bounds__(256) void contrast_stages_forward_kernel(const ContrastStages S, float mu, float nu, float temperature)
+{
+    int blk = blockIdx.x;
+    const AmcContrastStage &st = S.st[contrast_stage_of_block(S, blk)];
+    device_with_lpr(st.C, [&](auto lpr) {
+        contrast_forward_unit_wave<decltype(lpr)::value>(blk * 4 + (threadIdx.x >> 6), st.b * st.n, st.k, st.nbr_stride, st.unit, st.nbr,
+                                                         st.posmask, st.a, st.sel, mu, nu, temperature, nullptr, st.stats, st.loss_pt);
+    });
+}
+
+__global__ __launch_bounds__(1024) void contrast_stages_mean_kernel(const ContrastStages S, float scale, float *__restrict__ total)
+{
+    __shared__ double s_sum[16];
+    __shared__ int s_cnt[16];
+    __shared__ float s_mean[AMC_CONTRAST_MAX_STAGES];
+#pragma unroll 1
+    for (int s = 0; s < S.nstages; ++s) {
+        const AmcContrastStage &st = S.st[s];
+        const float l = masked_mean_block(s_sum, s_cnt, st.b * st.n, st.loss_pt, st.a, st.mean_cnt);
+        if (threadIdx.x == 0) s_mean[s] = l;
+        __syncthreads();
+    }
+    if (threadIdx.x == 0) {
+        float t = s_mean[0];
+        for (int s = 1; s < S.nstages; ++s) t = __fadd_rn(t, s_mean[s]);
+        total[0] = __fmul_rn(scale, t);
+    }
+}
+
+__global__ __launch_bounds__(256) void contrast_stages_record_kernel(const ContrastStages S, float mu, float nu, float temperature,
+                                                                     float scale, const float *__restrict__ grad_out)
+{
+    int blk = blockIdx.x;
+    const AmcContrastStage &st = S.st[contrast_stage_of_block(S, blk)];
+    contrast_record_stats_anchor(blk * 256 + threadIdx.x, st.b * st.n, st.norm, st.a, mu, nu, temperature, st.stats, st.mean_cnt,
+                                 __fmul_rn(grad_out[0], scale), (ContrastRecord *)st.rec);
+}
+
+template <int LPR, int TP>
+__device__ __forceinline__ void contrast_mutual_tile_cm(float *s_tile, const AmcContrastStage &st, int blk, float temperature)
+{
+    constexpr int C = 4 * LPR, TS = TP + 1;
+    const int tiles = (st.n + TP - 1) / TP;
+    const int b = blk / tiles, n0 = (blk % tiles) * TP;
+    const int np = min(TP, st.n - n0);
+    int lane = threadIdx.x & 63;
+    for (int pl = __builtin_amdgcn_readfirstlane(threadIdx.x >> 6); pl < np; pl += 4) {
+        asm volatile("" : "+v"(lane));
+        const float4 acc = contrast_mutual_row<LPR>(lane, b * st.n + n0 + pl, st.b * st.n, st.k, st.nbr_stride, st.unit, st.nbr, st.posmask,
+                                                    st.mutual, st.rev, (const ContrastRecord *)st.rec, temperature);
+        if (lane < LPR) {
+            s_tile[(4 * lane) * TS + pl] = acc.x;
+            s_tile[(4 * lane + 1) * TS + pl] = acc.y;
+            s_tile[(4 * lane + 2) * TS + pl] = acc.z;
+            s_tile[(4 * lane + 3) * TS + pl] = acc.w;
+        }
+    }
+    __syncthreads();
+    for (int e = threadIdx.x; e < C * TP; e += 256) {
+        const int ch = e / TP, pt = e - ch * TP;
+        if (pt < np) st.grad_cm[((size_t)b * C + ch) * st.n + n0 + pt] = s_tile[ch * TS + pt];
+    }
+}
+
+__global__ __launch_bounds__(256) void contrast_stages_backward_kernel(const ContrastStages S, float temperature)
+{
+    extern __shared__ float s_tile[];
+    int blk = blockIdx.x;
+    const AmcContrastStage &st = S.st[contrast_stage_of_block(S, blk)];
+    device_with_lpr(st.C, [&](auto lpr) {
+        constexpr int LPR = decltype(lpr)::value;
+        contrast_mutual_tile_cm<LPR, grad_tile_points<LPR>()>(s_tile, st, blk, temperature);
+    });
 }
 
 template <int LPR>
@@ -1259,7 +1423,6 @@
     return launch_status("amc3d_select_anchors");
 }
 
-template <int N> using int_c = std::integral_constant<int, N>;
 
 template <class F>
 static bool with_lpr(int C, F &&fn)
@@ -1505,6 +1668,129 @@
     return launch_status("amc3d_contrast_backward_mutual");
 }
 
+static bool contrast_stages_ok(int nstages, const AmcContrastStage *stages, bool backward)
+{
+    if (nstages < 0 || nstages > AMC_CONTRAST_MAX_STAGES || !stages) return false;
+    for (int s = 0; s < nstages; ++s) {
+        const AmcContrastStage &t = stages[s];
+        if (t.b <= 0 || t.n <= 0 || (long)t.b * t.n > 0x7fffffffL || !amc3d_contrast_backward_csr_supported(t.C) || t.k <= 0 ||
+            t.nbr_stride < t.k || (long)t.b * t.n * t.C >= (1L << 34) || !t.nbr || !t.posmask || !t.a || !t.norm || !t.unit ||
+            !t.stats || !t.mean_cnt || (((uintptr_t)t.unit) & 15))
+            return false;
+        if (backward ? (!t.mutual || !t.rev || !t.grad_cm) : (!t.f_cm || !t.sel || !t.loss_pt || (((uintptr_t)t.f_cm) & 15)))
+            return false;
+    }
+    return true;
+}
+
+template <class F>
+static bool contrast_stages_grid(ContrastStages &S, F &&blocks, bool fewest_first = false)
+{
+    long count[AMC_CONTRAST_MAX_STAGES];
+    for (int s = 0; s < S.nstages; ++s) count[s] = blocks(S.st[s]);
+    if (fewest_first)
+        for (int s = 1; s < S.nstages; ++s)
+            for (int t = s; t > 0 && count[t] < count[t - 1]; --t) {
+                std::swap(count[t], count[t - 1]);
+                std::swap(S.st[t], S.st[t - 1]);
+            }
+    long total = 0;
+    for (int s = 0; s < S.nstages; ++s) {
+        S.first[s] = (int)total;
+        total += count[s];
+        if (total > 0x7fffffffL) return false;
+    }
+    for (int s = S.nstages; s <= AMC_CONTRAST_MAX_STAGES; ++s) S.first[s] = (int)total;
+    return true;
+}
+
+template <class TileOf>
+static void contrast_stage_tiles(const AmcContrastStage &t, TileOf &&tile_of, long &blocks, size_t &lds)
+{
+    with_lpr(t.C, [&](auto lpr) {
+        const int TP = tile_of(lpr);
+        blocks = (long)t.b * div_up(t.n, TP);
+        lds = (size_t)t.C * (TP + 1) * sizeof(float);
+    });
+}
+
+static ContrastStages contrast_stages_arg(int nstages, const AmcContrastStage *stages)
+{
+    ContrastStages S{};
+    S.nstages = nstages;
+    for (int s = 0; s < nstages; ++s) S.st[s] = stages[s];
+    return S;
+}
+
+AMC_API int amc3d_contrast_stages_forward_cm(int nstages, const AmcContrastStage *stages, float mu, float nu, float temperature,
+                                             float scale, float *total, void *stream_)
+{
+    if (nstages == 0) return 0;
+    if (!contrast_stages_ok(nstages, stages, false) || !total)
+        return bad_arg("amc3d_contrast_stages_forward_cm: bad argument (1..8 stages; C must be 16, 32, 64, 128 or 256; f_cm and unit 16-byte aligned)");
+    hipStream_t stream = (hipStream_t)stream_;
+    ContrastStages tiles = contrast_stages_arg(nstages, stages), waves = tiles;
+    size_t lds = 0;
+    auto unit_blocks = [&](const AmcContrastStage &t) {
+        long blocks = 0;
+        size_t bytes = 0;
+        contrast_stage_tiles(t, [](auto lpr) { return unit_tile_points<decltype(lpr)::value>(); }, blocks, bytes);
+        lds = bytes > lds ? bytes : lds;
+        return blocks;
+    };
+    if (!contrast_stages_grid(tiles, unit_blocks) ||
+        !contrast_stages_grid(waves, [](const AmcContrastStage &t) { return (long)div_up((long)t.b * t.n, 4); }))
+        return bad_arg("amc3d_contrast_stages_forward_cm: the stages' blocks do not fit one grid");
+    hipLaunchKernelGGL(contrast_stages_unit_kernel, dim3(tiles.first[nstages]), dim3(256), lds, stream, tiles);
+    hipLaunchKernelGGL(contrast_stages_forward_kernel, dim3(waves.first[nstages]), dim3(256), 0, stream, waves, mu, nu, temperature);
+    hipLaunchKernelGGL(contrast_stages_mean_kernel, dim3(1), dim3(1024), 0, stream, waves, scale, total);
+    return launch_status("amc3d_contrast_stages_forward_cm");
+}
+
+static size_t contrast_stages_rec_bytes(const AmcContrastStage &t) { return ((size_t)t.b * t.n * sizeof(ContrastRecord) + 63) / 64 * 64; }
+
+AMC_API size_t amc3d_contrast_stages_backward_cm_workspace_bytes(int nstages, const AmcContrastStage *stages)
+{
+    size_t bytes = 64;
+    if (nstages < 0 || nstages > AMC_CONTRAST_MAX_STAGES || !stages) return bytes;
+    for (int s = 0; s < nstages; ++s)
+        if (stages[s].b > 0 && stages[s].n > 0) bytes += contrast_stages_rec_bytes(stages[s]);
+    return bytes;
+}
+
+AMC_API int amc3d_contrast_stages_backward_cm(int nstages, const AmcContrastStage *stages, float mu, float nu, float temperature,
+                                              float scale, const float *grad_out, void *workspace, size_t workspace_bytes,
+                                              void *stream_)
+{
+    if (nstages == 0) return 0;
+    if (!contrast_stages_ok(nstages, stages, true) || !grad_out || !workspace || (((uintptr_t)workspace) & 15) ||
+        workspace_bytes < amc3d_contrast_stages_backward_cm_workspace_bytes(nstages, stages))
+        return bad_arg("amc3d_contrast_stages_backward_cm: bad argument (1..8 stages; C must be 16, 32, 64, 128 or 256; unit and workspace 16-byte aligned)");
+    hipStream_t stream = (hipStream_t)stream_;
+    ContrastStages anchors = contrast_stages_arg(nstages, stages);
+    size_t at = 0;
+    for (int s = 0; s < nstages; ++s) {
+        anchors.st[s].rec = (char *)workspace + at;
+        at += contrast_stages_rec_bytes(anchors.st[s]);
+    }
+    ContrastStages tiles = anchors;
+    size_t lds = 0;
+    auto grad_blocks = [&](const AmcContrastStage &t) {
+        long blocks = 0;
+        size_t bytes = 0;
+        contrast_stage_tiles(t, [](auto lpr) { return grad_tile_points<decltype(lpr)::value>(); }, blocks, bytes);
+        lds = bytes > lds ? bytes : lds;
+        return blocks;
+    };
+    if (!contrast_stages_grid(anchors, [](const AmcContrastStage &t) { return (long)div_up((long)t.b * t.n, 256); }) ||
+        !contrast_stages_grid(tiles, grad_blocks, true))
+        return bad_arg("amc3d_contrast_stages_backward_cm: the stages' blocks do not fit one grid");
+    hipLaunchKernelGGL(contrast_stages_record_kernel, dim3(anchors.first[nstages]), dim3(256), 0, stream, anchors, mu, nu, temperature,
+                       scale, grad_out);
+    hipLaunchKernelGGL(contrast_stages_backward_kernel, dim3(tiles.first[nstages]), dim3(256), lds, stream, tiles, temperature);
+    return launch_status("amc3d_contrast_stages_backward_cm");
+}
+
 __global__ __launch_bounds__(256) void confusion_kernel(int C, long N, int v, long long ignore, int has_ignore,
                                                         const float *__restrict__ logits, const long long *__restrict__ target,
                                                         long long *__restrict__ cm, long long *__restrict__ invalid)
diff --git a/amcontrast3d_amd/openpoints/AMContrast3D/MarginContrast.py b/amcontrast3d_amd/openpoints/AMContrast3D/MarginContrast.py
--- a/amcontrast3d_amd/openpoints/AMContrast3D/MarginContrast.py
+++ b/amcontrast3d_amd/openpoints/AMContrast3D/MarginContrast.py
@@ -77,6 +77,7 @@
         self.contrast_func = self.contrast_softnn_margin
         self.posmask_func = self.posmask_cnt
         self.main_contrast = self.point_contrast_margin
+        self._forward_plans = None
 
     def dist_cos(self, features, neighbor_feature):
         return F.cosine_similarity(torch.unsqueeze(features, -2), neighbor_feature, dim=2)
@@ -123,19 +124,33 @@
             return [plan_stage(ambiguity_args.stages, i, stageACE_list, target.flatten(), self.nstride, num_classes,
                                ignore_index, ambiguity_args, self.ftype) for i in range(ambiguity_args.stages_num)]
 
-    def point_contrast_margin(self, n, i, stageACE_list, target, num_classes, ignore_index, ambiguity_args):
+    def _plan_once(self, n, i, stageACE_list, target, num_classes, ignore_index, ambiguity_args):
+        plans = getattr(self, "_forward_plans", None)
+        if plans is not None and i in plans:
+            return plans[i]
+        g = _stage_plan(n, i, stageACE_list, target, self.nstride, num_classes, ignore_index, ambiguity_args, self.ftype)
+        if plans is not None:
+            plans[i] = g
+        return g
+
+    def _stage_channel_major(self, n, i, stageACE_list, target, num_classes, ignore_index, ambiguity_args):
         from amcontrast3d_amd import ops
-        g = _stage_plan(n, i, stageACE_list, target, self.nstride, num_classes, ignore_index, ambiguity_args,
-                        self.ftype)
-        neighbor_idx, posmask, ambiguity_soft = g['neighbor_idx'], g['posmask'], g['ambiguity']
-        target_ai = ambiguity_soft
-        output_ai = stageACE_list['ambiguity'][i].flatten() if 'ambiguity' in stageACE_list.keys() else None
+        g = self._plan_once(n, i, stageACE_list, target, num_classes, ignore_index, ambiguity_args)
         fused = (ambiguity_args.margin == 'adaptive' and ambiguity_args.db == '-m'
                  and ambiguity_args.supervisedCL == 'Method1' and ambiguity_args.temperature is not None)
         stage = stageACE_list[n][i]
         f_cm = stage.channel_major() if fused and hasattr(stage, 'channel_major') else None
-        if (f_cm is not None
-                and ops.contrast_stage_supported_cm(f_cm, g.get('anchors'), g.get('rev'), g.get('mutual'))):
+        if f_cm is not None and not ops.contrast_stage_supported_cm(f_cm, g.get('anchors'), g.get('rev'), g.get('mutual')):
+            f_cm = None
+        return g, fused, f_cm
+
+    def point_contrast_margin(self, n, i, stageACE_list, target, num_classes, ignore_index, ambiguity_args):
+        from amcontrast3d_amd import ops
+        g, fused, f_cm = self._stage_channel_major(n, i, stageACE_list, target, num_classes, ignore_index, ambiguity_args)
+        neighbor_idx, posmask, ambiguity_soft = g['neighbor_idx'], g['posmask'], g['ambiguity']
+        target_ai = ambiguity_soft
+        output_ai = stageACE_list['ambiguity'][i].flatten() if 'ambiguity' in stageACE_list.keys() else None
+        if f_cm is not None:
             loss = ops.contrast_stage_cm(f_cm, neighbor_idx, posmask, ambiguity_soft, ambiguity_args.mu, ambiguity_args.nu,
                                          ambiguity_args.temperature, g['anchors'], g['rev'], g['mutual'])
             return loss, output_ai, target_ai
@@ -161,12 +176,42 @@
         loss = self.contrast_func(dist, posmask[keep], ambiguity_soft[keep], ambiguity_args)
         return torch.mean(loss), output_ai, target_ai
 
-    def forward(self, output, target, stageACE_list, num_classes, ignore_index, ambiguity_args):
+    def _merged_stages(self, target, stageACE_list, num_classes, ignore_index, ambiguity_args):
+        from amcontrast3d_amd import _lib
+        merged = []
+        if self.main_contrast != self.point_contrast_margin:
+            return merged
+        for i in range(min(ambiguity_args.stages_num, _lib.CONTRAST_MAX_STAGES)):
+            g, _, f_cm = self._stage_channel_major(ambiguity_args.stages, i, stageACE_list, target, num_classes, ignore_index,
+                                                   ambiguity_args)
+            if f_cm is None:
+                break
+            merged.append((g, f_cm))
+        return merged
+
+    def forward(self, output, target, stageACE_list, num_classes, ignore_index, ambiguity_args, scale=None):
+        self._forward_plans = {}
+        try:
+            return self._forward(target, stageACE_list, num_classes, ignore_index, ambiguity_args, scale)
+        finally:
+            self._forward_plans = None
+
+    def _forward(self, target, stageACE_list, num_classes, ignore_index, ambiguity_args, scale):
         loss_sum = 0
         target_ai_list = []
-        for i in range(ambiguity_args.stages_num):
+        merged = self._merged_stages(target, stageACE_list, num_classes, ignore_index, ambiguity_args)
+        whole = len(merged) == ambiguity_args.stages_num
+        if merged:
+            from amcontrast3d_amd import ops
+            loss_sum, _ = ops.contrast_stages_cm(
+                [(f_cm, g['neighbor_idx'], g['posmask'], g['ambiguity'], g['anchors'], g['rev'], g['mutual']) for g, f_cm in merged],
+                ambiguity_args.mu, ambiguity_args.nu, ambiguity_args.temperature, scale if whole and scale is not None else 1.0)
+            target_ai_list = [g['ambiguity'] for g, _ in merged]
+        for i in range(len(merged), ambiguity_args.stages_num):
             loss, _, target_ai = self.main_contrast(ambiguity_args.stages, i, stageACE_list, target, num_classes,
                                                     ignore_index, ambiguity_args)
-            loss_sum += loss
+            loss_sum = loss_sum + loss
             target_ai_list.append(target_ai)
+        if scale is not None and not (merged and whole):
+            loss_sum = scale * loss_sum
         return loss_sum, torch.cat(target_ai_list), target_ai_list
diff --git a/amcontrast3d_amd/openpoints/loss/build.py b/amcontrast3d_amd/openpoints/loss/build.py
--- a/amcontrast3d_amd/openpoints/loss/build.py
+++ b/amcontrast3d_amd/openpoints/loss/build.py
@@ -55,8 +55,9 @@
 
     def forward(self, logit, target, stageACE_list, num_classes, ignore_index, ambiguity_args):
         ce, target = _cross_entropy(self.creterion, logit, target)
-        contrast, _, _ = self.contrast_head(logit, target, stageACE_list, num_classes, ignore_index, ambiguity_args)
-        return ambiguity_args.w1 * ce + ambiguity_args.w2 * contrast
+        contrast, _, _ = self.contrast_head(logit, target, stageACE_list, num_classes, ignore_index, ambiguity_args,
+                                            scale=ambiguity_args.w2)
+        return ambiguity_args.w1 * ce + contrast
 
 
 @LOSS.register_module()
@@ -73,11 +74,10 @@
     def forward(self, logit, target, stageACE_list, num_classes, ignore_index, ambiguity_args):
         ce, target = _cross_entropy(self.creterion, logit, target)
         contrast, target_ai, _ = self.contrast_head(logit, target, stageACE_list, num_classes, ignore_index,
-                                                    ambiguity_args)
+                                                    ambiguity_args, scale=ambiguity_args.w2)
         logits_ai = torch.cat(stageACE_list['ambiguity']).flatten()
         regression = _l1_mean(self.MAE, logits_ai, target_ai)
         ce = ambiguity_args.w1 * ce
-        contrast = ambiguity_args.w2 * contrast
         regression = ambiguity_args.w3 * regression
         return ce + contrast, ce, contrast, regression
 
diff --git a/amcontrast3d_amd/ops.py b/amcontrast3d_amd/ops.py
--- a/amcontrast3d_amd/ops.py
+++ b/amcontrast3d_amd/ops.py
@@ -801,6 +801,88 @@
 
 
 contrast_stage_cm = ContrastStageChannelMajor.apply
+
+_STAGE_TENSORS = 7
+
+
+def _contrast_stage_descs(stages):
+    descs = (_lib.ContrastStageDesc * len(stages))()
+    for d, st in zip(descs, stages):
+        for name, v in st.items():
+            setattr(d, name, _ptr(v) if torch.is_tensor(v) else v)
+    return descs
+
+
+class ContrastStagesChannelMajor(Function):
+
+    @staticmethod
+    def forward(ctx, mu, nu, temperature, scale, *tensors):
+        assert tensors and len(tensors) % _STAGE_TENSORS == 0
+        lib, dev = _lib.load(), tensors[0].device
+        nst = len(tensors) // _STAGE_TENSORS
+        if nst > _lib.CONTRAST_MAX_STAGES:
+            raise ValueError(f"contrast_stages_cm: at most {_lib.CONTRAST_MAX_STAGES} stages per call (got {nst})")
+        means = torch.empty(nst, 2, dtype=torch.float32, device=dev)
+        total = torch.empty((), dtype=torch.float32, device=dev)
+        stages, keep, nbytes, moved = [], [], 0, 0
+        for s in range(nst):
+            f_cm, neighbor_idx, posmask, a, anchors, rev, mutual = tensors[s * _STAGE_TENSORS:(s + 1) * _STAGE_TENSORS]
+            assert anchors is not None and rev is not None and mutual is not None and f_cm.dim() == 3 and f_cm.device == dev
+            f_cm = f_cm.contiguous()
+            B, C, n = f_cm.shape
+            m = B * n
+            nptr, k, stride, nbr = _contrast_inputs(f_cm, m, neighbor_idx, posmask, a, anchors, rev, mutual, "f_cm")
+            norm, unit, stats, loss_pt, _ = _contrast_buffers(m, C, k, dev, True, False)
+            stages.append(dict(b=B, C=C, n=n, k=k, nbr_stride=stride, f_cm=f_cm, nbr=nptr, posmask=posmask, a=a, sel=anchors,
+                               mutual=mutual, rev=rev, norm=norm, unit=unit, stats=stats, loss_pt=loss_pt, mean_cnt=means[s]))
+            keep += [nbr, posmask, a, rev, mutual, norm, unit, stats]
+            nbytes += m * C * 4 + m * k * 5 + m * 20
+            moved += m * C * 4 * (2 + k) + m * k * 5 + m * 20
+        with torch.cuda.device(dev), timing.span("contrast_forward", nbytes, moved=moved):
+            _lib.check(lib.amc3d_contrast_stages_forward_cm(nst, _contrast_stage_descs(stages), float(mu), float(nu),
+                                                            float(temperature), float(scale), _ptr(total), _stream(total)),
+                       "contrast_stages_forward_cm")
+        timing.note("contrast_forward", nst - 1)
+        timing.note("contrast_stages_forward")
+        ctx.save_for_backward(means, *keep)
+        ctx.args = (float(mu), float(nu), float(temperature), float(scale),
+                    [{key: st[key] for key in ("b", "C", "n", "k", "nbr_stride")} for st in stages])
+        ctx.mark_non_differentiable(means)
+        ctx.set_materialize_grads(False)
+        return total, means
+
+    @staticmethod
+    def backward(ctx, grad_total, _grad_means):
+        mu, nu, temperature, scale, sizes = ctx.args
+        nst = len(sizes)
+        if grad_total is None:
+            return (None,) * (4 + nst * _STAGE_TENSORS)
+        means, saved = ctx.saved_tensors[0], ctx.saved_tensors[1:]
+        lib, dev = _lib.load(), means.device
+        g = _contrast_grad_out(grad_total)
+        stages, grads, nbytes, moved = [], [], 0, 0
+        for s, sz in enumerate(sizes):
+            nbr, posmask, a, rev, mutual, norm, unit, stats = saved[s * 8:(s + 1) * 8]
+            m, C, k = sz["b"] * sz["n"], sz["C"], sz["k"]
+            grad_cm = torch.empty(sz["b"], C, sz["n"], dtype=torch.float32, device=dev)
+            stages.append(dict(sz, nbr=nbr, posmask=posmask, a=a, mutual=mutual, rev=rev, norm=norm, unit=unit, stats=stats,
+                               mean_cnt=means[s], grad_cm=grad_cm))
+            grads += [grad_cm] + [None] * (_STAGE_TENSORS - 1)
+            nbytes += m * C * 8 + m * k * 10 + m * 8
+            moved += m * C * 4 * (2 + k) + m * k * 42 + m * 40
+        descs = _contrast_stage_descs(stages)
+        wb = int(lib.amc3d_contrast_stages_backward_cm_workspace_bytes(nst, descs))
+        work = torch.empty(wb, dtype=torch.uint8, device=dev)
+        with torch.cuda.device(dev), timing.span("contrast_backward", nbytes, moved=moved):
+            _lib.check(lib.amc3d_contrast_stages_backward_cm(nst, descs, mu, nu, temperature, scale, _ptr(g), _ptr(work), wb,
+                                                             _stream(means)), "contrast_stages_backward_cm")
+        timing.note("contrast_backward", nst - 1)
+        timing.note("contrast_stages_backward")
+        return (None,) * 4 + tuple(grads)
+
+
+def contrast_stages_cm(stages, mu, nu, temperature, scale=1.0):
+    return ContrastStagesChannelMajor.apply(mu, nu, temperature, scale, *(t for st in stages for t in st))
 
 
 def _bn_ws(C, dev, extra=0):
diff --git a/amcontrast3d_amd/roofline.py b/amcontrast3d_amd/roofline.py
--- a/amcontrast3d_amd/roofline.py
+++ b/amcontrast3d_amd/roofline.py
@@ -10,10 +10,11 @@
                 "select_anchors", "group_csr", "group_moments", "group_points", "contrast_csr")
 OPERATOR_KERNELS = {
     "contrast_backward": ("contrast_backward_kernel", "contrast_backward_mutual_kernel", "contrast_record_kernel",
-                          "contrast_record_stats_kernel"),
+                          "contrast_record_stats_kernel", "contrast_stages_record_kernel", "contrast_stages_backward_kernel"),
     "contrast_backward_csr": ("contrast_backward_rows_kernel", "contrast_backward_rows_wide_kernel", "contrast_coef_kernel"),
     "contrast_forward": ("contrast_forward_unit_kernel", "contrast_forward_kernel", "row_norm_kernel", "row_unit_kernel",
-                         "row_unit_cm_kernel", "masked_mean_kernel"),
+                         "row_unit_cm_kernel", "masked_mean_kernel", "contrast_stages_unit_kernel", "contrast_stages_forward_kernel",
+                         "contrast_stages_mean_kernel"),
     "pointwise_conv_forward": ("pw_gemm_kernel", "gm_gemm_kernel", "gb_gemm_kernel", "gm_split_reduce"),
     "pointwise_conv_backward": ("pw_gemm_kernel", "pw_wgrad_kernel", "gw_wgrad_kernel", "gm_gemm_kernel", "gcc_reduce", "gb_gemm_kernel"),
     "sa_tail_forward": ("sat_kernel", "sat_finalize"),
diff --git a/amcontrast3d_amd/timing.py b/amcontrast3d_amd/timing.py
--- a/amcontrast3d_amd/timing.py
+++ b/amcontrast3d_amd/timing.py
@@ -32,9 +32,9 @@
     return _enabled
 
 
-def note(name):
+def note(name, n=1):
     if calls is not None:
-        calls[name] += 1
+        calls[name] += n
 
 
 class span:
diff --git a/include/amc3d.h b/include/amc3d.h
--- a/include/amc3d.h
+++ b/include/amc3d.h
@@ -114,6 +114,26 @@
                                    float mu, float nu, float temperature, const float *sim, const float *stats ,
                                    const float *mean_cnt, const float *grad_out, void *workspace, size_t workspace_bytes,
                                    float *grad_f, void *stream);
+
+#define AMC_CONTRAST_MAX_STAGES 8
+typedef struct AmcContrastStage {
+    int b, C, n, k, nbr_stride;
+    const float *f_cm;
+    const int *nbr;
+    const unsigned char *posmask;
+    const float *a;
+    const int *sel;
+    const unsigned char *mutual;
+    const int *rev;
+    float *norm, *unit, *stats, *loss_pt, *mean_cnt;
+    void *rec;
+    float *grad_cm;
+} AmcContrastStage;
+int amc3d_contrast_stages_forward_cm(int nstages, const AmcContrastStage *stages, float mu, float nu, float temperature,
+                                     float scale, float *total, void *stream);
+size_t amc3d_contrast_stages_backward_cm_workspace_bytes(int nstages, const AmcContrastStage *stages);
+int amc3d_contrast_stages_backward_cm(int nstages, const AmcContrastStage *stages, float mu, float nu, float temperature,
+                                      float scale, const float *grad_out, void *workspace, size_t workspace_bytes, void *stream);
 
 int amc3d_contrast_variant_forward(int m, int C, int k, int nbr_stride, const float *f, const int *nbr,
                                    const unsigned char *posmask, const float *a, const int *sel, int margin_mode, int db,
```

Measured after the change: 34.44 million points/s (median of 6 runs). 1.03x the previous value.
